# plumer/pbrs

Hardware: AMD Instinct MI355X
Metric: Msamples/s (higher is better)
Workload: dtype f32

## Files before the change

include/pbrs_gpu.h:

```cpp
#ifndef PBRS_GPU_H
#define PBRS_GPU_H

#include <stdint.h>

#ifdef __cplusplus
extern "C" {
#endif

#define PBRS_OK 0
#define PBRS_E_INVALID (-1)
#define PBRS_E_DEVICE (-2)
#define PBRS_E_NO_SCENE (-3)
#define PBRS_E_LIMIT (-4)

#define PBRS_LEAF_FLAG 0x80000000u
#define PBRS_TLAS_LEAF_KIND_SHIFT 8

typedef struct pbrs_node {
    float min[3];
    uint32_t a;
    float max[3];
    uint32_t b;
} pbrs_node;

// ... 109 lines not shown
    uint32_t tlas_height;
    uint32_t n_instances;
    const pbrs_instance* instances;
    uint32_t n_shapes;
    const pbrs_shape* shapes;
    uint32_t n_meshes;
    const pbrs_mesh* meshes;
    uint32_t n_blas_nodes;
    const pbrs_node* blas_nodes;
    uint32_t n_triangles;
    const pbrs_tri_verts* tri_verts;
    const pbrs_tri_shade* tri_shade;
    uint32_t n_materials;
    const pbrs_material* materials;
    uint32_t n_bxdfs;
    const pbrs_bxdf* bxdfs;
    uint32_t n_area_lights;
    const pbrs_area_light* area_lights;
    uint32_t n_delta_lights;
    const pbrs_delta_light* delta_lights;
    float env_constant[3];
    uint32_t env_kind;
    uint32_t n_textures;
    const pbrs_texture* textures;
    uint32_t n_tex_floats;
    const float* tex_floats;
    uint32_t n_tex_words;
    const uint32_t* tex_words;
    uint32_t env_texture;
    float env_scale[3];
    uint32_t n_fourier_tables;
    const pbrs_fourier_table* fourier_tables;
} pbrs_scene_desc;

typedef struct pbrs_camera {
    float center[3];
    uint32_t width;
    float c[3];
    uint32_t height;
    float a[3];
    float pad0;
    float b[3];
    float pad1;
} pbrs_camera;

typedef struct pbrs_stats {
    uint64_t samples;
    uint64_t closest_rays;
    uint64_t shadow_rays;
    uint64_t shade_events;
    uint64_t tlas_nodes, blas_nodes, instances, instance_hits, triangles, tri_shading;
    uint64_t spheres, quads, cuboids, disks;
    uint64_t shadow_tlas_nodes, shadow_blas_nodes, shadow_instances, shadow_triangles, shadow_prims;
    uint64_t invalid_samples;
    float ms_raygen, ms_extend, ms_shade, ms_shadow, ms_accumulate, ms_total;
    uint32_t launches_extend, launches_shadow, launches_shade, passes;
    uint32_t kernel_features_extend, kernel_features_shadow;
    uint64_t paths_at_bounce[16];
    uint64_t shadow_rays_at_bounce[16];
} pbrs_stats;
#define PBRS_STATS_MAX_BOUNCES 16

typedef struct pbrs_ctx pbrs_ctx;

int pbrs_create(int device_ordinal, pbrs_ctx** out);
void pbrs_destroy(pbrs_ctx*);
const char* pbrs_last_error(const pbrs_ctx*);
int pbrs_set_stream(pbrs_ctx*, void* hip_stream);

int pbrs_set_pass_overlap(pbrs_ctx*, int enabled);

int pbrs_upload_scene(pbrs_ctx*, const pbrs_scene_desc*);

typedef struct pbrs_render_params {
    uint32_t x0, y0, w, h;
    uint32_t strata_x, strata_y;
    uint32_t max_depth;
    uint32_t samples_per_pass;
    uint64_t seed;
    uint32_t collect_counters;
    uint32_t time_stages;
    uint32_t band_rows, band_count, band_index;
    uint32_t integrator;
} pbrs_render_params;
#define PBRS_INTEGRATOR_PATH 0u
#define PBRS_INTEGRATOR_DIRECT 1u
#define PBRS_INTEGRATOR_MATERIALS 2u
#define PBRS_INTEGRATOR_NORMALS 3u

int pbrs_render_tile(pbrs_ctx*, const pbrs_camera*, const pbrs_render_params*, float* rgb_out_host, pbrs_stats* stats_out);
int pbrs_render_tile_device(pbrs_ctx*, const pbrs_camera*, const pbrs_render_params*, float* rgb_out_device, pbrs_stats* stats_out);
int pbrs_collect_stats(pbrs_ctx*, pbrs_stats* stats_out);

typedef struct pbrs_aov_buffers {
    float* albedo;
    float* normal;
    float* coverage;
    float* depth;
    uint32_t* instance;
    uint32_t* material;
    uint32_t* prim;
} pbrs_aov_buffers;
int pbrs_render_tile_aovs(pbrs_ctx*, const pbrs_camera*, const pbrs_render_params*, float* rgb_out_host, const pbrs_aov_buffers* aovs_host,
                          pbrs_stats* stats_out);
int pbrs_render_tile_aovs_device(pbrs_ctx*, const pbrs_camera*, const pbrs_render_params*, float* rgb_out_device,
                                 const pbrs_aov_buffers* aovs_device, pbrs_stats* stats_out);

enum pbrs_filter_kind { PBRS_FILTER_BOX = 0, PBRS_FILTER_TRIANGLE = 1, PBRS_FILTER_GAUSSIAN = 2, PBRS_FILTER_MITCHELL = 3, PBRS_FILTER_LANCZOS = 4 };
#define PBRS_FILTER_MAX_RADIUS 4.0f
typedef struct pbrs_pixel_filter {
    uint32_t kind;
    float radius[2];
    float a, b;
    uint32_t pad;
} pbrs_pixel_filter;
int pbrs_render_tile_filtered(pbrs_ctx*, const pbrs_camera*, const pbrs_render_params*, const pbrs_pixel_filter*, float* rgb_out_host,
                              pbrs_stats* stats_out);
int pbrs_render_tile_filtered_device(pbrs_ctx*, const pbrs_camera*, const pbrs_render_params*, const pbrs_pixel_filter*,
                                     float* rgb_out_device, pbrs_stats* stats_out);

#define PBRS_DENOISE_MAX_ITERATIONS 6
#define PBRS_DENOISE_DEMODULATE 1u
#define PBRS_DENOISE_ID_STOP 2u
typedef struct pbrs_denoise_params {
    uint32_t w, h;
    uint32_t iterations;
    uint32_t flags;
    float sigma_color, sigma_normal, sigma_depth;
    float albedo_floor;
} pbrs_denoise_params;
typedef struct pbrs_denoise_guides {
    const float* albedo;
    const float* normal;
    const float* depth;
    const uint32_t* instance;
} pbrs_denoise_guides;
int pbrs_denoise(pbrs_ctx*, const pbrs_denoise_params*, const float* rgb_in_host, const pbrs_denoise_guides* guides_host, float* rgb_out_host);
int pbrs_denoise_device(pbrs_ctx*, const pbrs_denoise_params*, const float* rgb_in_device, const pbrs_denoise_guides* guides_device,
                        float* rgb_out_device);

typedef struct pbrs_hit_record {
    float t;
    uint32_t inst;
    uint32_t prim;
    float b1, b2;
} pbrs_hit_record;
int pbrs_intersect_rays(pbrs_ctx*, uint32_t n, const float* origins, const float* dirs, const float* tmax,
                        pbrs_hit_record* hits_out, uint8_t* occluded_out);
typedef struct pbrs_intersect_info {
    uint32_t wide_any, wide_closest;
    uint32_t slow_any, slow_closest;
} pbrs_intersect_info;
int pbrs_last_intersect_info(const pbrs_ctx*, pbrs_intersect_info* out);
int pbrs_camera_rays(pbrs_ctx*, const pbrs_camera*, const pbrs_render_params*, uint32_t sample_index, float* origins_out,
                     float* dirs_out);
int pbrs_numeric_eval(pbrs_ctx*, uint32_t fn, uint32_t n, const float* x, const float* y, float* out);
int pbrs_numeric_eval_k(pbrs_ctx*, uint32_t fn, uint32_t n, uint32_t k, const uint32_t* ops, uint32_t* out);
int pbrs_render_sample_radiance(pbrs_ctx*, const pbrs_camera*, const pbrs_render_params*, uint32_t sample_index, float* rgb_out_host);

int pbrs_render_tile_aovs_var(pbrs_ctx*, const pbrs_camera*, const pbrs_render_params*, float* rgb_out_host, const pbrs_aov_buffers* aovs_host,
                              float* variance_host, pbrs_stats* stats_out);
int pbrs_render_tile_aovs_var_device(pbrs_ctx*, const pbrs_camera*, const pbrs_render_params*, float* rgb_out_device,
                                     const pbrs_aov_buffers* aovs_device, float* variance_device, pbrs_stats* stats_out);

typedef struct pbrs_denoise_var_params {
    uint32_t w, h;
    uint32_t iterations;
    uint32_t flags;
    float sigma_luminance, sigma_normal, sigma_depth;
    float albedo_floor;
} pbrs_denoise_var_params;
typedef struct pbrs_denoise_var_guides {
    const float* albedo;
    const float* normal;
    const float* depth;
    const uint32_t* instance;
    const float* variance;
} pbrs_denoise_var_guides;
int pbrs_denoise_var(pbrs_ctx*, const pbrs_denoise_var_params*, const float* rgb_in_host, const pbrs_denoise_var_guides* guides_host,
                     float* rgb_out_host, float* variance_out_host);
int pbrs_denoise_var_device(pbrs_ctx*, const pbrs_denoise_var_params*, const float* rgb_in_device, const pbrs_denoise_var_guides* guides_device,
                            float* rgb_out_device, float* variance_out_device);

#define PBRS_MATTE_INSTANCE 0u
#define PBRS_MATTE_MATERIAL 1u
#define PBRS_MATTE_MAX_SLOTS 8u
typedef struct pbrs_matte_params {
    uint32_t key;
    uint32_t slots;
} pbrs_matte_params;
typedef struct pbrs_matte_buffers {
    uint32_t* ids;
    float* coverage;
    float* residual;
} pbrs_matte_buffers;
int pbrs_render_tile_matte(pbrs_ctx*, const pbrs_camera*, const pbrs_render_params*, float* rgb_out_host, const pbrs_aov_buffers* aovs_host,
                           float* variance_host, const pbrs_matte_params* params, const pbrs_matte_buffers* matte_host, pbrs_stats* stats_out);
int pbrs_render_tile_matte_device(pbrs_ctx*, const pbrs_camera*, const pbrs_render_params*, float* rgb_out_device,
                                  const pbrs_aov_buffers* aovs_device, float* variance_device, const pbrs_matte_params* params,
                                  const pbrs_matte_buffers* matte_device, pbrs_stats* stats_out);

#define PBRS_MATTE_MAX_SELECT 4096u
int pbrs_matte_mask(pbrs_ctx*, uint32_t w, uint32_t h, uint32_t slots, const uint32_t* ids_host, const float* coverage_host,
                    const uint32_t* select, uint32_t n_select, float* mask_out_host);
int pbrs_matte_mask_device(pbrs_ctx*, uint32_t w, uint32_t h, uint32_t slots, const uint32_t* ids_device, const float* coverage_device,
                           const uint32_t* select, uint32_t n_select, float* mask_out_device);

typedef struct pbrs_pass_buffers {
    float* direct;
    float* indirect;
    float* direct_variance;
    float* indirect_variance;
} pbrs_pass_buffers;
int pbrs_render_tile_passes(pbrs_ctx*, const pbrs_camera*, const pbrs_render_params*, float* rgb_out_host, const pbrs_aov_buffers* aovs_host,
                            float* variance_host, const pbrs_matte_params* matte_params, const pbrs_matte_buffers* matte_host,
                            const pbrs_pass_buffers* passes_host, pbrs_stats* stats_out);
int pbrs_render_tile_passes_device(pbrs_ctx*, const pbrs_camera*, const pbrs_render_params*, float* rgb_out_device,
                                   const pbrs_aov_buffers* aovs_device, float* variance_device, const pbrs_matte_params* matte_params,
                                   const pbrs_matte_buffers* matte_device, const pbrs_pass_buffers* passes_device, pbrs_stats* stats_out);

int pbrs_combine_passes(pbrs_ctx*, uint32_t w, uint32_t h, const float* direct_host, const float* indirect_host, float* rgb_out_host);
int pbrs_combine_passes_device(pbrs_ctx*, uint32_t w, uint32_t h, const float* direct_device, const float* indirect_device,
                               float* rgb_out_device);

#define PBRS_TEMPORAL_ID_TEST 1u
typedef struct pbrs_temporal_params {
    uint32_t w, h;
    uint32_t flags;
    float max_history;
    float depth_tolerance;
    float normal_tolerance;
    float min_temporal;
    uint32_t pad;
} pbrs_temporal_params;
typedef struct pbrs_temporal_frame {
    const float* rgb;
    const float* variance;
    const float* depth;
    const float* normal;
    const uint32_t* instance;
} pbrs_temporal_frame;
typedef struct pbrs_temporal_guides {
    const float* depth;
    const float* normal;
    const uint32_t* instance;
} pbrs_temporal_guides;
typedef struct pbrs_temporal_history {
    float* rgb;
    float* moments;
    float* length;
} pbrs_temporal_history;
int pbrs_temporal_accumulate(pbrs_ctx*, const pbrs_temporal_params*, const pbrs_camera* cam, const pbrs_camera* cam_prev,
                             const pbrs_temporal_frame* frame_host, const pbrs_temporal_guides* prev_host,
                             const pbrs_temporal_history* history_in_host, const pbrs_temporal_history* history_out_host, float* variance_out_host);
int pbrs_temporal_accumulate_device(pbrs_ctx*, const pbrs_temporal_params*, const pbrs_camera* cam, const pbrs_camera* cam_prev,
                                    const pbrs_temporal_frame* frame_device, const pbrs_temporal_guides* prev_device,
                                    const pbrs_temporal_history* history_in_device, const pbrs_temporal_history* history_out_device,
                                    float* variance_out_device);

#define PBRS_MOTION_IDENTITY 1u
typedef struct pbrs_instance_motion {
    float m[3][4];
    float n[3][3];
    uint32_t flags;
    uint32_t pad[2];
} pbrs_instance_motion;
int pbrs_temporal_accumulate_motion(pbrs_ctx*, const pbrs_temporal_params*, const pbrs_camera* cam, const pbrs_camera* cam_prev,
                                    const pbrs_temporal_frame* frame_host, const pbrs_temporal_guides* prev_host,
                                    const pbrs_temporal_history* history_in_host, const pbrs_temporal_history* history_out_host,
                                    float* variance_out_host, const pbrs_instance_motion* motion, uint32_t n_motion);
int pbrs_temporal_accumulate_motion_device(pbrs_ctx*, const pbrs_temporal_params*, const pbrs_camera* cam, const pbrs_camera* cam_prev,
                                           const pbrs_temporal_frame* frame_device, const pbrs_temporal_guides* prev_device,
                                           const pbrs_temporal_history* history_in_device, const pbrs_temporal_history* history_out_device,
                                           float* variance_out_device, const pbrs_instance_motion* motion, uint32_t n_motion);

int pbrs_motion_vectors(pbrs_ctx*, uint32_t w, uint32_t h, const pbrs_camera* cam, const pbrs_camera* cam_prev, const float* depth_host,
                        const uint32_t* instance_host, const pbrs_instance_motion* motion, uint32_t n_motion, float* motion_out_host,
                        float* prev_depth_out_host);
int pbrs_motion_vectors_device(pbrs_ctx*, uint32_t w, uint32_t h, const pbrs_camera* cam, const pbrs_camera* cam_prev,
                               const float* depth_device, const uint32_t* instance_device, const pbrs_instance_motion* motion,
                               uint32_t n_motion, float* motion_out_device, float* prev_depth_out_device);

#define PBRS_CLIP_MAX_RADIUS 3u
typedef struct pbrs_history_clip_params {
    uint32_t radius;
    float gamma;
    float clip_history;
    uint32_t flags;
} pbrs_history_clip_params;
int pbrs_temporal_accumulate_clip(pbrs_ctx*, const pbrs_temporal_params*, const pbrs_camera* cam, const pbrs_camera* cam_prev,
                                  const pbrs_temporal_frame* frame_host, const pbrs_temporal_guides* prev_host,
                                  const pbrs_temporal_history* history_in_host, const pbrs_temporal_history* history_out_host,
                                  float* variance_out_host, const pbrs_instance_motion* motion, uint32_t n_motion,
                                  const pbrs_history_clip_params* clip);
int pbrs_temporal_accumulate_clip_device(pbrs_ctx*, const pbrs_temporal_params*, const pbrs_camera* cam, const pbrs_camera* cam_prev,
                                         const pbrs_temporal_frame* frame_device, const pbrs_temporal_guides* prev_device,
                                         const pbrs_temporal_history* history_in_device, const pbrs_temporal_history* history_out_device,
                                         float* variance_out_device, const pbrs_instance_motion* motion, uint32_t n_motion,
                                         const pbrs_history_clip_params* clip);

#define PBRS_SPATIAL_ID_STOP 1u
#define PBRS_SPATIAL_ONLY_UNKNOWN 2u
#define PBRS_SPATIAL_MAX_RADIUS 3u
typedef struct pbrs_spatial_variance_params {
    uint32_t w, h;
    uint32_t radius;
// ... 74 lines not shown
```

pbrs_amd/api.py:

```python
import ctypes as C
import os

import numpy as np

from .spec import SceneSpec

from . import spec as _spec

_HERE = os.path.dirname(os.path.abspath(__file__))
_LIBDIR = os.path.join(_HERE, "lib")


class PbrsError(RuntimeError):
    pass


class Node(C.Structure):
    _fields_ = [("min", C.c_float * 3), ("a", C.c_uint32), ("max", C.c_float * 3), ("b", C.c_uint32)]


class SceneDesc(C.Structure):
    _fields_ = [("n_tlas_nodes", C.c_uint32), ("tlas_nodes", C.c_void_p), ("tlas_height", C.c_uint32),
                ("n_instances", C.c_uint32), ("instances", C.c_void_p),
                ("n_shapes", C.c_uint32), ("shapes", C.c_void_p),
# ... 253 lines not shown
                ("sigma_depth", C.c_float), ("min_temporal", C.c_float), ("pad", C.c_uint32)]

    @classmethod
    def make(cls, w, h, radius=3, sigma_normal=0.3, sigma_depth=0.2, min_temporal=4.0, id_stop=False, only_unknown=False):
        p = cls()
        p.w, p.h, p.radius = w, h, radius
        p.flags = (cls.ID_STOP if id_stop else 0) | (cls.ONLY_UNKNOWN if only_unknown else 0)
        p.sigma_normal, p.sigma_depth, p.min_temporal = sigma_normal, sigma_depth, min_temporal
        return p

    def as_dict(self):
        return {n: getattr(self, n) for n, _ in self._fields_}


class DisplayParams(C.Structure):
    CURVES = {"none": 0, "reinhard": 1, "aces": 2}
    ENCODES = {"sqrt": 0, "srgb": 1}
    QUANTIZERS = {"trunc": 0, "round": 1, "dither": 2}
    AUTO_EXPOSURE = 1
    BINS = 512
    _fields_ = [("w", C.c_uint32), ("h", C.c_uint32), ("curve", C.c_uint32), ("encode", C.c_uint32), ("quantize", C.c_uint32),
                ("flags", C.c_uint32), ("exposure", C.c_float), ("key", C.c_float), ("white", C.c_float), ("min_exposure", C.c_float),
                ("max_exposure", C.c_float), ("adapt", C.c_float), ("low_q16", C.c_uint32), ("high_q16", C.c_uint32), ("pad", C.c_uint32 * 2)]

    @classmethod
    def make(cls, w, h, curve="aces", encode="srgb", quantize="round", auto=False, exposure=1.0, key=0.18, white=None, min_exposure=2.0 ** -20,
             max_exposure=2.0 ** 20, adapt=1.0, low_q16=6554, high_q16=62259):
        p = cls()
        p.w, p.h = w, h
        p.curve = cls.CURVES[curve] if isinstance(curve, str) else curve
        p.encode = cls.ENCODES[encode] if isinstance(encode, str) else encode
        p.quantize = cls.QUANTIZERS[quantize] if isinstance(quantize, str) else quantize
        p.flags = cls.AUTO_EXPOSURE if auto else 0
        p.exposure, p.key, p.white = exposure, key, float("inf") if white is None else white
        p.min_exposure, p.max_exposure, p.adapt = min_exposure, max_exposure, adapt
        p.low_q16, p.high_q16 = low_q16, high_q16
        return p

    def as_dict(self):
        return {n: getattr(self, n) for n, _ in self._fields_ if n != "pad"}


class UpsampleParams(C.Structure):
    DEMODULATE, ID_STOP = 1, 2
    FACTORS, RADII = (2, 3, 4), (1, 2)
    _fields_ = [("w", C.c_uint32), ("h", C.c_uint32), ("factor", C.c_uint32), ("radius", C.c_uint32), ("flags", C.c_uint32),
                ("sigma_normal", C.c_float), ("sigma_depth", C.c_float), ("albedo_floor", C.c_float), ("min_weight", C.c_float),
                ("pad", C.c_uint32 * 3)]

    @classmethod
    def make(cls, w, h, factor=2, radius=1, sigma_normal=0.3, sigma_depth=0.2, albedo_floor=1e-3, min_weight=1e-3, demodulate=False,
             id_stop=False):
        p = cls()
        p.w, p.h, p.factor, p.radius = w, h, factor, radius
        p.flags = (cls.DEMODULATE if demodulate else 0) | (cls.ID_STOP if id_stop else 0)
        p.sigma_normal, p.sigma_depth, p.albedo_floor, p.min_weight = sigma_normal, sigma_depth, albedo_floor, min_weight
        return p

    @classmethod
    def for_guides(cls, w, h, factor, albedo=False, instance=False, **params):
        params.setdefault("demodulate", bool(albedo))
        params.setdefault("id_stop", bool(instance))
        return cls.make(w, h, factor, **params)

    @property
    def low_size(self):
        return (self.w + self.factor - 1) // self.factor, (self.h + self.factor - 1) // self.factor

    def as_dict(self):
        return {n: getattr(self, n) for n, _ in self._fields_ if n != "pad"}


def scaled_camera(camera, factor):
    factor = int(factor)
    if factor < 1:
        raise ValueError("the factor is a positive integer")
    cam = Camera.from_buffer_copy(camera)
    cam.width, cam.height = (camera.width + factor - 1) // factor, (camera.height + factor - 1) // factor
    f = np.float32(factor)
    for k in range(3):
        cam.a[k] = np.float32(camera.a[k]) * f
        cam.b[k] = np.float32(camera.b[k]) * f
    return cam


def _upscale_params(upscale, guides):
    if upscale is None or upscale is False:
        return None
    if isinstance(upscale, dict):
        up = dict(upscale)
        factor = int(up.pop("factor", 2))
    elif isinstance(upscale, (int, np.integer)) and not isinstance(upscale, bool):
        up, factor = {}, int(upscale)
    else:
        raise ValueError("upscale is None, a factor or a dict of UpsampleParams.make's keywords plus \"factor\"")
    if factor not in UpsampleParams.FACTORS:
        raise ValueError(f"the upscale factor is one of {UpsampleParams.FACTORS}, not {factor}")
    UpsampleParams.for_guides(1, 1, factor, "albedo" in guides, "instance" in guides, **up)
    return factor, up


class DisplayIO(C.Structure):
    _fields_ = [(n, C.c_void_p) for n in ("exposure_in", "exposure_out", "histogram_out")]


def _display_params(display):
    if display is None or display is False:
        return None
    if display is not True and not isinstance(display, dict):
        raise ValueError("display is None, True or a dict of DisplayParams.make's keywords")
    dp = {} if display is True else dict(display)
    dp.setdefault("auto", True)
    DisplayParams.make(1, 1, **dp)
    return dp


class SpatialVarianceGuides(C.Structure):
    _fields_ = [(n, C.c_void_p) for n in ("depth", "normal", "instance")]


TEMPORAL_FRAME = {"rgb": (3, np.float32), "variance": (1, np.float32), "depth": (1, np.float32), "normal": (3, np.float32),
                  "instance": (1, np.uint32)}
TEMPORAL_GUIDES = {n: TEMPORAL_FRAME[n] for n in ("depth", "normal", "instance")}
TEMPORAL_HISTORY = {"rgb": (3, np.float32), "moments": (2, np.float32), "length": (1, np.float32)}
SPATIAL_VARIANCE_PLANES = {"moments": (2, np.float32), "length": (1, np.float32), "variance": (1, np.float32)}


def _temporal_struct(cls, layout, ptrs, what):
    s = cls()
    for n, ptr in dict(ptrs).items():
        if n not in layout:
            raise ValueError(f"unknown {what} plane {n!r}; known: {list(layout)}")
        setattr(s, n, ptr)
    return s


def _matte_select(select):
    sel = np.unique(np.asarray(select, dtype=np.int64).reshape(-1))
    if sel.size and (sel[0] < 0 or sel[-1] > 0xFFFFFFFF):
        raise ValueError("a selected id is not a u32")
    return np.ascontiguousarray(sel, dtype=np.uint32)


DENOISE_GUIDES = {"albedo": (3, np.float32), "normal": (3, np.float32), "depth": (1, np.float32), "instance": (1, np.uint32)}

HIT_DTYPE = np.dtype([("t", np.float32), ("inst", np.uint32), ("prim", np.uint32), ("b1", np.float32), ("b2", np.float32)])
NUMERIC_FNS = {"sin": 0, "cos": 1, "tan": 2, "atan": 3, "atan2": 4, "acos": 5, "exp": 6, "ln": 7, "hypot": 8, "div": 9,
               "sqrt": 10, "asin": 11, "powi": 12, "fract": 13, "floor": 14, "box_quotient": 15, "trunc": 16, "f32_to_i32": 17, "ldexp": 18, "max": 19,
               "min": 20, "signum": 21, "weak_recip": 22, "sincos64_sin_hi": 23, "sincos64_sin_lo": 24, "sincos64_cos_hi": 25,
               "sincos64_cos_lo": 26, "rng_u32": 27, "rng_f32": 28}
NUMERIC_K_FNS = {"mul_add": 0, "clamp": 1, "slab_filter": 2, "rng_init_lo": 3, "rng_init_hi": 4, "rng_stream_u32": 5, "rng_stream_f32": 6}

GPU_SYMBOLS = ["pbrs_create", "pbrs_destroy", "pbrs_last_error", "pbrs_set_stream", "pbrs_set_pass_overlap", "pbrs_upload_scene", "pbrs_render_tile",
               "pbrs_render_tile_device", "pbrs_collect_stats", "pbrs_intersect_rays", "pbrs_last_intersect_info", "pbrs_camera_rays",
               "pbrs_numeric_eval", "pbrs_numeric_eval_k", "pbrs_render_sample_radiance", "pbrs_render_tile_aovs", "pbrs_render_tile_aovs_device",
               "pbrs_render_tile_filtered", "pbrs_render_tile_filtered_device", "pbrs_denoise", "pbrs_denoise_device",
               "pbrs_render_tile_aovs_var", "pbrs_render_tile_aovs_var_device", "pbrs_denoise_var", "pbrs_denoise_var_device",
               "pbrs_render_tile_matte", "pbrs_render_tile_matte_device", "pbrs_matte_mask", "pbrs_matte_mask_device",
               "pbrs_render_tile_passes", "pbrs_render_tile_passes_device", "pbrs_combine_passes", "pbrs_combine_passes_device",
               "pbrs_temporal_accumulate", "pbrs_temporal_accumulate_device", "pbrs_temporal_accumulate_motion",
               "pbrs_temporal_accumulate_motion_device", "pbrs_motion_vectors", "pbrs_motion_vectors_device",
               "pbrs_temporal_accumulate_clip", "pbrs_temporal_accumulate_clip_device",
               "pbrs_spatial_variance", "pbrs_spatial_variance_device",
               "pbrs_display_params_default", "pbrs_display", "pbrs_display_device",
               "pbrs_upsample_params_default", "pbrs_upsample", "pbrs_upsample_device"]
HOST_SYMBOLS = ["pbrs_host_scene_build", "pbrs_host_scene_free", "pbrs_host_scene_desc", "pbrs_host_scene_camera",
                "pbrs_host_scene_stack_depth", "pbrs_host_last_error",
                "pbrs_host_load_pbrt", "pbrs_loaded_scene_spec", "pbrs_loaded_scene_free", "pbrs_host_load_error", "pbrs_loaded_scene_filter",
                "pbrs_host_write_exr", "pbrs_host_write_png", "pbrs_host_write_png_rgba8", "pbrs_host_io_error"]

_host = None
_gpu = None


def lib_paths():
    return os.path.join(_LIBDIR, "libpbrs_host.so"), os.path.join(_LIBDIR, "libpbrs_gpu.so")


def host_lib():
    global _host
    if _host is None:
        path = os.environ.get("PBRS_HOST_LIB") or lib_paths()[0]
        if not os.path.exists(path):
            raise PbrsError(f"{path} is missing: run `python -c 'import __graft_entry__ as g; g.build()'` (make -C pbrs_amd/csrc)")
        L = C.CDLL(path)
        L.pbrs_host_scene_build.argtypes = [C.c_void_p, C.POINTER(C.c_void_p)]
        L.pbrs_host_scene_free.argtypes = [C.c_void_p]
        L.pbrs_host_scene_desc.restype = C.POINTER(SceneDesc)
        L.pbrs_host_scene_desc.argtypes = [C.c_void_p]
        L.pbrs_host_scene_camera.restype = C.POINTER(Camera)
        L.pbrs_host_scene_camera.argtypes = [C.c_void_p]
        L.pbrs_host_scene_stack_depth.restype = C.c_uint32
        L.pbrs_host_scene_stack_depth.argtypes = [C.c_void_p]
        L.pbrs_host_last_error.restype = C.c_char_p
        L.pbrs_host_load_pbrt.argtypes = [C.c_char_p, C.POINTER(C.c_void_p)]
        L.pbrs_loaded_scene_spec.restype = C.POINTER(SceneSpec)
        L.pbrs_loaded_scene_spec.argtypes = [C.c_void_p]
        L.pbrs_loaded_scene_free.argtypes = [C.c_void_p]
        L.pbrs_loaded_scene_filter.argtypes = [C.c_void_p, C.c_void_p]
        L.pbrs_host_load_error.restype = C.c_char_p
        L.pbrs_host_write_exr.argtypes = [C.c_char_p, C.c_void_p, C.c_uint32, C.c_uint32]
        L.pbrs_host_write_png.argtypes = [C.c_char_p, C.c_void_p, C.c_uint32, C.c_uint32]
        L.pbrs_host_write_png_rgba8.argtypes = [C.c_char_p, C.c_void_p, C.c_uint32, C.c_uint32]
        L.pbrs_host_io_error.restype = C.c_char_p
        _host = L
    return _host


def gpu_lib():
    global _gpu
    if _gpu is None:
        path = os.environ.get("PBRS_GPU_LIB") or lib_paths()[1]
        if not os.path.exists(path):
            raise PbrsError(f"{path} is missing: the HIP extension must be built (make -C pbrs_amd/csrc); there is no CPU fallback")
        L = C.CDLL(path)
        L.pbrs_create.argtypes = [C.c_int, C.POINTER(C.c_void_p)]
        L.pbrs_destroy.argtypes = [C.c_void_p]
        L.pbrs_last_error.restype = C.c_char_p
        L.pbrs_last_error.argtypes = [C.c_void_p]
        L.pbrs_set_stream.argtypes = [C.c_void_p, C.c_void_p]
        L.pbrs_set_pass_overlap.argtypes = [C.c_void_p, C.c_int]
        L.pbrs_upload_scene.argtypes = [C.c_void_p, C.c_void_p]
        L.pbrs_render_tile.argtypes = [C.c_void_p, C.c_void_p, C.c_void_p, C.c_void_p, C.c_void_p]
        L.pbrs_render_tile_device.argtypes = [C.c_void_p, C.c_void_p, C.c_void_p, C.c_void_p, C.c_void_p]
        L.pbrs_collect_stats.argtypes = [C.c_void_p, C.c_void_p]
        L.pbrs_intersect_rays.argtypes = [C.c_void_p, C.c_uint32] + [C.c_void_p] * 5
        L.pbrs_last_intersect_info.argtypes = [C.c_void_p, C.c_void_p]
        L.pbrs_camera_rays.argtypes = [C.c_void_p, C.c_void_p, C.c_void_p, C.c_uint32, C.c_void_p, C.c_void_p]
        L.pbrs_numeric_eval.argtypes = [C.c_void_p, C.c_uint32, C.c_uint32, C.c_void_p, C.c_void_p, C.c_void_p]
        L.pbrs_numeric_eval_k.argtypes = [C.c_void_p, C.c_uint32, C.c_uint32, C.c_uint32, C.c_void_p, C.c_void_p]
        L.pbrs_render_sample_radiance.argtypes = [C.c_void_p, C.c_void_p, C.c_void_p, C.c_uint32, C.c_void_p]
        L.pbrs_render_tile_aovs.argtypes = [C.c_void_p] * 6
        L.pbrs_render_tile_aovs_device.argtypes = [C.c_void_p] * 6
        L.pbrs_render_tile_filtered.argtypes = [C.c_void_p] * 6
        L.pbrs_render_tile_filtered_device.argtypes = [C.c_void_p] * 6
        L.pbrs_denoise.argtypes = [C.c_void_p] * 5
        L.pbrs_denoise_device.argtypes = [C.c_void_p] * 5
        L.pbrs_render_tile_aovs_var.argtypes = [C.c_void_p] * 7
        L.pbrs_render_tile_aovs_var_device.argtypes = [C.c_void_p] * 7
        L.pbrs_denoise_var.argtypes = [C.c_void_p] * 6
        L.pbrs_denoise_var_device.argtypes = [C.c_void_p] * 6
        L.pbrs_render_tile_matte.argtypes = [C.c_void_p] * 9
        L.pbrs_render_tile_matte_device.argtypes = [C.c_void_p] * 9
        L.pbrs_matte_mask.argtypes = [C.c_void_p, C.c_uint32, C.c_uint32, C.c_uint32, C.c_void_p, C.c_void_p, C.c_void_p, C.c_uint32, C.c_void_p]
        L.pbrs_matte_mask_device.argtypes = L.pbrs_matte_mask.argtypes
        L.pbrs_render_tile_passes.argtypes = [C.c_void_p] * 10
        L.pbrs_render_tile_passes_device.argtypes = [C.c_void_p] * 10
        L.pbrs_combine_passes.argtypes = [C.c_void_p, C.c_uint32, C.c_uint32, C.c_void_p, C.c_void_p, C.c_void_p]
        L.pbrs_combine_passes_device.argtypes = L.pbrs_combine_passes.argtypes
        L.pbrs_temporal_accumulate.argtypes = [C.c_void_p] * 9
        L.pbrs_temporal_accumulate_device.argtypes = [C.c_void_p] * 9
        L.pbrs_temporal_accumulate_motion.argtypes = [C.c_void_p] * 10 + [C.c_uint32]
        L.pbrs_temporal_accumulate_motion_device.argtypes = L.pbrs_temporal_accumulate_motion.argtypes
        L.pbrs_temporal_accumulate_clip.argtypes = L.pbrs_temporal_accumulate_motion.argtypes + [C.c_void_p]
        L.pbrs_temporal_accumulate_clip_device.argtypes = L.pbrs_temporal_accumulate_clip.argtypes
        L.pbrs_motion_vectors.argtypes = [C.c_void_p, C.c_uint32, C.c_uint32] + [C.c_void_p] * 5 + [C.c_uint32, C.c_void_p, C.c_void_p]
        L.pbrs_motion_vectors_device.argtypes = L.pbrs_motion_vectors.argtypes
        L.pbrs_spatial_variance.argtypes = [C.c_void_p] * 7
        L.pbrs_spatial_variance_device.argtypes = [C.c_void_p] * 7
        L.pbrs_display_params_default.argtypes = [C.c_uint32, C.c_uint32, C.c_void_p]
        L.pbrs_display_params_default.restype = None
        L.pbrs_display.argtypes = [C.c_void_p] * 5
        L.pbrs_display_device.argtypes = [C.c_void_p] * 5
        L.pbrs_upsample_params_default.argtypes = [C.c_uint32, C.c_uint32, C.c_uint32, C.c_void_p]
        L.pbrs_upsample_params_default.restype = None
        L.pbrs_upsample.argtypes = [C.c_void_p] * 7
        L.pbrs_upsample_device.argtypes = [C.c_void_p] * 7
        _gpu = L
    return _gpu


_hip = None


def hip_runtime():
    global _hip
    if _hip is None:
        gpu_lib()
        path = next(line.split()[-1] for line in open("/proc/self/maps") if "libamdhip64" in line)
        L = C.CDLL(path)
        L.hipMalloc.argtypes = [C.POINTER(C.c_void_p), C.c_size_t]
        L.hipMemcpy.argtypes = [C.c_void_p, C.c_void_p, C.c_size_t, C.c_int]
        L.hipFree.argtypes = [C.c_void_p]
        _hip = L
    return _hip


def orbited(camera, about, axis, degrees):
    k = np.asarray(axis, dtype=np.float64)
    k = k / np.linalg.norm(k)
    t = np.radians(degrees)

    def rot(v):
        return v * np.cos(t) + np.cross(k, v) * np.sin(t) + k * np.dot(k, v) * (1.0 - np.cos(t))
    about = np.asarray(about, dtype=np.float64)
    out = Camera()
    out.width, out.height = camera.width, camera.height
    out.center[:] = [float(v) for v in about + rot(np.array(list(camera.center), dtype=np.float64) - about)]
    for n in ("c", "a", "b"):
        getattr(out, n)[:] = [float(v) for v in rot(np.array(list(getattr(camera, n)), dtype=np.float64))]
    return out


def instance_motion(scene, scene_prev):
    fwd, inv = scene.instance_transforms()
    fwd_p, inv_p = scene_prev.instance_transforms()
    if len(fwd) != len(fwd_p):
        raise ValueError(f"instance_motion: {len(fwd)} instances beside {len(fwd_p)} in the previous scene")
    table = (InstanceMotion * max(len(fwd), 1))()
    bottom = np.array([[0.0, 0.0, 0.0, 1.0]])
    for i in range(len(fwd)):
        r = table[i]
        if fwd[i].tobytes() == fwd_p[i].tobytes() and inv[i].tobytes() == inv_p[i].tobytes():
            m, n, r.flags = np.eye(3, 4), np.eye(3), InstanceMotion.IDENTITY
        else:
            m = (np.vstack([fwd_p[i].astype(np.float64), bottom]) @ np.vstack([inv[i].astype(np.float64), bottom]))[:3]
            n = (fwd[i, :, :3].astype(np.float64) @ inv_p[i, :, :3].astype(np.float64)).T
        for a in range(3):
            r.m[a][:] = [float(v) for v in m[a].astype(np.float32)]
            r.n[a][:] = [float(v) for v in n[a].astype(np.float32)]
    return table


def _motion_args(motion):
    if motion is None:
        return None, 0
    if not isinstance(motion, C.Array) or motion._type_ is not InstanceMotion:
        raise ValueError("a motion table is a ctypes array of InstanceMotion (api.instance_motion)")
    return C.addressof(motion), len(motion)


INTEGRATORS = {"path": 0, "direct": 1, "materials": 2, "normals": 3}


class LoadedScene:

    def __init__(self, path):
        h = C.c_void_p()
        rc = host_lib().pbrs_host_load_pbrt(os.fsencode(path), C.byref(h))
        if rc != 0:
            raise PbrsError(f"pbrs_host_load_pbrt({path}) failed ({rc}): {host_lib().pbrs_host_load_error().decode()}")
        self._h = h
        self.spec = host_lib().pbrs_loaded_scene_spec(h).contents

    def build(self):
        return self.spec

    def pixel_filter(self):
        f = PixelFilter()
        rc = host_lib().pbrs_loaded_scene_filter(self._h, C.byref(f))
        if rc != 0:
            raise PbrsError(f"pbrs_loaded_scene_filter failed ({rc}): {host_lib().pbrs_host_load_error().decode()}")
        return f

    def close(self):
        if getattr(self, "_h", None):
            host_lib().pbrs_loaded_scene_free(self._h)
            self._h = None

    def __del__(self):
        self.close()


def load_pbrt(path):
    return LoadedScene(path)


def write_image(path, rgb):
    rgb = np.ascontiguousarray(rgb, dtype=np.float32)
    h, w, _ = rgb.shape
    fn = host_lib().pbrs_host_write_exr if str(path).lower().endswith(".exr") else host_lib().pbrs_host_write_png
    rc = fn(os.fsencode(path), rgb.ctypes.data, w, h)
    if rc != 0:
        raise PbrsError(f"writing {path} failed ({rc}): {host_lib().pbrs_host_io_error().decode()}")


def write_image_u8(path, rgba8):
    img = np.asarray(rgba8)
    if img.dtype != np.uint8 or img.ndim != 3 or img.shape[2] not in (3, 4):
# ... 631 lines not shown

    @staticmethod
    def _spatial_params(spatial, tparams, guides):
        if spatial is None or spatial is False:
            return None
        sp = {} if spatial is True else dict(spatial)
        sp.setdefault("min_temporal", tparams.get("min_temporal", TemporalParams.make(1, 1).min_temporal))
        sp.setdefault("id_stop", "instance" in guides)
        SpatialVarianceParams.make(1, 1, **sp)
        return sp

    def render_temporal(self, cameras, strata_x, strata_y, depth, seeds, guides=("albedo", "normal", "depth", "instance"), samples_per_pass=0,
                        temporal=None, spatial=None, clip=None, display=None, upscale=None, **params):
        self._denoise_guide_names(guides)
        if "depth" not in guides:
            raise ValueError("render_temporal reprojects through the depth AOV: guides must hold \"depth\"")
        cameras, seeds = list(cameras), list(seeds)
        if len(cameras) != len(seeds):
            raise ValueError(f"{len(cameras)} cameras beside {len(seeds)} seeds")
        frames = [(None, cam, seed) for cam, seed in zip(cameras, seeds)]
        for out in self._temporal_frames(frames, strata_x, strata_y, depth, guides, samples_per_pass, temporal, params, False, spatial, clip, display,
                                         upscale):
            yield out[:4]

    def render_animation(self, frames, strata_x, strata_y, depth, guides=("albedo", "normal", "depth", "instance"), samples_per_pass=0,
                         temporal=None, motion_vectors=False, spatial=None, clip=None, display=None, upscale=None, **params):
        self._denoise_guide_names(guides)
        if "depth" not in guides or "instance" not in guides:
            raise ValueError("render_animation reprojects through the depth AOV and the instance ids: guides must hold \"depth\" and \"instance\"")
        for out in self._temporal_frames(frames, strata_x, strata_y, depth, guides, samples_per_pass, temporal, params, motion_vectors, spatial, clip, display,
                                         upscale):
            yield out if motion_vectors else out[:4]

    def _temporal_frames(self, frames, strata_x, strata_y, depth, guides, samples_per_pass, temporal, params, motion_vectors, spatial=None,
                         clip=None, display=None, upscale=None):
        tparams = dict(temporal or {})
        TemporalParams.make(1, 1, **tparams)
        clip = _history_clip(clip)
        sparams = self._spatial_params(spatial, tparams, guides)
        dparams = _display_params(display)
        uparams = _upscale_params(upscale, guides)
        hip = hip_runtime()
        kept = [n for n in ("depth", "normal", "instance") if n in guides]
        dev = {}
        try:
            cam_prev = scene_prev = None
            w = h = fw = fh = n_rgb = 0
            for i, (scene, cam, seed) in enumerate(frames):
                table = None
                if scene is not None:
                    self.upload(scene)
                    if scene_prev is not None:
                        table = instance_motion(scene, scene_prev)
                    scene_prev = scene
                cam = Camera.from_buffer_copy(cam if cam is not None else self.scene.camera)
                cam_full, tile = cam, None
                if uparams is not None:
                    cam = scaled_camera(cam_full, uparams[0])
                    tile = (0, 0, cam.width, cam.height)
                if i == 0:
                    fw, fh = self.scene.width, self.scene.height
                    w, h = (fw, fh) if uparams is None else (cam.width, cam.height)
                    n_rgb = 3 * w * h * 4
                    sizes = {"rgb": n_rgb, "out": n_rgb, VARIANCE: w * h * 4, "acc_variance": w * h * 4}
                    for k in (0, 1):
                        sizes.update({f"{n}{k}": DENOISE_GUIDES[n][0] * w * h * 4 for n in kept})
                        sizes.update({f"h_{n}{k}": ch * w * h * 4 for n, (ch, _) in TEMPORAL_HISTORY.items()})
                    sizes.update({n: DENOISE_GUIDES[n][0] * w * h * 4 for n in guides if n not in kept})
                    if motion_vectors:
                        sizes["motion"], sizes["prev_depth"] = 2 * w * h * 4, w * h * 4
                    if uparams is not None:
                        sizes["up"] = 3 * fw * fh * 4
                        sizes.update({f"{n}_hi": DENOISE_GUIDES[n][0] * fw * fh * 4 for n in guides})
                    if dparams is not None:
                        sizes["display"], sizes["exposure"] = fw * fh * 4, 4
                    for n, nbytes in sizes.items():
                        ptr = C.c_void_p()
                        if hip.hipMalloc(C.byref(ptr), nbytes) != 0:
                            raise PbrsError(f"hipMalloc of {nbytes} bytes for a temporal sequence failed")
                        dev[n] = ptr
                elif (self.scene.width, self.scene.height) != (fw, fh):
                    raise ValueError(f"frame {i} has a film of {self.scene.width} x {self.scene.height}, the sequence {fw} x {fh}")
                cur, old = i & 1, (i & 1) ^ 1
                gp = {n: dev[f"{n}{cur}" if n in kept else n].value for n in guides}
                bufs, _ = self._aov_device(gp)
                self._render_device(self._params(strata_x, strata_y, depth, seed, tile, samples_per_pass), dev["rgb"].value, bufs,
                                    dev[VARIANCE].value, camera=cam)
                frame = {"rgb": dev["rgb"].value, "variance": dev[VARIANCE].value, **{n: gp[n] for n in kept}}
                hist = [{n: dev[f"h_{n}{k}"].value for n in TEMPORAL_HISTORY} for k in (0, 1)]
                self.temporal_accumulate_device(frame, hist[cur], w, h, cam, hist[old] if i else None,
                                                {n: dev[f"{n}{old}"].value for n in kept} if i else None, cam_prev,
                                                dev["acc_variance"].value, motion=table if i else None, clip=clip, **tparams)
                if motion_vectors and i:
                    self.motion_vectors_device(gp["depth"], dev["motion"].value, w, h, cam, cam_prev, gp.get("instance") if table else None, table,
                                               dev["prev_depth"].value)
                if sparams is not None:
                    self.spatial_variance_device(hist[cur]["moments"], hist[cur]["length"], dev["acc_variance"].value, dev["acc_variance"].value,
                                                 w, h, {n: gp[n] for n in kept}, **sparams)
                self.denoise_var_device(hist[cur]["rgb"], dev["out"].value, w, h, dev["acc_variance"].value, gp, **params)
                shown_src = dev["out"]
                if uparams is not None:
                    gh = {n: dev[f"{n}_hi"].value for n in guides}
                    self._render_guides_device(dev["up"].value, gh, seed, camera=cam_full)
                    self.upsample_device(dev["out"].value, dev["up"].value, fw, fh, uparams[0], gp, gh, **uparams[1])
                    shown_src = dev["up"]
                if dparams is not None:
                    self.display_device(shown_src.value, dev["display"].value, fw, fh,
                                        {"exposure_in": dev["exposure"].value if i else None, "exposure_out": dev["exposure"].value}, **dparams)
                stats = self.collect_stats()
                if dparams is not None:
                    shown, e = np.empty((fh, fw, 4), dtype=np.uint8), np.zeros(1, dtype=np.float32)
                    if hip.hipMemcpy(shown.ctypes.data, dev["display"], shown.nbytes, 2) != 0 or hip.hipMemcpy(e.ctypes.data, dev["exposure"], 4, 2) != 0:
                        raise PbrsError("hipMemcpy of a temporal sequence's display image failed")
                    stats["display"], stats["exposure"] = shown, e[0]
                if uparams is not None:
                    stats["low_res"] = (w, h)
                images = []
                for src in (shown_src, dev[f"h_rgb{cur}"], dev["rgb"]):
                    img = np.empty((fh, fw, 3) if src is dev.get("up") else (h, w, 3), dtype=np.float32)
                    if hip.hipMemcpy(img.ctypes.data, src, img.nbytes, 2) != 0:
                        raise PbrsError("hipMemcpy of a temporal sequence's image failed")
                    images.append(img)
                mv = None
                if motion_vectors:
                    mv, wq = np.zeros((h, w, 2), dtype=np.float32), np.full((h, w), np.inf, dtype=np.float32)
                    if i and (hip.hipMemcpy(mv.ctypes.data, dev["motion"], mv.nbytes, 2) != 0 or
                              hip.hipMemcpy(wq.ctypes.data, dev["prev_depth"], wq.nbytes, 2) != 0):
                        raise PbrsError("hipMemcpy of the motion vectors failed")
                    if motion_vectors == "prev_depth":
                        mv = np.concatenate([mv, wq[:, :, None]], axis=2)
                cam_prev = cam
                yield images[0], images[1], images[2], stats, mv
        finally:
            for ptr in dev.values():
                hip.hipFree(ptr)

    def collect_stats(self):
        st = Stats()
        self._check(self._L.pbrs_collect_stats(self._h, C.addressof(st)), "pbrs_collect_stats")
        return st.as_dict()

    def intersect(self, origins, dirs, tmax, closest=True, anyhit=True):
        origins = np.ascontiguousarray(origins, dtype=np.float32)
        dirs = np.ascontiguousarray(dirs, dtype=np.float32)
        tmax = np.ascontiguousarray(tmax, dtype=np.float32)
        n = len(tmax)
        hits = np.empty(n, dtype=HIT_DTYPE) if closest else None
        occ = np.empty(n, dtype=np.uint8) if anyhit else None
        self._check(self._L.pbrs_intersect_rays(self._h, n, origins.ctypes.data, dirs.ctypes.data, tmax.ctypes.data,
                                                hits.ctypes.data if closest else None, occ.ctypes.data if anyhit else None),
                    "pbrs_intersect_rays")
        return hits, occ

    def last_intersect_info(self):
        v = (C.c_uint32 * 4)()
        self._check(self._L.pbrs_last_intersect_info(self._h, C.addressof(v)), "pbrs_last_intersect_info")
        return {"wide_any": int(v[0]), "wide_closest": int(v[1]), "slow_any": int(v[2]), "slow_closest": int(v[3])}

    def camera_rays(self, sample, strata_x, strata_y, seed, tile=None):
        p = self._params(strata_x, strata_y, 1, seed, tile)
        o = np.empty((p.w * p.h, 3), dtype=np.float32)
        d = np.empty((p.w * p.h, 3), dtype=np.float32)
        self._check(self._L.pbrs_camera_rays(self._h, C.addressof(self.scene.camera), C.addressof(p), sample, o.ctypes.data, d.ctypes.data),
                    "pbrs_camera_rays")
        return o, d

    def sample_radiance(self, sample, strata_x, strata_y, depth, seed, tile=None, integrator="path"):
        p = self._params(strata_x, strata_y, depth, seed, tile, integrator=integrator)
        out = np.empty((p.h, p.w, 3), dtype=np.float32)
        self._check(self._L.pbrs_render_sample_radiance(self._h, C.addressof(self.scene.camera), C.addressof(p), sample, out.ctypes.data),
                    "pbrs_render_sample_radiance")
        return out

    def numeric_eval(self, fn, x, y=None):
        x = np.ascontiguousarray(x, dtype=np.float32)
        out = np.empty_like(x)
        yp = None
        if y is not None:
            y = np.ascontiguousarray(y, dtype=np.float32)
            yp = y.ctypes.data
        self._check(self._L.pbrs_numeric_eval(self._h, NUMERIC_FNS[fn], x.size, x.ctypes.data, yp, out.ctypes.data), "pbrs_numeric_eval")
        return out

    def numeric_eval_k(self, fn, ops):
        ops = np.ascontiguousarray(ops)
        assert ops.ndim == 2 and ops.dtype.itemsize == 4
        out = np.empty(len(ops), dtype=np.uint32)
        self._check(self._L.pbrs_numeric_eval_k(self._h, NUMERIC_K_FNS[fn], ops.shape[0], ops.shape[1], ops.ctypes.data, out.ctypes.data),
                    "pbrs_numeric_eval_k")
        return out
```

pbrs_amd/csrc/device/accumulate.h:

```cpp
#pragma once
#include "path_state.h"

__global__ void __launch_bounds__(256) k_nee_resolve(PathState st, const uint32_t* queue, const uint32_t* count) {
  const uint32_t n = count[0];
  for (uint32_t i = blockIdx.x * blockDim.x + threadIdx.x; i < n; i += gridDim.x * blockDim.x) {
    uint32_t slot = queue[i];
    bool occ0 = at(st.occ[0], slot) != 0, occ1 = at(st.occ[1], slot) != 0;
    const float4 n0 = st.nee[0][slot], n1 = st.nee[1][slot], n2 = st.nee[2][slot];
    f3 c1 = xyz(n0), c2 = xyz(n1);
    f3 one = gray(0.0f);
    if (!occ0) one = one + c1;
    if (!occ1) one = one + c2;
    f3 nb = xyz(n2);
    const float4 rl = st.L[slot];
    f3 L = xyz(rl);
    L = L + cmul(nb, one * n0.w) * n1.w;
    st.L[slot] = pack4(L, rl.w);
  }
}

__global__ void __launch_bounds__(256) k_accumulate(PathState st, float* sum, uint32_t n_pixels, uint32_t k_count, uint32_t chunk, uint32_t w,
                                                     uint32_t tiles8_per_row, unsigned long long* nonfinite) {
    uint32_t p = blockIdx.x * blockDim.x + threadIdx.x;
    if (p >= n_pixels) return;
    f3 s = mk3(sum[p], sum[n_pixels + p], sum[2 * n_pixels + p]);
    uint32_t bad = 0;
    for (uint32_t k = 0; k < k_count; ++k) {
        const uint32_t slot = slot_of_sample(k, order_of_pixel(p, w, tiles8_per_row), n_pixels, k_count, chunk);
        const f3 l = xyz(st.L[slot]);
        bad += (pn_isfinite(l.x) && pn_isfinite(l.y) && pn_isfinite(l.z)) ? 0u : 1u;
        s = s + l;
    }
    if (__ballot(bad != 0u)) {
        for (int off = 32; off > 0; off >>= 1) bad += __shfl_down(bad, off, 64);
        if ((threadIdx.x & 63u) == 0) atomicAdd(nonfinite, (unsigned long long)bad);
    }
    sum[p] = s.x;
    sum[n_pixels + p] = s.y;
    sum[2 * n_pixels + p] = s.z;
}
__global__ void __launch_bounds__(256) k_finalize(const float* sum, float* rgb, uint32_t n_pixels, float inv_spp) {
    uint32_t p = blockIdx.x * blockDim.x + threadIdx.x;
    if (p >= n_pixels) return;
    rgb[3 * p] = sum[p] * inv_spp;
    rgb[3 * p + 1] = sum[n_pixels + p] * inv_spp;
    rgb[3 * p + 2] = sum[2 * n_pixels + p] * inv_spp;
}

__global__ void k_sum_bounce_counts(const uint32_t* act, const unsigned long long* ns, uint32_t n_pass, uint32_t n_bounces, unsigned long long* acc) {
    const uint32_t b = threadIdx.x;
    if (b >= n_bounces) return;
    const uint32_t at = b < PBRS_STATS_MAX_BOUNCES ? b : PBRS_STATS_MAX_BOUNCES - 1u;
    atomicAdd(acc + at, (unsigned long long)(b == 0 ? n_pass : act[b]));
    atomicAdd(acc + PBRS_STATS_MAX_BOUNCES + at, ns[b] >> 32);
}
```

pbrs_amd/csrc/device/extend.h:

```cpp
#pragma once
#include "path_state.h"
#include "traverse.h"

template <bool STATS>
PD void flush_counters(const Cnt<STATS>& cnt, GlobalCounters* g, bool valid, uint32_t rays, uint32_t hits) {
    if (!STATS) return;
    const WorkCounters& c = cnt.c;
    uint32_t v[12] = {c.tlas_nodes, c.blas_nodes, c.instances, c.instance_hits, c.triangles, c.tri_shading,
                      c.spheres,    c.quads,      c.cuboids,   c.disks,         rays,        hits};
    unsigned long long* out = reinterpret_cast<unsigned long long*>(g);
    for (int k = 0; k < 12; ++k) {
        uint32_t x = valid ? v[k] : 0u;
        for (int off = 32; off > 0; off >>= 1) x += __shfl_down(x, off, 64);
        if ((threadIdx.x & 63u) == 0 && x) atomicAdd(out + k, (unsigned long long)x);
    }
}

#ifndef PBRS_NODE_STEPS_LONG
#define PBRS_NODE_STEPS_LONG 3u
#endif
#ifndef PBRS_CHUNK_MAX
#define PBRS_CHUNK_MAX 512u
#endif
#ifndef PBRS_TRAV_WAVES
#define PBRS_TRAV_WAVES 5
#endif
#ifndef PBRS_LEAN_EXTEND_WAVES
#define PBRS_LEAN_EXTEND_WAVES 6
#endif
#ifndef PBRS_SHADOW_WAVES
#define PBRS_SHADOW_WAVES 6
#endif

#ifndef PBRS_EXT_XFER_MIN
#define PBRS_EXT_XFER_MIN 8
#endif
#ifndef PBRS_EXT_LEAF_MIN
#define PBRS_EXT_LEAF_MIN 10
#endif
#ifndef PBRS_SHD_XFER_MIN
#define PBRS_SHD_XFER_MIN 2
#endif
#ifndef PBRS_SHD_LEAF_MIN
#define PBRS_SHD_LEAF_MIN 8
#endif
#define PBRS_MORE_NODE_STEPS(walk, S, stk, cnt, NSTEPS, FULL)                      \
    do {                                                                           \
        _Pragma("unroll") for (uint32_t k_ = 1; k_ < (NSTEPS); ++k_) {             \
            PBRS_KP_LANE(5 + (k_ < 2u ? k_ : 2u), walk.mode == PBRS_WALK_NODE);    \
            if (walk.mode == PBRS_WALK_NODE) {                                     \
                if constexpr (FULL) walk.node_step(S, stk, cnt);                   \
                else walk.node_step_fast(S, stk, cnt);                             \
            }                                                                      \
        }                                                                          \
    } while (0)
#define PBRS_STEP_WALK(walk, S, stk, cnt, XFER_MIN, LEAF_MIN, NSTEPS, FULL)                                                \
    do {                                                                                                       \
        PBRS_KP_WAVE(0);                                                                                       \
        PBRS_KP_LANE(10, walk.mode == PBRS_WALK_NODE || walk.mode == PBRS_WALK_LEAF || walk.mode == PBRS_WALK_XFER); \
        const uint32_t nx = (uint32_t)__popcll(__ballot(walk.mode == PBRS_WALK_XFER));                         \
        if (nx) {                                                                                              \
            if (nx >= XFER_MIN || __ballot(walk.mode == PBRS_WALK_NODE || walk.mode == PBRS_WALK_LEAF) == 0) { \
                PBRS_PROBE_XFER_COUNT(cnt);                                                                    \
                PBRS_KP_WAVE(3);                                                                               \
                PBRS_KP_LANE(4, walk.mode == PBRS_WALK_XFER);                                                  \
                if (walk.mode == PBRS_WALK_XFER) walk.xfer_step(S, stk, cnt);                                   \
            }                                                                                                  \
        }                                                                                                      \
        PBRS_TT(1);                                                                                            \
        PBRS_PROBE_UTIL_COUNT(walk, cnt);                                                                      \
        PBRS_KP_LANE(5, walk.mode == PBRS_WALK_NODE);                                                          \
        if (__ballot(walk.mode == PBRS_WALK_NODE)) PBRS_KP_WAVE(11);                                           \
        if (walk.mode == PBRS_WALK_NODE) walk.node_step(S, stk, cnt);                                          \
        PBRS_MORE_NODE_STEPS(walk, S, stk, cnt, NSTEPS, FULL);                                                            \
        PBRS_TT(2);                                                                                            \
        const uint32_t nl = (uint32_t)__popcll(__ballot(walk.mode == PBRS_WALK_LEAF));                         \
        if (nl && (nl >= LEAF_MIN || __ballot(walk.mode == PBRS_WALK_NODE) == 0)) {                            \
            PBRS_PROBE_LEAF_COUNT(cnt);                                                                        \
            PBRS_KP_WAVE(8);                                                                                   \
            PBRS_KP_LANE(9, walk.mode == PBRS_WALK_LEAF);                                                      \
            walk.leaf_wave(S, cnt);                                                                            \
        }                                                                                                      \
        PBRS_TT(3);                                                                                            \
    } while (0)
struct WaveWork {
    uint32_t cur, end, chunk;
    uint32_t head, tried;
    PD bool left() const { return tried < PBRS_WORK_HEADS || cur < end; }
};
PD WaveWork wave_work_init(uint32_t n) {
    uint32_t waves = gridDim.x * (blockDim.x >> 6);
    uint32_t chunk = n / (waves * 4u);
    chunk = chunk < 64u ? 64u : (chunk > PBRS_CHUNK_MAX ? PBRS_CHUNK_MAX : (chunk & ~63u));
    return WaveWork{0u, 0u, chunk, blockIdx.x % PBRS_WORK_HEADS, 0u};
}
PD uint32_t work_segment(uint32_t n, uint32_t h) {
    return h >= PBRS_WORK_HEADS ? n : (uint32_t)(((unsigned long long)n * h / PBRS_WORK_HEADS) & ~63ull);
}
PD uint32_t wave_fetch(WaveWork& w, bool need, uint32_t* heads, uint32_t n) {
    const uint64_t mask = __ballot(need);
    const uint32_t want = (uint32_t)__popcll(mask), rank = lane_prefix(mask);
    const uint32_t avail = w.end - w.cur;
    uint32_t idx = (need && rank < avail) ? w.cur + rank : 0xffffffffu;
    if (want <= avail) {
        w.cur += want;
        return idx;
    }
    w.cur = w.end;
    const int leader = __ffsll((unsigned long long)mask) - 1;
    while (w.tried < PBRS_WORK_HEADS) {
        const uint32_t seg_lo = work_segment(n, w.head), seg_hi = work_segment(n, w.head + 1);
        uint32_t base = 0;
        if ((int)(threadIdx.x & 63u) == leader) base = atomicAdd(heads + w.head * PBRS_WORK_HEAD_STRIDE, w.chunk);
        base = __shfl(base, leader, 64);
        const uint32_t len = seg_hi - seg_lo;
        const uint32_t lo = seg_lo + (base < len ? base : len), hi = seg_lo + (base + w.chunk < len ? base + w.chunk : len);
        if (base + w.chunk >= len) {
            w.head = (w.head + 1u) % PBRS_WORK_HEADS;
            w.tried++;
        }
        if (lo == hi) continue;
        const uint32_t rest = want - avail, got = hi - lo;
        if (need && rank >= avail && rank - avail < got) idx = lo + (rank - avail);
        w.cur = lo + (rest < got ? rest : got);
        w.end = hi;
        break;
    }
    return idx;
}
PD void wave_append_slow(bool slow, uint32_t item, uint32_t* list, uint32_t* count) {
    const uint64_t m = __ballot(slow);
    if (m == 0) return;
    const int leader = __ffsll((unsigned long long)m) - 1;
    uint32_t base = 0;
    if ((int)(threadIdx.x & 63u) == leader) base = atomicAdd(count, (uint32_t)__popcll(m));
    base = __shfl(base, leader, 64);
    if (slow) list[base + lane_prefix(m)] = item;
}
#ifndef PBRS_WIDE_SHADOW_WAVES
#define PBRS_WIDE_SHADOW_WAVES 5
#endif
#ifndef PBRS_WIDE_NODE_STEPS
#define PBRS_WIDE_NODE_STEPS 2u
#endif
template <uint32_t ARITY, bool STATS, uint32_t FEAT>
struct AnySel {
    typedef AnyWalkW<FEAT> type;
};
template <bool STATS, uint32_t FEAT>
struct AnySel<0u, STATS, FEAT> {
    typedef AnyWalk<STATS, (FEAT & (PBRS_FEAT_ALL | PBRS_FEAT_LDS_TOP))> type;
};
#define PBRS_WALK_ARITY(STATS, FEAT) ((STATS) ? 0u : ((FEAT) & PBRS_FEAT_WIDE) ? 4u : 0u)
#ifndef PBRS_NODE_STEPS_SHORT
#define PBRS_NODE_STEPS_SHORT 1u
#endif
#define PBRS_WALK_NSTEPS(FEAT, ARITY) \
    (!((FEAT) & PBRS_FEAT_LONG_WALKS) ? ((ARITY) == 0u ? PBRS_NODE_STEPS_SHORT : 1u) : (ARITY) == 4u ? PBRS_WIDE_NODE_STEPS : PBRS_NODE_STEPS_LONG)
PD DevScene stage_scene(const DevScene& G, uint32_t* lds_base) {
    DevScene S = G;
    uint4* dst = reinterpret_cast<uint4*>(__builtin_assume_aligned(lds_base + G.lds_off_words, 16));
    S.nodes = reinterpret_cast<const pbrs_node*>(dst);
    dst = stage_array(dst, G.nodes, G.lds_nodes * (uint32_t)(sizeof(pbrs_node) / 16));
    S.tv = reinterpret_cast<const pbrs_tri_verts*>(dst);
    dst = stage_array(dst, G.tv, G.lds_tris * (uint32_t)(sizeof(pbrs_tri_verts) / 16));
    S.inst = reinterpret_cast<const pbrs_instance*>(dst);
    dst = stage_array(dst, G.inst, G.lds_inst * (uint32_t)(sizeof(pbrs_instance) / 16));
    S.shapes = reinterpret_cast<const pbrs_shape*>(dst);
    stage_array(dst, G.shapes, G.lds_shapes * (uint32_t)(sizeof(pbrs_shape) / 16));
    __syncthreads();
    return S;
}
static_assert(sizeof(pbrs_node) % 16 == 0 && sizeof(pbrs_tri_verts) % 16 == 0 && sizeof(pbrs_instance) % 16 == 0 && sizeof(pbrs_shape) % 16 == 0, "stage_scene copies 16-byte pieces");

PD DevScene stage_top(const DevScene& G, uint32_t* lds_base) {
    DevScene S = G;
    uint4* dst = reinterpret_cast<uint4*>(__builtin_assume_aligned(lds_base + G.lds_off_words, 16));
    S.nodes_top = reinterpret_cast<const pbrs_node*>(dst);
    stage_array(dst, G.nodes, G.lds_nodes * (uint32_t)(sizeof(pbrs_node) / 16));
    __syncthreads();
    return S;
}

template <bool STATS, uint32_t FEAT>
__global__ void __launch_bounds__(256, STATS ? 3 : (FEAT & PBRS_FEAT_SHADING_CHECK) ? PBRS_TRAV_WAVES : PBRS_LEAN_EXTEND_WAVES)
    k_extend(DevScene G, PathState st, uint32_t set, const uint32_t* count, uint32_t n_direct, uint32_t* next, GlobalCounters* gc, const uint32_t* indirect,
             uint32_t* slow_list, uint32_t* slow_count, uint32_t split) {
    extern __shared__ __attribute__((aligned(16))) uint32_t lds_stack[];
    const DevScene S = (!STATS && (FEAT & PBRS_FEAT_LDS_SCENE)) ? stage_scene(G, lds_stack) : (!STATS && (FEAT & PBRS_FEAT_LDS_TOP)) ? stage_top(G, lds_stack) : G;
    const uint32_t n = count ? *count : n_direct;
    const float4* q0 = st.q[set][0];
    const float4* q1 = st.q[set][1];
    LaneStack stk{lds_stack + threadIdx.x, q0, q1, 0u};
    Cnt<STATS> cnt;
    cnt.init();
    uint32_t nrays = 0, nhit = 0;
    ClosestWalk<STATS, (FEAT & (PBRS_FEAT_ALL | PBRS_FEAT_LDS_TOP | PBRS_FEAT_EXTENT))> walk;
    walk.mode = PBRS_WALK_IDLE;
    PBRS_KP_DECL(walk);
    PBRS_TT_DECL;
    uint32_t item = 0;
    WaveWork work = wave_work_init(n);
    for (;;) {
        uint64_t live = __ballot(walk.mode == PBRS_WALK_NODE || walk.mode == PBRS_WALK_LEAF || walk.mode == PBRS_WALK_XFER);
        if ((uint32_t)__popcll(live) < S.refill_below) {
            PBRS_KP_WAVE(1);
            if (walk.mode == PBRS_WALK_DONE) {
                walk.finish(cnt);
                const Hit& h = walk.best;
                nhit += h.inst != 0xffffffffu ? 1u : 0u;
                uint32_t cls = (S.n_classes > 1u && h.inst != 0xffffffffu) ? S.inst[h.inst].pad[0] : 0u;
                if (split) {
                    cls = 1u;
                    if (h.inst == 0xffffffffu) {
                        const bool specular = (item >> 31) != 0u;
                        cls = (specular || ((split & PBRS_QSPLIT_ENV) && S.has_env != 0u)) ? 1u : 0u;
                    }
                }
                const uint32_t pos = item & 0x7fffffffu;
                if (!split || cls) st_stream(&st.hit[pos], make_float4(h.t, __uint_as_float(h.inst), __uint_as_float(h.prim), __uint_as_float(split ? 0u : cls)));
                if (S.n_classes > 1u || split) st.cls[pos] = (uint8_t)cls;
                walk.mode = PBRS_WALK_IDLE;
            }
            if (work.left()) {
                uint32_t idx = wave_fetch(work, walk.mode == PBRS_WALK_IDLE, next, n);
                if (idx != 0xffffffffu) {
                    if (indirect) idx = indirect[idx];
                    stk.item = idx;
                    const float4 a = q0[idx], b = q1[idx];
                    item = idx | (__float_as_uint(a.w) & 0x80000000u);
                    walk.start(S, xyz(a), xyz(b), pn_inf(), stk);
                    nrays++;
                    PBRS_KP_LANE(2, true);
                }
                walk.scan_wave(S, cnt);
                live = __ballot(walk.mode == PBRS_WALK_NODE || walk.mode == PBRS_WALK_LEAF || walk.mode == PBRS_WALK_XFER);
            }
            if (live == 0) break;
        }
        PBRS_TT(0);
        PBRS_STEP_WALK(walk, S, stk, cnt, PBRS_EXT_XFER_MIN, PBRS_EXT_LEAF_MIN, PBRS_WALK_NSTEPS(FEAT, 0u), ((FEAT & PBRS_FEAT_FULL_STEPS) != 0u));
    }
    flush_counters<STATS>(cnt, gc, true, nrays, nhit);
    if (!STATS) PBRS_KP_FLUSH(0, walk);
    if (!STATS) PBRS_TT_FLUSH(0);
}
```

pbrs_amd/csrc/device/intersect.h:

```cpp
#pragma once
#include "extend.h"

template <bool WIDE_ANY>
__global__ void __launch_bounds__(256) k_intersect_rays(DevScene S, uint32_t n, const float4* origins, const float4* dirs, const float* tmax,
                                                       pbrs_hit_record* hits, uint8_t* occluded, uint32_t* info) {
    extern __shared__ __attribute__((aligned(16))) uint32_t lds_stack[];
    LaneStack stk{lds_stack + threadIdx.x, origins, dirs, 0u};
    Cnt<false> cnt;
    for (uint32_t base = blockIdx.x * blockDim.x; base < n; base += gridDim.x * blockDim.x) {
        const uint32_t i = base + threadIdx.x;
        const bool active = i < n;
        f3 o = gray(0.0f), d = gray(1.0f);
        float t_max = 0.0f;
        if (active) {
            o = xyz(origins[i]);
            d = xyz(dirs[i]);
            t_max = tmax[i];
            stk.item = i;
        }
        if (hits) {
            Hit h;
            if (S.exact_extent) tlas_closest<false, PBRS_FEAT_EXTENT>(S, active, o, d, t_max, stk, h, cnt);
            else tlas_closest<false>(S, active, o, d, t_max, stk, h, cnt);
            if (active) {
                pbrs_hit_record r;
                r.t = h.t;
                r.inst = h.inst;
                r.prim = 0;
                if (h.inst != 0xffffffffu && S.inst[h.inst].shape_kind == PBRS_SHAPE_MESH) r.prim = S.ts[h.prim].orig;
                r.b1 = h.b1;
                r.b2 = h.b2;
                hits[i] = r;
            }
        }
        if (occluded) {
            bool slow = false;
            const bool occ = WIDE_ANY ? tlas_any_wide(S, active, o, d, t_max, stk, slow) : tlas_any<false>(S, active, o, d, t_max, stk, cnt);
            if (active) {
                occluded[i] = occ ? 1 : 0;
                if (slow) atomicAdd(info, 1u);
            }
        }
    }
}
```

pbrs_amd/csrc/device/scene.h:

```cpp
#pragma once
#include <stddef.h>
#include <stdint.h>

#include "../../../include/pbrs_gpu.h"

constexpr uint32_t kBlock = 256;
constexpr size_t kLdsBytesPerCU = 160 * 1024;

struct pbrs_wnode;
struct DevScene {
    const pbrs_node* nodes;
    const pbrs_instance* inst;
    const pbrs_shape* shapes;
    const pbrs_mesh* meshes;
    const pbrs_tri_verts* tv;
    const pbrs_tri_shade* ts;
    const pbrs_material* mats;
    const pbrs_bxdf* bxdfs;
    const pbrs_area_light* alights;
    const pbrs_delta_light* dlights;
    uint32_t n_area, n_delta;
    float env[3];
    uint32_t has_env;
    uint32_t fast_slab;
    uint32_t exact_extent;
    uint32_t flat_off, n_flat;
    uint32_t features;
    uint32_t refill_below;
    uint32_t refill_below_shadow;
    const pbrs_texture* textures;
    const float* tex_floats;
    const uint32_t* tex_words;
    uint32_t env_kind, env_texture;
    float env_scale[3];
    const pbrs_fourier_table* fourier;
    uint32_t n_classes;
    const pbrs_wnode* wnodes;
    uint32_t wide_cap;
    uint32_t lds_off_words, lds_nodes, lds_tris, lds_inst, lds_shapes;
    const pbrs_node* nodes_top;
    uint32_t n_inst, n_shapes, n_tris, n_mats, n_bxdfs;
};

#define PBRS_INSTANCE_TRANSLATION 0x100u
#define PBRS_FEAT_ANALYTIC 1u
#define PBRS_FEAT_SHADING_CHECK 2u
#define PBRS_FEAT_FLAT_TLAS 4u
#define PBRS_FEAT_ALL 7u
#define PBRS_FEAT_EXTENT 256u
#define PBRS_FEAT_LONG_WALKS 8u
#define PBRS_FEAT_WIDE 16u
#define PBRS_FEAT_LDS_TOP 128u
#define PBRS_FEAT_LDS_SCENE 64u
#define PBRS_FEAT_FULL_STEPS 32u
#define PBRS_FLAT_TLAS_MIN 2u
#ifndef PBRS_FLAT_TLAS_MAX
#define PBRS_FLAT_TLAS_MAX 20u
#endif
#ifndef PBRS_FLAT_TLAS_MAX_ANYHIT
#define PBRS_FLAT_TLAS_MAX_ANYHIT 32u
#endif

struct pbrs_wnode {
    float lo[3][4];
    float hi[3][4];
    uint32_t child[4];
    uint32_t pad[4];
};
#ifndef PBRS_WIDE_STACK_MAX
#define PBRS_WIDE_STACK_MAX 16
#endif
#ifndef PBRS_WIDE_MIN_LEVELS
#define PBRS_WIDE_MIN_LEVELS 4u
#endif
#define PBRS_WREF_LEAF 0x80000000u
#define PBRS_WREF_NONE 0xffffffffu
#define PBRS_WREF_INDEX 0x07ffffffu
#define PBRS_WREF_AXIS_SHIFT 27
#define PBRS_WIDE_UNUSED_PLANE 1152921504606846976.0f

#ifndef PBRS_REFILL_BELOW_SHORT
#define PBRS_REFILL_BELOW_SHORT 20u
#endif
#ifndef PBRS_REFILL_BELOW_LONG
#define PBRS_REFILL_BELOW_LONG 48u
#endif
#ifndef PBRS_REFILL_BELOW_LONG_SHADOW
#define PBRS_REFILL_BELOW_LONG_SHADOW 40u
#endif
#define PBRS_LONG_WALK_HEIGHT 12u

#define PBRS_SHADE_LAMBERT 1u
#define PBRS_SHADE_LIGHT_SPHERE 2u
#define PBRS_SHADE_LIGHT_TRIANGLE 4u
#define PBRS_SHADE_FOURIER 8u
#define PBRS_SHADE_FOURIER_ONLY 16u
#define PBRS_SHADE_LDS_RECORDS 32u
#define PBRS_SHADE_LDS_TRIS 64u
#define PBRS_MAX_CLASSES 16u

#define PBRS_PERSISTENT_BLOCKS 1536
#ifndef PBRS_WORK_HEADS
#define PBRS_WORK_HEADS 8u
#endif
#define PBRS_WORK_HEAD_STRIDE 32u
#define PBRS_SORT_TILE 16384u
#define PBRS_QSPLIT_ON 1u
#define PBRS_QSPLIT_ENV 2u
```

pbrs_amd/csrc/host/kernel_choice.cpp:

```cpp
#include "kernel_choice.h"

#include <algorithm>

namespace pbrs {

KernelChoice choose_kernels(const SceneFacts& f, const DevOverrides& dev) {
    KernelChoice p;
    const bool long_walks = dev.long_walks.value_or(f.long_walks);
    const bool full_steps = dev.full_steps.value_or(f.full_steps);
    const uint32_t steps = long_walks ? PBRS_FEAT_LONG_WALKS | (full_steps ? PBRS_FEAT_FULL_STEPS : 0u) : 0u;
    p.wide_shadow = f.tlas_scanned && f.wide_ok && dev.wide_shadow;
    const bool lds_scene = dev.lds_scene && !p.wide_shadow && !full_steps && f.stack_bytes + f.scene_bytes <= kLdsBytesPerCU / 8;
    const bool lds_top = dev.lds_top && !lds_scene && !f.tlas_scanned && !full_steps && f.stack_bytes + f.top_bytes + 512 <= kLdsBytesPerCU / 7;
    p.lds_staging = lds_scene ? PBRS_FEAT_LDS_SCENE : lds_top ? PBRS_FEAT_LDS_TOP : 0u;
    const size_t stack = std::max(f.stack_bytes, dev.lds_min);
    const size_t staged = stack + (lds_scene ? f.scene_bytes : lds_top ? f.top_bytes : 0u);
    if (f.exact_extent) {
        p.extend[0] = {kExtentFeatures, stack};
        p.extend[1] = {kStatsKey | kExtentFeatures, stack};
    } else {
        p.extend[0] = {(f.features & PBRS_FEAT_ALL) | steps | p.lds_staging, staged};
        p.extend[1] = {kStatsKey | PBRS_FEAT_ALL, stack};
    }
    const uint32_t shadow_feat = (f.features & PBRS_FEAT_ANALYTIC) | (f.tlas_scanned ? PBRS_FEAT_FLAT_TLAS : 0u) | steps;
    if (p.wide_shadow) {
        p.shadow[0] = {shadow_feat | PBRS_FEAT_WIDE, f.wide_stack_bytes};
        p.shadow_slow = {shadow_feat, stack};
    } else {
        p.shadow[0] = {shadow_feat | p.lds_staging, staged};
    }
    p.shadow[1] = {kStatsKey | kShadowStatsFeatures, stack};
    p.split_queue = f.n_classes <= 1u && dev.split_queue;

    const uint32_t shade_lds = f.shade_lds & dev.shade_lds;
    const uint32_t path_lds = (shade_lds == PBRS_SHADE_LDS_ALL || shade_lds == PBRS_SHADE_LDS_RECORDS) ? shade_lds : 0u;
    const size_t path_lds_bytes = path_lds == PBRS_SHADE_LDS_ALL ? f.shade_rec_bytes + f.shade_tri_bytes : path_lds ? f.shade_rec_bytes : 0u;
    uint32_t spec = f.lambert ? (PBRS_SHADE_LAMBERT | f.light_spec) & dev.shade_spec : 0u;
    if (!(spec & PBRS_SHADE_LAMBERT)) spec = 0u;
    auto shade = [](IntegratorChoice& ip, uint32_t integ, bool tex, uint32_t sp, size_t lds, uint32_t range) {
        ip.shade[ip.n_shade++] = ShadeKey{integ, tex, sp, lds, range};
    };
    auto path_untextured = [&](IntegratorChoice& ip, uint32_t sp, uint32_t range) { shade(ip, PBRS_INTEGRATOR_PATH, false, sp | path_lds, path_lds_bytes, range); };
    const bool sorted = f.n_classes > 1u && dev.sort_classes;
    for (uint32_t i = PBRS_INTEGRATOR_PATH; i <= PBRS_INTEGRATOR_DIRECT; ++i) {
        IntegratorChoice& ip = p.integ[i];
        const bool path = i == PBRS_INTEGRATOR_PATH;
        const bool split = sorted && path && f.lambert_class && dev.split_lambert && !f.textured && !f.fourier;
        const bool fsplit = sorted && f.fourier && f.fourier_class && dev.split_fourier;
        ip.order = (split || fsplit) ? IntegratorChoice::CLASS_MAJOR : sorted ? IntegratorChoice::CLASS_SORT : IntegratorChoice::NO_ORDER;
        ip.last_class = split ? f.lambert_class : fsplit ? f.fourier_class : 0u;
        if (fsplit) {
            shade(ip, i, false, PBRS_SHADE_FOURIER_ALONE, 0, f.fourier_class);
            shade(ip, i, f.textured, 0u, 0, PBRS_MAX_CLASSES);
        } else if (f.fourier && f.fourier_class && f.n_classes == 1u) {
            shade(ip, i, false, PBRS_SHADE_FOURIER_ALONE, 0, 0u);
        } else if (f.fourier) {
            shade(ip, i, true, PBRS_SHADE_FOURIER, 0, 0u);
        } else if (f.textured) {
            shade(ip, i, true, 0u, 0, 0u);
        } else if (!path) {
            shade(ip, i, false, 0u, 0, 0u);
        } else if (split) {
            path_untextured(ip, PBRS_SHADE_LAMBERT | f.light_spec, f.lambert_class);
            path_untextured(ip, 0u, PBRS_MAX_CLASSES);
        } else {
            path_untextured(ip, spec, 0u);
        }
    }
    shade(p.integ[PBRS_INTEGRATOR_MATERIALS], PBRS_INTEGRATOR_MATERIALS, false, 0u, 0, 0u);
    shade(p.integ[PBRS_INTEGRATOR_NORMALS], PBRS_INTEGRATOR_NORMALS, false, 0u, 0, 0u);
    return p;
}

}
```

pbrs_amd/csrc/host/kernel_choice.h:

```cpp
#pragma once
#include <cstddef>
#include <cstdint>
#include <optional>

#include "../device/scene.h"

namespace pbrs {

struct DevOverrides {
    bool overlap_passes = true;
    bool sort_classes = true;
    bool split_lambert = true;
    bool split_fourier = true;
    bool split_queue = true;
    bool wide_shadow = true;
    bool lds_scene = true;
    bool lds_top = true;
    bool raygen_tiles8 = true;
    uint32_t shade_spec = ~0u;
    uint32_t shade_lds = ~0u;
    std::optional<bool> long_walks, full_steps;
    std::optional<uint32_t> overlap_from, refill_below;
    std::optional<uint32_t> raygen_chunk;
    size_t lds_min = 0;
};

struct SceneFacts {
    uint32_t features = 0;
    bool tlas_scanned = false;
    bool exact_extent = false;
    bool long_walks = false;
    bool full_steps = false;
    bool wide_ok = false;
    size_t stack_bytes = 0;
    size_t wide_stack_bytes = 0;
    size_t scene_bytes = 0;
    size_t top_bytes = 0;
    uint32_t n_classes = 0;
    uint32_t lambert_class = 0;
    uint32_t fourier_class = 0;
    bool textured = false;
    bool fourier = false;
    bool lambert = false;
    uint32_t light_spec = 0;
    uint32_t shade_lds = 0;
    size_t shade_rec_bytes = 0, shade_tri_bytes = 0;
};

constexpr uint32_t kStatsKey = 512u;
constexpr uint32_t kTraversalKeys = 2u * kStatsKey;
constexpr uint32_t kExtentFeatures = PBRS_FEAT_ANALYTIC | PBRS_FEAT_SHADING_CHECK | PBRS_FEAT_EXTENT;
constexpr uint32_t kShadowStatsFeatures = PBRS_FEAT_ANALYTIC | PBRS_FEAT_FLAT_TLAS;
constexpr bool extend_key_ok(uint32_t k) {
    const uint32_t f = k & ~kStatsKey;
    if (f & PBRS_FEAT_EXTENT) return f == kExtentFeatures;
    if (k & kStatsKey) return f == PBRS_FEAT_ALL;
    if (f & PBRS_FEAT_WIDE) return false;
    if ((f & PBRS_FEAT_FULL_STEPS) && !(f & PBRS_FEAT_LONG_WALKS)) return false;
    if ((f & PBRS_FEAT_LDS_SCENE) && (f & PBRS_FEAT_FULL_STEPS)) return false;
    if ((f & PBRS_FEAT_LDS_TOP) && (f & (PBRS_FEAT_LDS_SCENE | PBRS_FEAT_FULL_STEPS | PBRS_FEAT_FLAT_TLAS))) return false;
    return true;
}
constexpr bool shadow_key_ok(uint32_t k) {
    const uint32_t f = k & ~kStatsKey;
    if (k & kStatsKey) return f == kShadowStatsFeatures;
    if (f & (PBRS_FEAT_SHADING_CHECK | PBRS_FEAT_EXTENT)) return false;
    if ((f & PBRS_FEAT_FULL_STEPS) && !(f & PBRS_FEAT_LONG_WALKS)) return false;
    if ((f & PBRS_FEAT_LDS_SCENE) && (f & (PBRS_FEAT_WIDE | PBRS_FEAT_FULL_STEPS))) return false;
    if ((f & PBRS_FEAT_LDS_TOP) && (f & (PBRS_FEAT_LDS_SCENE | PBRS_FEAT_WIDE | PBRS_FEAT_FULL_STEPS | PBRS_FEAT_FLAT_TLAS))) return false;
    if ((f & PBRS_FEAT_WIDE) && !(f & PBRS_FEAT_FLAT_TLAS)) return false;
    return true;
}

#define PBRS_SHADE_LDS_ALL (PBRS_SHADE_LDS_RECORDS | PBRS_SHADE_LDS_TRIS)
#define PBRS_SHADE_FOURIER_ALONE (PBRS_SHADE_FOURIER | PBRS_SHADE_FOURIER_ONLY)
#define PBRS_SHADE_KERNELS(X)                                                                                                            \
                                                                                         \
    X(PBRS_INTEGRATOR_PATH, false, 0u)                                                                                                   \
    X(PBRS_INTEGRATOR_PATH, false, PBRS_SHADE_LAMBERT)                                                                                   \
    X(PBRS_INTEGRATOR_PATH, false, PBRS_SHADE_LAMBERT | PBRS_SHADE_LIGHT_SPHERE)                                                         \
    X(PBRS_INTEGRATOR_PATH, false, PBRS_SHADE_LAMBERT | PBRS_SHADE_LIGHT_TRIANGLE)                                                       \
    X(PBRS_INTEGRATOR_PATH, false, PBRS_SHADE_LDS_RECORDS)                                                                               \
    X(PBRS_INTEGRATOR_PATH, false, PBRS_SHADE_LDS_RECORDS | PBRS_SHADE_LAMBERT)                                                          \
    X(PBRS_INTEGRATOR_PATH, false, PBRS_SHADE_LDS_RECORDS | PBRS_SHADE_LAMBERT | PBRS_SHADE_LIGHT_SPHERE)                                \
    X(PBRS_INTEGRATOR_PATH, false, PBRS_SHADE_LDS_RECORDS | PBRS_SHADE_LAMBERT | PBRS_SHADE_LIGHT_TRIANGLE)                              \
    X(PBRS_INTEGRATOR_PATH, false, PBRS_SHADE_LDS_ALL)                                                                                   \
    X(PBRS_INTEGRATOR_PATH, false, PBRS_SHADE_LDS_ALL | PBRS_SHADE_LAMBERT)                                                              \
    X(PBRS_INTEGRATOR_PATH, false, PBRS_SHADE_LDS_ALL | PBRS_SHADE_LAMBERT | PBRS_SHADE_LIGHT_SPHERE)                                    \
    X(PBRS_INTEGRATOR_PATH, false, PBRS_SHADE_LDS_ALL | PBRS_SHADE_LAMBERT | PBRS_SHADE_LIGHT_TRIANGLE)                                  \
                                                                    \
    X(PBRS_INTEGRATOR_PATH, true, 0u)                                                                                                    \
    X(PBRS_INTEGRATOR_PATH, true, PBRS_SHADE_FOURIER)                                                                                    \
    X(PBRS_INTEGRATOR_PATH, false, PBRS_SHADE_FOURIER_ALONE)                                                                             \
    X(PBRS_INTEGRATOR_DIRECT, false, 0u)                                                                                                 \
    X(PBRS_INTEGRATOR_DIRECT, true, 0u)                                                                                                  \
    X(PBRS_INTEGRATOR_DIRECT, true, PBRS_SHADE_FOURIER)                                                                                  \
    X(PBRS_INTEGRATOR_DIRECT, false, PBRS_SHADE_FOURIER_ALONE)                                                                           \
                                                                                                                   \
    X(PBRS_INTEGRATOR_MATERIALS, false, 0u)                                                                                              \
    X(PBRS_INTEGRATOR_NORMALS, false, 0u)

struct TraversalKey {
    uint32_t key = 0;
    size_t lds = 0;
};
struct ShadeKey {
    uint32_t integ = 0;
    bool tex = false;
    uint32_t spec = 0;
    size_t lds = 0;
    uint32_t range = 0;
};
struct IntegratorChoice {
    enum Order { NO_ORDER, CLASS_SORT, CLASS_MAJOR } order = NO_ORDER;
    uint32_t last_class = 0;
    uint32_t n_shade = 0;
    ShadeKey shade[2];
};
struct KernelChoice {
    TraversalKey extend[2];
    TraversalKey shadow[2];
    bool wide_shadow = false;
    TraversalKey shadow_slow;
    bool split_queue = false;
    uint32_t lds_staging = 0;
    IntegratorChoice integ[PBRS_INTEGRATOR_NORMALS + 1];
};

KernelChoice choose_kernels(const SceneFacts& f, const DevOverrides& dev);

}
```

pbrs_amd/csrc/host/pass_plan.cpp:

```cpp
#include "pass_plan.h"

namespace pbrs {

PathLayout path_layout(size_t n_slots) {
    PathLayout l{};
    size_t at = 0;
    for (uint32_t i = 0; i < N_PATH_COLUMNS; ++i) {
        const PathColumnRow& r = kPathColumns[i];
        const size_t part = (r.per_slot * n_slots + r.per_tile * path_tiles(n_slots) + r.fixed) * r.elem / r.parts;
        l.offset[i] = at;
        l.bytes[i] = r.parts * ((part + kPathAlign - 1) / kPathAlign * kPathAlign);
        at += l.bytes[i];
    }
    l.total = at;
    return l;
}

uint32_t samples_per_pass(uint64_t tile_pixels, uint64_t spp, uint32_t requested, bool with_direct, uint64_t held_slots, uint64_t held_direct_bytes,
                          std::optional<uint64_t> free_bytes) {
    const uint64_t P = tile_pixels;
    uint64_t k = requested;
    if (k == 0) {
        uint64_t target = 240ull << 20;
        if (free_bytes) {
            const uint64_t per_path = kPathBytesPerSlot + (with_direct ? 16u : 0u);
            const uint64_t held_direct = with_direct ? held_direct_bytes : 0u;
            const uint64_t fit = (*free_bytes + held_slots * kPathBytesPerSlot + held_direct) / 4 / per_path;
            if (fit < target) target = fit < (4ull << 20) ? (4ull << 20) : fit;
        }
        k = P >= target ? 1 : target / P;
        if (k < 1) k = 1;
        if (k < spp) {
            const uint64_t passes = (spp + k - 1) / k;
            k = (spp + passes - 1) / passes;
        }
    }
    if (k > spp) k = spp;
    if (k < 1) k = 1;
    return (uint32_t)k;
}

uint32_t bounce_count(uint32_t integrator, uint32_t max_depth) {
    if (integrator == PBRS_INTEGRATOR_DIRECT) return max_depth ? 2u : 0u;
    if (integrator >= PBRS_INTEGRATOR_MATERIALS) return 1u;
    return max_depth;
}

PassShape pass_shape(uint32_t P, uint32_t kc) {
    PassShape s{};
    s.n_slots = P * kc;
    s.grid = (s.n_slots + kBlock - 1) / kBlock;
    s.sgrid = s.grid < kStreamGridCap ? s.grid : kStreamGridCap;
    s.pgrid = s.grid < kPersistentBlocks ? s.grid : kPersistentBlocks;
    s.slow_grid = s.pgrid < kSlowGrid ? s.pgrid : kSlowGrid;
    s.n_tiles = (s.n_slots + PBRS_SORT_TILE - 1) / PBRS_SORT_TILE;
    return s;
}

BouncePlan bounce_plan(uint32_t integrator, bool split_queue, const IntegratorChoice& ic, int split_decision, uint32_t bounce) {
    BouncePlan b{};
    const bool split = integrator == PBRS_INTEGRATOR_PATH && split_queue && split_decision != 2;
    b.split = split ? (PBRS_QSPLIT_ON | (bounce == 0 ? PBRS_QSPLIT_ENV : 0u)) : 0u;
    b.order = split ? IntegratorChoice::CLASS_MAJOR : ic.order;
    b.n_classes = split ? 2u : PBRS_MAX_CLASSES;
    b.last = split ? 1u : ic.last_class;
    b.zero_dropped = (split && bounce == 0) ? 1u : 0u;
    b.sorted = b.order != IntegratorChoice::NO_ORDER ? 1u : 0u;
    for (uint32_t k = 0; k < ic.n_shade; ++k) b.shade_range[k] = ic.shade[k].range ? ic.shade[k].range : split ? 1u : 0u;
    return b;
}

}
```

pbrs_amd/csrc/host/pass_plan.h:

```cpp
#pragma once
#include <cstddef>
#include <cstdint>
#include <optional>

#include "arg_checks.h"
#include "kernel_choice.h"

namespace pbrs {

enum PathColumn : uint32_t {
    COL_Q,
    COL_HIT = COL_Q + 6,
    COL_L,
    COL_NEE,
    COL_SR = COL_NEE + 3,
    COL_OCC = COL_SR + 3,
    COL_NEEQ,
    COL_PERM,
    COL_CLS,
    COL_SLOW,
    COL_TILE_HIST,
    COL_CLASS_RANGE,
    COL_RNG_HI0,
    N_PATH_COLUMNS
};
struct PathColumnRow {
    const char* name;
    uint32_t elem, per_slot, per_tile, fixed, parts;
};
constexpr size_t kPathAlign = 256;
constexpr PathColumnRow kPathColumns[N_PATH_COLUMNS] = {
    {"q[0][0]", 16, 1, 0, 0, 1}, {"q[0][1]", 16, 1, 0, 0, 1}, {"q[0][2]", 16, 1, 0, 0, 1},
    {"q[1][0]", 16, 1, 0, 0, 1}, {"q[1][1]", 16, 1, 0, 0, 1}, {"q[1][2]", 16, 1, 0, 0, 1},
    {"hit", 16, 1, 0, 0, 1},
    {"L", 16, 1, 0, 0, 1},
    {"nee[0]", 16, 1, 0, 0, 1}, {"nee[1]", 16, 1, 0, 0, 1}, {"nee[2]", 16, 1, 0, 0, 1},
    {"sr[0]", 16, 2, 0, 0, 2}, {"sr[1]", 16, 2, 0, 0, 2}, {"sr[2]", 16, 2, 0, 0, 2},
    {"occ", 1, 2, 0, 0, 1},
    {"nee queue", 4, 1, 0, 0, 1},
    {"perm", 4, 1, 0, 0, 1},
    {"cls", 1, 1, 0, 0, 1},
    {"slow", 4, 2, 0, 0, 1},
    {"tile_hist", 4, 0, PBRS_MAX_CLASSES, 0, 1},
    {"class_range", 8, 0, 0, PBRS_MAX_CLASSES + 1, 1},
    {"rng_hi0", 4, 1, 0, 0, 1},
};
constexpr uint64_t path_bytes_per_slot() {
    uint64_t b = 0;
    for (const PathColumnRow& r : kPathColumns) b += (uint64_t)r.elem * r.per_slot;
    return b;
}
constexpr uint64_t kPathBytesPerSlot = path_bytes_per_slot();
static_assert(kPathBytesPerSlot == 295, "a column changed: every automatic pass size moves with it");

constexpr size_t path_tiles(size_t n_slots) { return n_slots / PBRS_SORT_TILE + 1; }

struct PathLayout {
    size_t offset[N_PATH_COLUMNS];
    size_t bytes[N_PATH_COLUMNS];
    size_t total;
};
PathLayout path_layout(size_t n_slots);

constexpr uint32_t kHeadWords = PBRS_WORK_HEADS * PBRS_WORK_HEAD_STRIDE;
struct CounterLayout {
    uint32_t act, ns, slows, xhead, shead, shead2;
    uint32_t words;
};
constexpr CounterLayout counter_layout(uint32_t max_depth, uint32_t head_words) {
    const uint32_t stride = max_depth + 2;
    CounterLayout l{};
    l.act = 0;
    l.ns = l.act + stride;
    l.slows = l.ns + 2 * stride;
    l.xhead = l.slows + stride;
    l.shead = l.xhead + stride * head_words;
    l.shead2 = l.shead + stride * head_words;
    l.words = l.shead2 + stride * head_words;
    return l;
}
constexpr CounterLayout kCounters = counter_layout(kMaxDepth, kHeadWords);
static_assert(kCounters.ns % 2 == 0, "ns is read as 64-bit words");

uint32_t samples_per_pass(uint64_t tile_pixels, uint64_t spp, uint32_t requested, bool with_direct, uint64_t held_slots, uint64_t held_direct_bytes,
                          std::optional<uint64_t> free_bytes);

uint32_t bounce_count(uint32_t integrator, uint32_t max_depth);

constexpr uint32_t kStreamGridCap = 4096;
constexpr uint32_t kPersistentBlocks = PBRS_PERSISTENT_BLOCKS;
constexpr uint32_t kSlowGrid = 64;
struct PassShape {
    uint32_t n_slots;
    uint32_t grid;
    uint32_t sgrid;
    uint32_t pgrid;
    uint32_t slow_grid;
    uint32_t n_tiles;
};
PassShape pass_shape(uint32_t P, uint32_t kc);

struct BouncePlan {
    uint32_t split;
    IntegratorChoice::Order order;
    uint32_t n_classes;
    uint32_t last;
    uint32_t zero_dropped;
    uint32_t sorted;
    uint32_t shade_range[2];
};
BouncePlan bounce_plan(uint32_t integrator, bool split_queue, const IntegratorChoice& ic, int split_decision, uint32_t bounce);

}
```

pbrs_amd/csrc/kernel_tables.h:

```cpp
#pragma once
#include <cstdint>

#include "device/path_state.h"
#include "host/kernel_choice.h"

#pragma GCC visibility push(hidden)
namespace pbrs {

typedef void (*extend_fn_t)(DevScene, PathState, uint32_t, const uint32_t*, uint32_t, uint32_t*, GlobalCounters*, const uint32_t*, uint32_t*, uint32_t*, uint32_t);
typedef void (*shadow_fn_t)(DevScene, PathState, const uint32_t*, uint32_t*, GlobalCounters*, const uint32_t*, uint32_t*, uint32_t*);
typedef void (*shade_fn_t)(DevScene, PathState, RenderConst, uint32_t, const uint32_t*, uint32_t, uint32_t*, uint32_t*, unsigned long long*, uint32_t, const uint2*,
                           const uint32_t*);
typedef void (*intersect_fn_t)(DevScene, uint32_t, const float4*, const float4*, const float*, pbrs_hit_record*, uint8_t*, uint32_t*);

const extend_fn_t* extend_fns();
const shadow_fn_t* shadow_fns();
intersect_fn_t intersect_fn(bool wide_any);

shade_fn_t shade_fn(const ShadeKey& key);

}
#pragma GCC visibility pop
```

pbrs_amd/csrc/pbrs_gpu.hip:

```cpp
#include <hip/hip_runtime.h>

#include <algorithm>
#include <cmath>
#include <cstdio>
#include <cstdlib>
#include <cstring>
#include <utility>
#include <mutex>
#include <optional>
#include <string>
#include <vector>

#include "../../include/pbrs_gpu.h"
#include "device/raygen.h"
#include "device/class_sort.h"
#include "device/accumulate.h"
#include "device/dev_kernels.h"
#include "kernel_tables.h"
#include "host/scene_prepare.h"
#include "host/arg_checks.h"
#include "host/pass_plan.h"
#include "device/aov.h"
#include "device/film.h"
#include "device/denoise.h"
#include "device/moments.h"
#include "device/matte.h"
#include "device/passes.h"
#include "device/temporal.h"
#include "device/spatial_variance.h"
#include "device/display.h"
#include "device/upsample.h"

using namespace pbrs;

namespace {

#ifndef PBRS_SPLIT_KEEP_PERCENT
#define PBRS_SPLIT_KEEP_PERCENT 85u
#endif

struct StageEvent {
    int stage;
    hipEvent_t a, b;
};

#ifdef PBRS_DEV_OVERRIDES
const char* dev_env(const char* name) { return std::getenv(name); }

DevOverrides read_dev_overrides() {
    DevOverrides o;
    auto flag = [](const char* name, bool& v) {
        if (const char* e = dev_env(name)) v = std::atoi(e) != 0;
    };
    flag("PBRS_OVERLAP_PASSES", o.overlap_passes);
    flag("PBRS_SORT_CLASSES", o.sort_classes);
    flag("PBRS_SPLIT_LAMBERT", o.split_lambert);
    flag("PBRS_SPLIT_FOURIER", o.split_fourier);
    flag("PBRS_SPLIT_QUEUE", o.split_queue);
    flag("PBRS_LDS_SCENE", o.lds_scene);
    flag("PBRS_LDS_TOP", o.lds_top);
    flag("PBRS_RAYGEN_TILES8", o.raygen_tiles8);
    if (const char* e = dev_env("PBRS_WIDE")) o.wide_shadow = (std::atoi(e) & 2) != 0;
    if (const char* e = dev_env("PBRS_SHADE_SPEC")) o.shade_spec = (uint32_t)std::atoi(e);
    if (const char* e = dev_env("PBRS_SHADE_LDS")) o.shade_lds = (uint32_t)std::atoi(e);
    if (const char* e = dev_env("PBRS_LONG_WALKS")) o.long_walks = std::atoi(e) != 0;
    if (const char* e = dev_env("PBRS_FULL_STEPS")) o.full_steps = std::atoi(e) != 0;
    if (const char* e = dev_env("PBRS_OVERLAP_FROM")) o.overlap_from = (uint32_t)std::atoi(e);
    if (const char* e = dev_env("PBRS_REFILL_BELOW")) o.refill_below = (uint32_t)std::atoi(e);
    if (const char* e = dev_env("PBRS_RAYGEN_CHUNK")) {
        const long v = std::atol(e);
        o.raygen_chunk = v > 0 ? (uint32_t)v : 0xffffffffu;
    }
    if (const char* e = dev_env("PBRS_LDS_MIN")) o.lds_min = (size_t)std::atol(e);
    return o;
}
#endif

struct IntegratorPlan {
    IntegratorChoice choice;
    shade_fn_t shade[2] = {};
};
struct KernelPlan {
    KernelChoice choice;
    extend_fn_t extend[2] = {};
    shadow_fn_t shadow[2] = {};
    shadow_fn_t shadow_slow = nullptr;
    IntegratorPlan integ[PBRS_INTEGRATOR_NORMALS + 1];
};
uint32_t reported_features(const TraversalKey& k) { return (k.key & ~kStatsKey) | ((k.key & kStatsKey) ? 0x80000000u : 0u); }

struct DeviceBuffer {
    void* p = nullptr;
    size_t cap_bytes = 0;
    int grow(pbrs_ctx* c, size_t bytes, const char* what);
    template <class T>
    T* as() const { return static_cast<T*>(p); }
};
enum BufferId {
    BUF_AOV_STATE, BUF_AOV_OUT,
    BUF_FILTER_SUM,
    BUF_DENOISE, BUF_DENOISE_VAR, BUF_DENOISE_STAGE, BUF_DENOISE_VAR_STAGE,
    BUF_MOMENT_STATE, BUF_VARIANCE_OUT,
    BUF_MATTE_STATE, BUF_MATTE_OUT, BUF_MATTE_SELECT,
    BUF_PASS_STATE, BUF_PASS_OUT, BUF_PASS_DIRECT, BUF_PASS_DIRECT_SET1,
    BUF_TEMPORAL_STAGE,
    BUF_MOTION_TABLE, BUF_MOTION_STAGE,
    BUF_SPATIAL_STAGE,
    BUF_DISPLAY, BUF_DISPLAY_STAGE,
    BUF_UPSAMPLE_STAGE,
    N_BUFFERS
};

}

struct pbrs_ctx {
    int device = 0;
    hipStream_t own_stream = nullptr;
    hipStream_t stream = nullptr;
    std::string error;

    bool has_scene = false;
    std::vector<void*> scene_allocs;
    DevScene S{};
    uint32_t stack_depth = 0;

    struct PassSet {
        void* state_mem = nullptr;
        size_t cap_slots = 0;
        PathState st{};
        uint32_t* neeq = nullptr;
        uint32_t* rng_hi0 = nullptr;
        uint32_t* slow = nullptr;
        uint32_t* counters = nullptr;
        float4* direct = nullptr;
        hipEvent_t accumulated = nullptr;
        hipEvent_t late = nullptr;
        bool in_flight = false;
    } pass_set[2];
    int cur_set = 0;
    hipStream_t main_stream = nullptr;
    hipStream_t second_stream = nullptr;
    bool overlap_passes = true;
    uint32_t overlap_from = 2;
    size_t cap_pixels = 0;
    float* sum = nullptr;
    float* rgb_dev = nullptr;
    GlobalCounters* gcnt = nullptr;
    unsigned long long* nonfinite = nullptr;
    unsigned long long* bounce_acc = nullptr;

    std::vector<StageEvent> events;
    size_t events_used = 0;
    std::vector<hipEvent_t> total_ev;
    pbrs_stats pending{};
    bool pending_counters = false, pending_times = false;
    DevOverrides dev;
    KernelPlan plan;
    int split_decision = 0;
    unsigned long long* split_host = nullptr;
    hipEvent_t split_ev = nullptr;
    bool split_probe_in_flight = false;
    bool has_vis_records = false;
    uint64_t pending_closest = 0;
    pbrs_intersect_info last_intersect{};
    DeviceBuffer buf[N_BUFFERS];
};

namespace {

#define HIPCHK(ctx, expr)                                                                             \
    do {                                                                                              \
        hipError_t e_ = (expr);                                                                       \
        if (e_ != hipSuccess) {                                                                       \
            (ctx)->error = std::string(#expr) + ": " + hipGetErrorString(e_);                         \
            (void)hipGetLastError();  \
            return PBRS_E_DEVICE;                                                                     \
        }                                                                                             \
    } while (0)

struct CallAllocs {
    std::vector<void*> held;
    CallAllocs() = default;
    CallAllocs(const CallAllocs&) = delete;
    CallAllocs& operator=(const CallAllocs&) = delete;
    ~CallAllocs() {
        for (void* p : held) (void)hipFree(p);
    }
    template <class T>
    hipError_t alloc(T** p, size_t bytes) {
        void* q = nullptr;
        const hipError_t e = hipMalloc(&q, bytes);
        if (e == hipSuccess) held.push_back(q);
        *p = static_cast<T*>(q);
        return e;
    }
};

int fail(pbrs_ctx* c, int code, const char* msg) {
    c->error = msg;
    return code;
}
int fail(pbrs_ctx* c, const Refusal& r) { return r.code ? fail(c, r.code, r.message) : PBRS_OK; }

int enter(pbrs_ctx* c, const Refusal& r) {
    if (!c) return PBRS_E_INVALID;
    if (r.code) return fail(c, r);
    HIPCHK(c, hipSetDevice(c->device));
    return PBRS_OK;
}

template <class T>
int upload(pbrs_ctx* c, const T* src, size_t n, const T** dst) {
    *dst = nullptr;
    size_t bytes = (n ? n : 1) * sizeof(T);
    void* p = nullptr;
    HIPCHK(c, hipMalloc(&p, bytes));
    c->scene_allocs.push_back(p);
    if (n) HIPCHK(c, hipMemcpy(p, src, n * sizeof(T), hipMemcpyHostToDevice));
    *dst = static_cast<const T*>(p);
    return PBRS_OK;
}

void free_scene(pbrs_ctx* c) {
    for (void* p : c->scene_allocs) (void)hipFree(p);
    c->scene_allocs.clear();
    c->has_scene = false;
}

pbrs_ctx::PassSet& cur(pbrs_ctx* c) { return c->pass_set[c->cur_set]; }

void use_pass_set(pbrs_ctx* c, int k) {
    c->cur_set = k;
    c->stream = c->main_stream;
}

void free_paths(pbrs_ctx::PassSet& set) {
    set.cap_slots = 0;
// ... 73 lines not shown
}

int DeviceBuffer::grow(pbrs_ctx* c, size_t bytes, const char* what) {
    if (bytes <= cap_bytes) return PBRS_OK;
    cap_bytes = 0;
    if (p) (void)hipFree(p);
    p = nullptr;
    hipError_t e = hipMalloc(&p, bytes);
    if (e != hipSuccess) {
        p = nullptr;
        c->error = std::string("hipMalloc of ") + what + " (" + std::to_string(bytes >> 20) + " MiB): " + hipGetErrorString(e);
        (void)hipGetLastError();
        return PBRS_E_DEVICE;
    }
    cap_bytes = bytes;
    return PBRS_OK;
}

int ensure_direct(pbrs_ctx* c, int k, size_t n_slots, bool wanted) {
    c->pass_set[k].direct = nullptr;
    if (!wanted) return PBRS_OK;
    DeviceBuffer& b = c->buf[BUF_PASS_DIRECT + k];
    const int rc = b.grow(c, n_slots * sizeof(float4), "the light passes' path column");
    if (rc) return rc;
    c->pass_set[k].direct = b.as<float4>();
    return PBRS_OK;
}

struct Staged {
    const void* up;
    size_t words;
    void* down = nullptr;
    void* dev = nullptr;
    size_t pixels = 0;
    size_t count(size_t P) const { return words * (pixels ? pixels : P); }
    template <class T>
    T* as() const { return static_cast<T*>(dev); }
};

template <size_t N>
int stage(pbrs_ctx* c, BufferId id, const char* what, Staged (&s)[N], size_t P) {
    size_t words = 0;
    for (const Staged& r : s) words += r.count(P);
    DeviceBuffer& buf = c->buf[id];
    int rc = buf.grow(c, words * sizeof(uint32_t), what);
    if (rc) return rc;
    uint32_t* at = buf.as<uint32_t>();
    for (Staged& r : s) {
        r.dev = (r.up || r.down) ? at : nullptr;
        at += r.count(P);
    }
    return PBRS_OK;
}

template <size_t N>
int copy_staged(pbrs_ctx* c, const Staged (&s)[N], size_t P, hipMemcpyKind kind) {
    for (const Staged& r : s) {
        const bool up = kind == hipMemcpyHostToDevice;
        if (!(up ? r.up != nullptr : r.down != nullptr)) continue;
        HIPCHK(c, hipMemcpyAsync(up ? r.dev : r.down, up ? r.up : r.dev, r.count(P) * sizeof(uint32_t), kind, c->stream));
    }
    return PBRS_OK;
}

template <size_t N, class Launch>
int run_staged(pbrs_ctx* c, BufferId id, const char* what, Staged (&s)[N], size_t P, Launch launch) {
    int rc = stage(c, id, what, s, P);
    if (!rc) rc = copy_staged(c, s, P, hipMemcpyHostToDevice);
    if (!rc) rc = launch();
    if (!rc) rc = copy_staged(c, s, P, hipMemcpyDeviceToHost);
    if (rc) return rc;
    HIPCHK(c, hipStreamSynchronize(c->stream));
    return PBRS_OK;
}

constexpr size_t kDenoiseBytesPerPixel = 3 * sizeof(float4) + sizeof(uint32_t);

struct RenderTargets {
    float* rgb = nullptr;
    pbrs_aov_buffers aovs{};
    float* variance = nullptr;
    bool want_matte = false;
    const pbrs_matte_params* matte = nullptr;
    pbrs_matte_buffers matte_out{};
    pbrs_pass_buffers passes{};
    const FilterConst* filt = nullptr;

    bool want_aovs() const {
        const pbrs_aov_buffers& a = aovs;
        return a.albedo || a.normal || a.coverage || a.depth || a.instance || a.material || a.prim;
    }
    bool want_passes() const { return passes.direct || passes.indirect || passes.direct_variance || passes.indirect_variance; }
    WantedOutputs wanted() const { return {want_aovs(), variance != nullptr, want_passes(), want_matte, matte, matte_out.ids && matte_out.coverage}; }
};

SceneState scene_state(const pbrs_ctx* c) { return {c->has_scene, c->has_vis_records}; }

int pass_size(pbrs_ctx* c, const pbrs_render_params* p, uint32_t& K, bool with_direct = false) {
    std::optional<uint64_t> free_bytes;
    size_t free_b = 0, total_b = 0;
    if (p->samples_per_pass == 0 && hipMemGetInfo(&free_b, &total_b) == hipSuccess) free_bytes = free_b;
    K = samples_per_pass((uint64_t)p->w * p->h, (uint64_t)p->strata_x * p->strata_y, p->samples_per_pass, with_direct,
                         (uint64_t)c->pass_set[0].cap_slots + c->pass_set[1].cap_slots,
                         (uint64_t)c->buf[BUF_PASS_DIRECT].cap_bytes + c->buf[BUF_PASS_DIRECT_SET1].cap_bytes, free_bytes);
    if ((uint64_t)p->w * p->h * K >= (1ull << 28)) return fail(c, PBRS_E_LIMIT, "tile x samples_per_pass above 2^28 paths");
    return PBRS_OK;
}

struct Timer {
    pbrs_ctx* c;
    bool on;
    int begin(int stage) {
        if (!on) return 0;
        if (c->events_used == c->events.size()) {
            StageEvent e{};
            if (hipEventCreate(&e.a) != hipSuccess || hipEventCreate(&e.b) != hipSuccess) return -1;
            c->events.push_back(e);
        }
        StageEvent& e = c->events[c->events_used];
        e.stage = stage;
        return hipEventRecord(e.a, c->stream) == hipSuccess ? 0 : -1;
    }
    int end() {
        if (!on) return 0;
        StageEvent& e = c->events[c->events_used++];
        return hipEventRecord(e.b, c->stream) == hipSuccess ? 0 : -1;
    }
};

RenderConst make_const(const pbrs_ctx* c, const pbrs_camera* cam, const pbrs_render_params* p) {
    RenderConst rc{};
    rc.cam = *cam;
    rc.x0 = p->x0; rc.y0 = p->y0; rc.w = p->w; rc.h = p->h;
    rc.strata_x = p->strata_x; rc.strata_y = p->strata_y;
    rc.max_depth = p->max_depth;
    rc.n_pixels = p->w * p->h;
    rc.band_rows = p->band_rows; rc.band_count = p->band_count; rc.band_index = p->band_index;
    rc.seed = p->seed;
    rc.integrator = p->integrator;
    rc.chunk_pixels = c->dev.raygen_chunk.value_or(4096u);
    if (rc.chunk_pixels > rc.n_pixels) rc.chunk_pixels = rc.n_pixels;
    rc.tiles8_per_row = (c->dev.raygen_tiles8 && p->w % 8u == 0u && p->h % 8u == 0u) ? p->w / 8u : 0u;
    return rc;
}

bool bind_kernels(const KernelChoice& ch, KernelPlan& p) {
    p = KernelPlan{};
    p.choice = ch;
    for (int s = 0; s < 2; ++s) {
        p.extend[s] = extend_fns()[ch.extend[s].key];
        p.shadow[s] = shadow_fns()[ch.shadow[s].key];
    }
    if (ch.wide_shadow) p.shadow_slow = shadow_fns()[ch.shadow_slow.key];
    bool ok = p.extend[0] && p.extend[1] && p.shadow[0] && p.shadow[1] && (!ch.wide_shadow || p.shadow_slow);
    for (uint32_t i = 0; i <= PBRS_INTEGRATOR_NORMALS; ++i) {
        IntegratorPlan& ip = p.integ[i];
        ip.choice = ch.integ[i];
        for (uint32_t k = 0; k < ip.choice.n_shade; ++k) {
            ip.shade[k] = shade_fn(ip.choice.shade[k]);
            ok = ok && ip.shade[k];
        }
    }
    return ok;
}

void poll_split_probe(pbrs_ctx* c) {
    if (!c->split_probe_in_flight || hipEventQuery(c->split_ev) != hipSuccess) {
        (void)hipGetLastError();
        return;
    }
    c->split_probe_in_flight = false;
    c->split_decision = (c->split_host[0] * 100ull <= c->split_host[1] * PBRS_SPLIT_KEEP_PERCENT) ? 1 : 2;
}

struct MatteKernels {
    void (*fold)(const pbrs_instance*, PathState, uint32_t*, uint32_t, uint32_t, uint32_t, uint32_t, uint32_t);
    void (*finalize)(const uint32_t*, uint32_t, uint32_t, uint32_t, float, uint32_t*, float*, float*);
};
#define PBRS_MATTE_KERNELS(N) {k_matte<N>, k_matte_finalize<N>}
constexpr MatteKernels kMatte[PBRS_MATTE_MAX_SLOTS] = {PBRS_MATTE_KERNELS(1), PBRS_MATTE_KERNELS(2), PBRS_MATTE_KERNELS(3), PBRS_MATTE_KERNELS(4),
                                                       PBRS_MATTE_KERNELS(5), PBRS_MATTE_KERNELS(6), PBRS_MATTE_KERNELS(7), PBRS_MATTE_KERNELS(8)};
#undef PBRS_MATTE_KERNELS

int run_pass(pbrs_ctx* c, RenderConst rc, uint32_t first, uint32_t kc, bool stats, Timer& tm, bool handoff, const RenderTargets& t) {
    pbrs_ctx::PassSet& set = cur(c);
    if (handoff && set.in_flight) HIPCHK(c, hipStreamWaitEvent(c->stream, set.accumulated, 0));
    auto to_late_stream = [&]() -> hipError_t {
        hipError_t e = hipEventRecord(set.late, c->stream);
        c->stream = c->second_stream;
        return e != hipSuccess ? e : hipStreamWaitEvent(c->stream, set.late, 0);
    };
    const uint32_t P = rc.n_pixels;
    const PassShape shape = pass_shape(P, kc);
    const uint32_t N = shape.n_slots, grid = shape.grid, pgrid = shape.pgrid, n_tiles = shape.n_tiles;
    rc.pass_first_sample = first;
    rc.n_slots = N;
    uint32_t* act = set.counters + kCounters.act;
    unsigned long long* ns = reinterpret_cast<unsigned long long*>(set.counters + kCounters.ns);
    uint32_t* slows = set.counters + kCounters.slows;
    uint32_t* xhead = set.counters + kCounters.xhead;
    uint32_t* shead = set.counters + kCounters.shead;
    uint32_t* shead2 = set.counters + kCounters.shead2;
    uint32_t* neeq = set.neeq;
    const KernelPlan& plan = c->plan;
    const KernelChoice& choice = plan.choice;
    const IntegratorPlan& ip = plan.integ[rc.integrator];
    const TraversalKey &xk = choice.extend[stats], &sk = choice.shadow[stats];
    DevScene xS = c->S;
    if (!(xS.features & PBRS_FEAT_FLAT_TLAS)) xS.n_flat = 0u;
    HIPCHK(c, hipMemsetAsync(set.counters, 0, kCounters.words * sizeof(uint32_t), c->stream));
    if (tm.begin(0)) return fail(c, PBRS_E_DEVICE, "event record failed");
    hipLaunchKernelGGL(k_raygen, dim3(grid), dim3(kBlock), 0, c->stream, set.st, rc, set.rng_hi0);
    tm.end();
    poll_split_probe(c);
    const uint32_t n_bounces = bounce_count(rc.integrator, rc.max_depth);
    if (n_bounces == 0) HIPCHK(c, hipMemsetAsync(set.st.L, 0, (size_t)N * sizeof(float4), c->stream));
    const bool probe_split = c->split_decision == 0 && !c->split_probe_in_flight && rc.integrator == PBRS_INTEGRATOR_PATH && choice.split_queue && n_bounces > 0;
    for (uint32_t b = 0; b < n_bounces; ++b) {
        if (handoff && b == c->overlap_from) HIPCHK(c, to_late_stream());
        const uint32_t* cnt_in = b == 0 ? nullptr : act + b;
        const BouncePlan bp = bounce_plan(rc.integrator, choice.split_queue, ip.choice, c->split_decision, b);
        const uint32_t qsplit = bp.split;
        if (tm.begin(1)) return fail(c, PBRS_E_DEVICE, "event record failed");
        hipLaunchKernelGGL(plan.extend[stats], dim3(pgrid), dim3(kBlock), xk.lds, c->stream, xS, set.st, b & 1u, cnt_in, N, xhead + b * kHeadWords, c->gcnt, nullptr,
                           nullptr, nullptr, qsplit);
        c->pending.kernel_features_extend = reported_features(xk);
        tm.end();
        if (b == 0 && t.want_aovs())
            hipLaunchKernelGGL(k_aov, dim3((P + kBlock - 1) / kBlock), dim3(kBlock), 0, c->stream, c->S, set.st, c->buf[BUF_AOV_STATE].as<float>(), P, kc,
                               rc.chunk_pixels, qsplit);
        if (b == 0 && t.want_matte)
            hipLaunchKernelGGL(kMatte[t.matte->slots - 1u].fold, dim3((P + kBlock - 1) / kBlock), dim3(kBlock), 0, c->stream, c->S.inst, set.st,
                               c->buf[BUF_MATTE_STATE].as<uint32_t>(), P, kc, rc.chunk_pixels, qsplit, t.matte->key);
        if (tm.begin(2)) return fail(c, PBRS_E_DEVICE, "event record failed");
        if (bp.order == IntegratorChoice::CLASS_MAJOR) {
            const bool two = bp.n_classes == 2u;
            if (two) hipLaunchKernelGGL(k_class_count<2u>, dim3(n_tiles), dim3(kBlock), 0, c->stream, set.st, cnt_in, N);
            else hipLaunchKernelGGL(k_class_count<PBRS_MAX_CLASSES>, dim3(n_tiles), dim3(kBlock), 0, c->stream, set.st, cnt_in, N);
            hipLaunchKernelGGL(k_class_scan, dim3(1), dim3(64 * PBRS_MAX_CLASSES), 0, c->stream, set.st, cnt_in, N, bp.last,
                               (qsplit && probe_split) ? c->bounce_acc + 2 * PBRS_STATS_MAX_BOUNCES : nullptr);
            if (two) hipLaunchKernelGGL(k_class_scatter<2u>, dim3(n_tiles), dim3(kBlock), 0, c->stream, set.st, cnt_in, N, bp.zero_dropped);
            else hipLaunchKernelGGL(k_class_scatter<PBRS_MAX_CLASSES>, dim3(n_tiles), dim3(kBlock), 0, c->stream, set.st, cnt_in, N, bp.zero_dropped);
        } else if (bp.order == IntegratorChoice::CLASS_SORT) {
            hipLaunchKernelGGL(k_class_sort, dim3(n_tiles), dim3(kBlock), 0, c->stream, set.st, cnt_in, N);
        }
        for (uint32_t k = 0; k < ip.choice.n_shade; ++k) {
            const uint2* range = bp.shade_range[k] ? set.st.class_range + bp.shade_range[k] : nullptr;
            hipLaunchKernelGGL(ip.shade[k], dim3(grid), dim3(kBlock), ip.choice.shade[k].lds, c->stream, c->S, set.st, rc, b, cnt_in, N, act + b + 1, neeq, ns + b,
                               bp.sorted, range, set.rng_hi0);
        }
        tm.end();
        if (tm.begin(3)) return fail(c, PBRS_E_DEVICE, "event record failed");
        hipLaunchKernelGGL(plan.shadow[stats], dim3(pgrid), dim3(kBlock), sk.lds, c->stream, c->S, set.st, reinterpret_cast<const uint32_t*>(ns + b),
                           shead + b * kHeadWords, c->gcnt + 1, nullptr, set.slow, slows + b);
        c->pending.kernel_features_shadow = reported_features(sk);
        if (choice.wide_shadow && !stats)
            hipLaunchKernelGGL(plan.shadow_slow, dim3(shape.slow_grid), dim3(kBlock), choice.shadow_slow.lds, c->stream, c->S, set.st, slows + b, shead2 + b * kHeadWords,
                               c->gcnt + 1, set.slow, nullptr, nullptr);
        hipLaunchKernelGGL(k_nee_resolve, dim3(shape.sgrid), dim3(kBlock), 0, c->stream, set.st, neeq, reinterpret_cast<const uint32_t*>(ns + b));
        tm.end();
        if (b == 0 && t.want_passes()) hipLaunchKernelGGL(k_pass_direct, dim3(grid), dim3(kBlock), 0, c->stream, set.st.L, set.direct, N);
    }
    if (probe_split) {
        unsigned long long* acc = c->bounce_acc + 2 * PBRS_STATS_MAX_BOUNCES;
        HIPCHK(c, hipMemcpyAsync(c->split_host, acc, 2 * sizeof(unsigned long long), hipMemcpyDeviceToHost, c->stream));
        HIPCHK(c, hipEventRecord(c->split_ev, c->stream));
        HIPCHK(c, hipMemsetAsync(acc, 0, 2 * sizeof(unsigned long long), c->stream));
        c->split_probe_in_flight = true;
    }
    if (stats)
        hipLaunchKernelGGL(k_sum_bounce_counts, dim3(1), dim3(64), 0, c->stream, act, ns, N, n_bounces, c->bounce_acc);
    if (handoff && c->stream != c->second_stream) HIPCHK(c, to_late_stream());
    if (tm.begin(4)) return fail(c, PBRS_E_DEVICE, "event record failed");
    if (const FilterConst* filt = t.filt)
        hipLaunchKernelGGL(k_filter_accumulate, dim3((filt->w + PBRS_FILTER_CELL - 1) / PBRS_FILTER_CELL, (filt->h + PBRS_FILTER_CELL - 1) / PBRS_FILTER_CELL),
                           dim3(kBlock), filter_lds_bytes(filt->hx, filt->hy), c->stream, set.st, c->buf[BUF_FILTER_SUM].as<float>(), rc, *filt, kc, c->nonfinite);
    else
        hipLaunchKernelGGL(k_accumulate, dim3((P + kBlock - 1) / kBlock), dim3(kBlock), 0, c->stream, set.st, c->sum, P, kc, rc.chunk_pixels, rc.w, rc.tiles8_per_row, c->nonfinite);
    if (t.variance)
        hipLaunchKernelGGL(k_moments, dim3((P + kBlock - 1) / kBlock), dim3(kBlock), 0, c->stream, set.st, c->buf[BUF_MOMENT_STATE].as<float>(), P, kc, rc.chunk_pixels);
    if (t.want_passes())
        hipLaunchKernelGGL(k_pass_fold, dim3((P + kBlock - 1) / kBlock), dim3(kBlock), 0, c->stream, set.st.L, set.direct,
                           c->buf[BUF_PASS_STATE].as<float>(), P, kc, rc.chunk_pixels);
    tm.end();
    if (handoff) {
        HIPCHK(c, hipEventRecord(set.accumulated, c->stream));
        set.in_flight = true;
    }
    HIPCHK(c, hipGetLastError());
    return PBRS_OK;
}

int render_common(pbrs_ctx* c, const pbrs_camera* cam, const pbrs_render_params* p, uint32_t K, const RenderTargets& t) {
    const uint32_t P = p->w * p->h;
    const uint32_t spp = p->strata_x * p->strata_y;
    const FilterConst* filt = t.filt;
    float* aov = t.want_aovs() ? c->buf[BUF_AOV_STATE].as<float>() : nullptr;
    float* moments = t.variance ? c->buf[BUF_MOMENT_STATE].as<float>() : nullptr;
    uint32_t* matte = t.want_matte ? c->buf[BUF_MATTE_STATE].as<uint32_t>() : nullptr;
    float* pass_state = t.want_passes() ? c->buf[BUF_PASS_STATE].as<float>() : nullptr;
    float* filter_sum = c->buf[BUF_FILTER_SUM].as<float>();
    RenderConst rc = make_const(c, cam, p);
    const bool stats = p->collect_counters != 0;
    Timer tm{c, p->time_stages != 0};
    c->events_used = 0;
    c->pending = pbrs_stats{};
    c->pending_counters = stats;
    c->pending_times = p->time_stages != 0;
    c->pending.samples = (uint64_t)P * spp;
    if (stats) HIPCHK(c, hipMemsetAsync(c->gcnt, 0, 2 * sizeof(GlobalCounters), c->stream));
    if (stats) HIPCHK(c, hipMemsetAsync(c->bounce_acc, 0, 2 * PBRS_STATS_MAX_BOUNCES * sizeof(unsigned long long), c->stream));
    HIPCHK(c, hipMemsetAsync(c->nonfinite, 0, sizeof(unsigned long long), c->stream));
    if (c->pending_times) HIPCHK(c, hipEventRecord(c->total_ev[0], c->stream));
    if (filt) HIPCHK(c, hipMemsetAsync(filter_sum, 0, 4 * (size_t)filt->w * filt->h * sizeof(float), c->stream));
    else HIPCHK(c, hipMemsetAsync(c->sum, 0, 3 * (size_t)P * sizeof(float), c->stream));
    if (aov) HIPCHK(c, hipMemsetAsync(aov, 0, PBRS_AOV_STATE_WORDS * (size_t)P * sizeof(float), c->stream));
    if (moments) HIPCHK(c, hipMemsetAsync(moments, 0, PBRS_MOMENT_STATE_WORDS * (size_t)P * sizeof(float), c->stream));
    if (matte) HIPCHK(c, hipMemsetAsync(matte, 0, PBRS_MATTE_STATE_WORDS(t.matte->slots) * (size_t)P * sizeof(uint32_t), c->stream));
    if (pass_state) HIPCHK(c, hipMemsetAsync(pass_state, 0, PBRS_PASS_STATE_WORDS * (size_t)P * sizeof(float), c->stream));
    uint32_t passes = 0;
    bool two = c->overlap_passes && !stats && spp > K;
    if (two && (ensure_work(c, c->pass_set[1], (size_t)P * K, P) || ensure_direct(c, 1, (size_t)P * K, pass_state != nullptr))) {
        two = false;
        c->error.clear();
    }
    for (uint32_t first = 0; first < spp; first += K) {
        uint32_t kc = spp - first < K ? spp - first : K;
        if (two) use_pass_set(c, (int)(passes & 1u));
        const int rcode = run_pass(c, rc, first, kc, stats, tm, two, t);
        if (rcode) {
            use_pass_set(c, 0);
            return rcode;
        }
        ++passes;
    }
    if (two) {
        const hipEvent_t last = cur(c).accumulated;
        use_pass_set(c, 0);
        HIPCHK(c, hipStreamWaitEvent(c->main_stream, last, 0));
    }
    if (filt) {
        const uint32_t PT = filt->w * filt->h;
        hipLaunchKernelGGL(k_filter_finalize, dim3((PT + kBlock - 1) / kBlock), dim3(kBlock), 0, c->stream, filter_sum, t.rgb, PT);
    } else {
        hipLaunchKernelGGL(k_finalize, dim3((P + kBlock - 1) / kBlock), dim3(kBlock), 0, c->stream, c->sum, t.rgb, P, 1.0f / (float)spp);
    }
    if (aov)
        hipLaunchKernelGGL(k_aov_finalize, dim3((P + kBlock - 1) / kBlock), dim3(kBlock), 0, c->stream, aov, c->S.inst, P, rc.w, rc.tiles8_per_row,
                           1.0f / (float)spp, t.aovs);
    if (moments)
        hipLaunchKernelGGL(k_moments_finalize, dim3((P + kBlock - 1) / kBlock), dim3(kBlock), 0, c->stream, moments, P, rc.w, rc.tiles8_per_row, t.variance);
    if (matte)
        hipLaunchKernelGGL(kMatte[t.matte->slots - 1u].finalize, dim3((P + kBlock - 1) / kBlock), dim3(kBlock), 0, c->stream, matte, P, rc.w,
                           rc.tiles8_per_row, 1.0f / (float)spp, t.matte_out.ids, t.matte_out.coverage, t.matte_out.residual);
    if (pass_state)
        hipLaunchKernelGGL(k_pass_finalize, dim3((P + kBlock - 1) / kBlock), dim3(kBlock), 0, c->stream, pass_state, P, rc.w, rc.tiles8_per_row,
                           1.0f / (float)spp, t.passes);
    if (c->pending_times) HIPCHK(c, hipEventRecord(c->total_ev[1], c->stream));
    HIPCHK(c, hipGetLastError());
    c->pending.passes = passes;
    c->pending.launches_extend = c->pending.launches_shade = c->pending.launches_shadow = passes * bounce_count(rc.integrator, rc.max_depth);
    return PBRS_OK;
}

int collect(pbrs_ctx* c, pbrs_stats* out) {
    HIPCHK(c, hipStreamSynchronize(c->stream));
    pbrs_stats s = c->pending;
    {
        unsigned long long bad = 0;
        HIPCHK(c, hipMemcpy(&bad, c->nonfinite, sizeof bad, hipMemcpyDeviceToHost));
        s.invalid_samples = bad;
    }
    if (c->pending_counters) {
        GlobalCounters g[2];
        HIPCHK(c, hipMemcpy(g, c->gcnt, sizeof g, hipMemcpyDeviceToHost));
        s.closest_rays = g[0].rays;
        s.shade_events = g[0].hits;
        s.tlas_nodes = g[0].tlas_nodes; s.blas_nodes = g[0].blas_nodes; s.instances = g[0].instances;
        s.instance_hits = g[0].instance_hits; s.triangles = g[0].triangles; s.tri_shading = g[0].tri_shading;
        s.spheres = g[0].spheres; s.quads = g[0].quads; s.cuboids = g[0].cuboids; s.disks = g[0].disks;
        s.shadow_rays = g[1].rays;
        s.shadow_tlas_nodes = g[1].tlas_nodes; s.shadow_blas_nodes = g[1].blas_nodes; s.shadow_instances = g[1].instances;
        s.shadow_triangles = g[1].triangles;
        s.shadow_prims = g[1].spheres + g[1].quads + g[1].cuboids + g[1].disks;
        unsigned long long per_bounce[2 * PBRS_STATS_MAX_BOUNCES];
        HIPCHK(c, hipMemcpy(per_bounce, c->bounce_acc, sizeof per_bounce, hipMemcpyDeviceToHost));
        for (uint32_t b = 0; b < PBRS_STATS_MAX_BOUNCES; ++b) {
            s.paths_at_bounce[b] = per_bounce[b];
            s.shadow_rays_at_bounce[b] = per_bounce[PBRS_STATS_MAX_BOUNCES + b];
        }
    }
    if (c->pending_times) {
        float* acc[5] = {&s.ms_raygen, &s.ms_extend, &s.ms_shade, &s.ms_shadow, &s.ms_accumulate};
        for (size_t i = 0; i < c->events_used; ++i) {
            float ms = 0.0f;
            HIPCHK(c, hipEventElapsedTime(&ms, c->events[i].a, c->events[i].b));
            *acc[c->events[i].stage] += ms;
        }
        HIPCHK(c, hipEventElapsedTime(&s.ms_total, c->total_ev[0], c->total_ev[1]));
    }
    if (out) *out = s;
    return PBRS_OK;
}

std::mutex g_kernel_cfg_mutex;
bool g_kernel_cfg_done[64] = {};
int configure_kernels(pbrs_ctx* c) {
    std::lock_guard<std::mutex> lock(g_kernel_cfg_mutex);
    if (c->device < 64 && g_kernel_cfg_done[c->device]) return PBRS_OK;
    const int cap = (int)(kLdsBytesPerCU / 2);
    std::vector<const void*> traversal_kernels = {reinterpret_cast<const void*>(intersect_fn(false)), reinterpret_cast<const void*>(intersect_fn(true))};
    for (uint32_t k = 0; k < kTraversalKeys; ++k) {
        if (extend_fns()[k]) traversal_kernels.push_back(reinterpret_cast<const void*>(extend_fns()[k]));
        if (shadow_fns()[k]) traversal_kernels.push_back(reinterpret_cast<const void*>(shadow_fns()[k]));
    }
    for (const void* k : traversal_kernels) HIPCHK(c, hipFuncSetAttribute(k, hipFuncAttributeMaxDynamicSharedMemorySize, cap));
    if (c->device < 64) g_kernel_cfg_done[c->device] = true;
    return PBRS_OK;
}

int filter_setup(pbrs_ctx* c, const pbrs_camera* cam, const pbrs_render_params* p, const pbrs_pixel_filter* f, FilterConst& fc, pbrs_render_params& region) {
    const int rc = fail(c, check_filter(p, f));
    if (rc) return rc;
    fc = FilterConst{};
    fc.kind = f->kind;
    fc.rx = f->radius[0], fc.ry = f->radius[1], fc.a = f->a, fc.b = f->b;
    fc.hx = pf_halo(fc.rx), fc.hy = pf_halo(fc.ry);
    fc.x0 = p->x0, fc.y0 = p->y0, fc.w = p->w, fc.h = p->h;
    region = *p;
    region.x0 = p->x0 > fc.hx ? p->x0 - fc.hx : 0u;
    region.y0 = p->y0 > fc.hy ? p->y0 - fc.hy : 0u;
    region.w = std::min(p->x0 + p->w + fc.hx, cam->width) - region.x0;
    region.h = std::min(p->y0 + p->h + fc.hy, cam->height) - region.y0;
    return fail(c, check_params(scene_state(c), cam, &region));
}

int render(pbrs_ctx* c, const pbrs_camera* cam, const pbrs_render_params* p, const pbrs_pixel_filter* filter, RenderTargets t, bool host, pbrs_stats* stats_out) {
    HIPCHK(c, hipSetDevice(c->device));
    FilterConst fc;
    pbrs_render_params region;
    int rc = fail(c, check_params(scene_state(c), cam, p));
    if (rc) return rc;
    const size_t PT = (size_t)p->w * p->h;
    if (filter) {
        if ((rc = filter_setup(c, cam, p, filter, fc, region))) return rc;
        t.filt = &fc;
        p = &region;
    }
    if ((rc = fail(c, check_targets(p, t.wanted())))) return rc;
    const size_t P = (size_t)p->w * p->h;
    const pbrs_aov_buffers& a = t.aovs;
    Staged aovs[] = {{nullptr, 3, a.albedo}, {nullptr, 3, a.normal}, {nullptr, 1, a.coverage}, {nullptr, 1, a.depth}, {nullptr, 1, a.instance},
                     {nullptr, 1, a.material}, {nullptr, 1, a.prim}};
    Staged variance[] = {{nullptr, 1, t.variance}};
    const size_t slots = t.want_matte ? t.matte->slots : 0;
    Staged matte[] = {{nullptr, slots, t.matte_out.ids}, {nullptr, slots, t.matte_out.coverage}, {nullptr, 1, t.matte_out.residual}};
    Staged passes[] = {{nullptr, 3, t.passes.direct}, {nullptr, 3, t.passes.indirect}, {nullptr, 1, t.passes.direct_variance},
                       {nullptr, 1, t.passes.indirect_variance}};
    float* const rgb_host = t.rgb;
    if (t.filt) rc = c->buf[BUF_FILTER_SUM].grow(c, 4 * PT * sizeof(float), "the filter sums");
    if (t.want_aovs()) {
        if (!rc) rc = c->buf[BUF_AOV_STATE].grow(c, PBRS_AOV_STATE_WORDS * P * sizeof(float), "the AOV state");
        if (!rc && host) rc = stage(c, BUF_AOV_OUT, "the AOV buffers", aovs, P);
    }
    if (t.variance) {
        if (!rc) rc = c->buf[BUF_MOMENT_STATE].grow(c, PBRS_MOMENT_STATE_WORDS * P * sizeof(float), "the variance AOV's moments");
        if (!rc && host) rc = stage(c, BUF_VARIANCE_OUT, "the variance buffer", variance, P);
    }
    if (t.want_matte) {
        if (!rc) rc = c->buf[BUF_MATTE_STATE].grow(c, PBRS_MATTE_STATE_WORDS(slots) * P * sizeof(uint32_t), "the matte state");
        if (!rc && host) rc = stage(c, BUF_MATTE_OUT, "the matte buffers", matte, P);
    }
    if (t.want_passes()) {
        if (!rc) rc = c->buf[BUF_PASS_STATE].grow(c, PBRS_PASS_STATE_WORDS * P * sizeof(float), "the light passes' state");
        if (!rc && host) rc = stage(c, BUF_PASS_OUT, "the light pass buffers", passes, P);
    }
    uint32_t K = 0;
    if (!rc) rc = pass_size(c, p, K, t.want_passes());
    if (!rc) rc = ensure_work(c, cur(c), P * K, P);
    if (!rc) rc = ensure_direct(c, c->cur_set, P * K, t.want_passes());
    if (rc) return rc;
    if (host) {
        t.rgb = c->rgb_dev;
        t.aovs = {aovs[0].as<float>(), aovs[1].as<float>(), aovs[2].as<float>(), aovs[3].as<float>(), aovs[4].as<uint32_t>(), aovs[5].as<uint32_t>(), aovs[6].as<uint32_t>()};
        t.variance = variance[0].as<float>();
        t.matte_out = {matte[0].as<uint32_t>(), matte[1].as<float>(), matte[2].as<float>()};
        t.passes = {passes[0].as<float>(), passes[1].as<float>(), passes[2].as<float>(), passes[3].as<float>()};
    }
    rc = render_common(c, cam, p, K, t);
    if (rc) return rc;
    if (!host) return stats_out ? collect(c, stats_out) : PBRS_OK;
    HIPCHK(c, hipMemcpyAsync(rgb_host, t.rgb, 3 * PT * sizeof(float), hipMemcpyDeviceToHost, c->stream));
    if ((rc = copy_staged(c, variance, P, hipMemcpyDeviceToHost))) return rc;
    if ((rc = copy_staged(c, aovs, P, hipMemcpyDeviceToHost))) return rc;
    if ((rc = copy_staged(c, matte, P, hipMemcpyDeviceToHost))) return rc;
    if ((rc = copy_staged(c, passes, P, hipMemcpyDeviceToHost))) return rc;
    return collect(c, stats_out);
}

RenderTargets make_targets(float* rgb, const pbrs_aov_buffers* aovs, float* variance, const pbrs_matte_params* params, const pbrs_matte_buffers* matte,
                           const pbrs_pass_buffers* passes) {
    RenderTargets t;
    t.rgb = rgb;
    if (aovs) t.aovs = *aovs;
    t.variance = variance;
    t.want_matte = matte != nullptr;
    t.matte = params;
    if (matte) t.matte_out = *matte;
    if (passes) t.passes = *passes;
    return t;
}

}

extern "C" {

int pbrs_create(int device_ordinal, pbrs_ctx** out) {
    if (!out) return PBRS_E_INVALID;
    *out = nullptr;
    int n = 0;
    if (hipGetDeviceCount(&n) != hipSuccess || n <= 0 || device_ordinal < 0 || device_ordinal >= n) return PBRS_E_DEVICE;
    pbrs_ctx* c = new pbrs_ctx();
    c->device = device_ordinal;
    bool ok = hipSetDevice(device_ordinal) == hipSuccess && hipStreamCreateWithFlags(&c->own_stream, hipStreamNonBlocking) == hipSuccess;
    c->stream = c->main_stream = c->own_stream;
    {
        int least = 0, greatest = 0;
        ok = ok && hipDeviceGetStreamPriorityRange(&least, &greatest) == hipSuccess &&
             hipStreamCreateWithPriority(&c->second_stream, hipStreamNonBlocking, greatest) == hipSuccess;
    }
    ok = ok && hipEventCreateWithFlags(&c->pass_set[0].accumulated, hipEventDisableTiming) == hipSuccess &&
         hipEventCreateWithFlags(&c->pass_set[1].accumulated, hipEventDisableTiming) == hipSuccess &&
         hipEventCreateWithFlags(&c->pass_set[0].late, hipEventDisableTiming) == hipSuccess &&
         hipEventCreateWithFlags(&c->pass_set[1].late, hipEventDisableTiming) == hipSuccess;
#ifdef PBRS_DEV_OVERRIDES
    c->dev = read_dev_overrides();
#endif
    c->overlap_passes = c->dev.overlap_passes;
    for (int k = 0; ok && k < 2; ++k) {
        hipEvent_t ev = nullptr;
        ok = hipEventCreate(&ev) == hipSuccess;
        if (ok) c->total_ev.push_back(ev);
    }
    for (pbrs_ctx::PassSet& set : c->pass_set) ok = ok && hipMalloc(reinterpret_cast<void**>(&set.counters), kCounters.words * sizeof(uint32_t)) == hipSuccess;
    ok = ok && hipMalloc(reinterpret_cast<void**>(&c->gcnt), 2 * sizeof(GlobalCounters)) == hipSuccess &&
         hipMalloc(reinterpret_cast<void**>(&c->nonfinite), sizeof(unsigned long long)) == hipSuccess &&
         hipMalloc(reinterpret_cast<void**>(&c->bounce_acc), (2 * PBRS_STATS_MAX_BOUNCES + 2) * sizeof(unsigned long long)) == hipSuccess &&
         hipMemset(c->bounce_acc, 0, (2 * PBRS_STATS_MAX_BOUNCES + 2) * sizeof(unsigned long long)) == hipSuccess &&
         hipMemset(c->nonfinite, 0, sizeof(unsigned long long)) == hipSuccess &&
         hipHostMalloc(reinterpret_cast<void**>(&c->split_host), 2 * sizeof(unsigned long long), hipHostMallocDefault) == hipSuccess &&
         hipEventCreateWithFlags(&c->split_ev, hipEventDisableTiming) == hipSuccess;
    ok = ok && configure_kernels(c) == PBRS_OK;
    if (!ok) {
        pbrs_destroy(c);
        return PBRS_E_DEVICE;
    }
    *out = c;
    return PBRS_OK;
}

void pbrs_destroy(pbrs_ctx* c) {
    if (!c) return;
    (void)hipSetDevice(c->device);
    if (c->stream) (void)hipStreamSynchronize(c->stream);
    if (c->second_stream) (void)hipStreamSynchronize(c->second_stream);
    free_scene(c);
    free_work(c);
    for (DeviceBuffer& b : c->buf)
// ... 538 lines not shown
int pbrs_spatial_variance(pbrs_ctx* c, const pbrs_spatial_variance_params* p, const float* moments_host, const float* length_host,
                          const pbrs_spatial_variance_guides* guides_host, const float* variance_in_host, float* variance_out_host) {
    const int rc = enter(c, check_spatial_variance(p, moments_host, length_host, guides_host, variance_in_host, variance_out_host));
    if (rc) return rc;
    const size_t P = (size_t)p->w * p->h;
    const pbrs_spatial_variance_guides g = guides_host ? *guides_host : pbrs_spatial_variance_guides{};
    Staged s[] = {{moments_host, 2}, {length_host, 1}, {g.depth, 1}, {g.normal, 3}, {g.instance, 1}, {variance_in_host, 1, variance_out_host}};
    return run_staged(c, BUF_SPATIAL_STAGE, "the spatial variance estimate's staging", s, P, [&] {
        const pbrs_spatial_variance_guides gd{s[2].as<float>(), s[3].as<float>(), s[4].as<uint32_t>()};
        return spatial_variance_launch(c, *p, s[0].as<float>(), s[1].as<float>(), gd, s[5].as<float>(), s[5].as<float>());
    });
}

static_assert(sizeof(pbrs_display_params) == 64, "pbrs_display_params is 64 B");
static_assert(PBRS_DISPLAY_BINS == 512u && PBRS_DISPLAY_BINS % 64u == 0, "k_display_resolve holds the bins in one wave, eight per lane");

namespace {

using DisplayApplyKernel = void (*)(const float*, uint32_t*, DisplayApply);
#define PBRS_DISPLAY_ROW(C) {{k_display_apply<C, PBRS_ENCODE_SQRT, false>, k_display_apply<C, PBRS_ENCODE_SQRT, true>}, \
                             {k_display_apply<C, PBRS_ENCODE_SRGB, false>, k_display_apply<C, PBRS_ENCODE_SRGB, true>}}
constexpr DisplayApplyKernel kDisplayApply[3][2][2] = {PBRS_DISPLAY_ROW(PBRS_CURVE_NONE), PBRS_DISPLAY_ROW(PBRS_CURVE_REINHARD), PBRS_DISPLAY_ROW(PBRS_CURVE_ACES)};
#undef PBRS_DISPLAY_ROW

uint32_t display_grid(uint32_t work, uint32_t cap = kDisplayMaxBlocks) { return std::min((work + kDisplayBlock - 1) / kDisplayBlock, cap); }

int display_launch(pbrs_ctx* c, const pbrs_display_params& p, const float* rgb, const pbrs_display_io& io, uint32_t* out, bool histogram) {
    const uint32_t P = p.w * p.h;
    const bool auto_exposure = (p.flags & PBRS_DISPLAY_AUTO_EXPOSURE) != 0;
    DisplayApply a{};
    a.w = p.w, a.P = P;
    a.scale = p.exposure;
    a.iw2 = 1.0f / (p.white * p.white);
    a.d = p.quantize == PBRS_QUANT_ROUND ? 0.5f : 0.0f;
    a.dither = p.quantize == PBRS_QUANT_DITHER;
    a.exposure_out = io.exposure_out;
    if (auto_exposure || histogram) {
        uint32_t* scratch = c->buf[BUF_DISPLAY].as<uint32_t>();
        HIPCHK(c, hipMemsetAsync(scratch, 0, PBRS_DISPLAY_BINS * sizeof(uint32_t), c->stream));
        const bool rgb_aligned = (reinterpret_cast<uintptr_t>(rgb) & 15u) == 0;
        hipLaunchKernelGGL(rgb_aligned ? k_display_hist<true> : k_display_hist<false>, dim3(display_grid((P + 3u) / 4u, kDisplayHistMaxBlocks)),
                           dim3(kDisplayBlock), 0, c->stream, rgb, P, scratch);
        HIPCHK(c, hipGetLastError());
        float* scale_word = reinterpret_cast<float*>(scratch + kDisplayScaleWord);
        const DisplayResolve r{auto_exposure ? 1u : 0u, p.exposure, p.key, p.min_exposure, p.max_exposure, p.adapt, p.low_q16, p.high_q16,
                               auto_exposure ? io.exposure_in : nullptr, io.exposure_out, io.histogram_out};
        hipLaunchKernelGGL(k_display_resolve, dim3(1), dim3(64), 0, c->stream, scratch, scale_word, r);
        HIPCHK(c, hipGetLastError());
        a.scale_word = scale_word;
        a.exposure_out = nullptr;
    }
    const bool aligned = ((reinterpret_cast<uintptr_t>(rgb) | reinterpret_cast<uintptr_t>(out)) & 15u) == 0;
    hipLaunchKernelGGL(kDisplayApply[p.curve][p.encode][aligned], dim3(display_grid((P + 3u) / 4u)), dim3(kDisplayBlock), 0, c->stream, rgb, out, a);
    HIPCHK(c, hipGetLastError());
    return PBRS_OK;
}

int display_scratch(pbrs_ctx* c, bool needed) {
    return needed ? c->buf[BUF_DISPLAY].grow(c, kDisplayScratchWords * sizeof(uint32_t), "the display transform's histogram") : PBRS_OK;
}

}

int pbrs_display_device(pbrs_ctx* c, const pbrs_display_params* p, const float* rgb_device, const pbrs_display_io* io_device, uint32_t* rgba8_out_device) {
    int rc = enter(c, check_display(p, rgb_device, io_device, rgba8_out_device));
    if (rc) return rc;
    const pbrs_display_io io = io_device ? *io_device : pbrs_display_io{};
    if ((rc = display_scratch(c, (p->flags & PBRS_DISPLAY_AUTO_EXPOSURE) || io.histogram_out))) return rc;
    return display_launch(c, *p, rgb_device, io, rgba8_out_device, io.histogram_out != nullptr);
}

int pbrs_display(pbrs_ctx* c, const pbrs_display_params* p, const float* rgb_host, const pbrs_display_io* io_host, uint32_t* rgba8_out_host) {
    int rc = enter(c, check_display(p, rgb_host, io_host, rgba8_out_host));
    if (rc) return rc;
    const pbrs_display_io io = io_host ? *io_host : pbrs_display_io{};
    const bool auto_exposure = (p->flags & PBRS_DISPLAY_AUTO_EXPOSURE) != 0;
    if ((rc = display_scratch(c, auto_exposure || io.histogram_out || io.exposure_out))) return rc;
    const size_t P = (size_t)p->w * p->h;
    Staged s[] = {{rgb_host, 3}, {nullptr, 1, rgba8_out_host}};
    return run_staged(c, BUF_DISPLAY_STAGE, "the display transform's staging", s, P, [&] {
        uint32_t* scratch = c->buf[BUF_DISPLAY].as<uint32_t>();
        pbrs_display_io iod{};
        if (auto_exposure && io.exposure_in) {
            iod.exposure_in = reinterpret_cast<const float*>(scratch + kDisplayPrevWord);
            HIPCHK(c, hipMemcpyAsync(scratch + kDisplayPrevWord, io.exposure_in, sizeof(float), hipMemcpyHostToDevice, c->stream));
        }
        if (io.exposure_out) iod.exposure_out = reinterpret_cast<float*>(scratch + kDisplayExposureWord);
        const int lrc = display_launch(c, *p, s[0].as<float>(), iod, s[1].as<uint32_t>(), io.histogram_out != nullptr);
        if (lrc) return lrc;
        if (io.exposure_out) HIPCHK(c, hipMemcpyAsync(io.exposure_out, scratch + kDisplayExposureWord, sizeof(float), hipMemcpyDeviceToHost, c->stream));
        if (io.histogram_out) HIPCHK(c, hipMemcpyAsync(io.histogram_out, scratch, PBRS_DISPLAY_BINS * sizeof(uint32_t), hipMemcpyDeviceToHost, c->stream));
        return (int)PBRS_OK;
    });
}

static_assert(sizeof(pbrs_upsample_params) == 48, "pbrs_upsample_params is 48 B");
static_assert(PBRS_UPSAMPLE_MIN_FACTOR == 2u && PBRS_UPSAMPLE_MAX_FACTOR == 4u && PBRS_UPSAMPLE_MAX_RADIUS == 2u, "kUpsample holds every factor and radius");

namespace {

using UpsampleKernel = void (*)(UpsampleIn, float*, float*, UpsampleConst);
#define PBRS_UPSAMPLE_ROW(F) {{k_upsample<F, 1u, false>, k_upsample<F, 1u, true>}, {k_upsample<F, 2u, false>, k_upsample<F, 2u, true>}}
constexpr UpsampleKernel kUpsample[3][2][2] = {PBRS_UPSAMPLE_ROW(2u), PBRS_UPSAMPLE_ROW(3u), PBRS_UPSAMPLE_ROW(4u)};
#undef PBRS_UPSAMPLE_ROW

int upsample_launch(pbrs_ctx* c, const pbrs_upsample_params& p, const float* rgb_lo, const pbrs_denoise_guides& lo, const pbrs_denoise_guides& hi,
                    float* out, float* weight_out) {
    UpsampleConst k{};
    k.w = p.w, k.h = p.h;
    k.wl = (p.w + p.factor - 1) / p.factor, k.hl = (p.h + p.factor - 1) / p.factor;
    k.in = 1.0f / (p.sigma_normal * p.sigma_normal);
    k.id = 1.0f / (p.sigma_depth * p.sigma_depth);
    k.albedo_floor = p.albedo_floor, k.min_weight = p.min_weight;
    const bool demodulate = (p.flags & PBRS_UPSAMPLE_DEMODULATE) != 0, ids = (p.flags & PBRS_UPSAMPLE_ID_STOP) != 0;
    const UpsampleIn in{rgb_lo, demodulate ? lo.albedo : nullptr, lo.normal, lo.depth, ids ? lo.instance : nullptr,
                        demodulate ? hi.albedo : nullptr, hi.normal, hi.depth, ids ? hi.instance : nullptr};
    const dim3 grid((p.w + PBRS_DENOISE_CELL - 1) / PBRS_DENOISE_CELL, (p.h + PBRS_DENOISE_CELL - 1) / PBRS_DENOISE_CELL);
    hipLaunchKernelGGL(kUpsample[p.factor - 2u][p.radius - 1u][ids], grid, dim3(kBlock), 0, c->stream, in, out, weight_out, k);
    HIPCHK(c, hipGetLastError());
    return PBRS_OK;
}

}

int pbrs_upsample_device(pbrs_ctx* c, const pbrs_upsample_params* p, const float* rgb_lo_device, const pbrs_denoise_guides* guides_lo_device,
                         const pbrs_denoise_guides* guides_hi_device, float* out_device, float* weight_out_device) {
    const int rc = enter(c, check_upsample(p, rgb_lo_device, guides_lo_device, guides_hi_device, out_device, weight_out_device));
    if (rc) return rc;
    return upsample_launch(c, *p, rgb_lo_device, *guides_lo_device, *guides_hi_device, out_device, weight_out_device);
}

int pbrs_upsample(pbrs_ctx* c, const pbrs_upsample_params* p, const float* rgb_lo_host, const pbrs_denoise_guides* guides_lo_host,
                  const pbrs_denoise_guides* guides_hi_host, float* out_host, float* weight_out_host) {
    const int rc = enter(c, check_upsample(p, rgb_lo_host, guides_lo_host, guides_hi_host, out_host, weight_out_host));
    if (rc) return rc;
    const size_t P = (size_t)p->w * p->h;
    const size_t Pl = (size_t)((p->w + p->factor - 1) / p->factor) * ((p->h + p->factor - 1) / p->factor);
    const pbrs_denoise_guides &lo = *guides_lo_host, &hi = *guides_hi_host;
    Staged s[] = {{rgb_lo_host, 3, nullptr, nullptr, Pl}, {lo.albedo, 3, nullptr, nullptr, Pl}, {lo.normal, 3, nullptr, nullptr, Pl},
                  {lo.depth, 1, nullptr, nullptr, Pl},    {lo.instance, 1, nullptr, nullptr, Pl},
                  {hi.albedo, 3}, {hi.normal, 3}, {hi.depth, 1}, {hi.instance, 1}, {nullptr, 3, out_host}, {nullptr, 1, weight_out_host}};
    return run_staged(c, BUF_UPSAMPLE_STAGE, "the guided upsampling's staging", s, P, [&] {
        const pbrs_denoise_guides lod{s[1].as<float>(), s[2].as<float>(), s[3].as<float>(), s[4].as<uint32_t>()};
        const pbrs_denoise_guides hid{s[5].as<float>(), s[6].as<float>(), s[7].as<float>(), s[8].as<uint32_t>()};
        return upsample_launch(c, *p, s[0].as<float>(), lod, hid, s[9].as<float>(), s[10].as<float>());
    });
}

int pbrs_collect_stats(pbrs_ctx* c, pbrs_stats* stats_out) {
    if (!c) return PBRS_E_INVALID;
    return collect(c, stats_out);
}

int pbrs_intersect_rays(pbrs_ctx* c, uint32_t n, const float* origins, const float* dirs, const float* tmax, pbrs_hit_record* hits_out,
                        uint8_t* occluded_out) {
    if (!c) return PBRS_E_INVALID;
    if (!c->has_scene) return fail(c, PBRS_E_NO_SCENE, "no scene uploaded");
    if (n == 0) return PBRS_OK;
    if (!origins || !dirs || !tmax) return fail(c, PBRS_E_INVALID, "null ray arrays");
    HIPCHK(c, hipSetDevice(c->device));
    float4 *d_o = nullptr, *d_d = nullptr;
    float* d_t = nullptr;
    pbrs_hit_record* d_h = nullptr;
    uint8_t* d_occ = nullptr;
    uint32_t* d_info = nullptr;
    CallAllocs mem;
    std::vector<float4> h_o(n), h_d(n);
    for (uint32_t i = 0; i < n; ++i) {
        h_o[i] = make_float4(origins[3 * i], origins[3 * i + 1], origins[3 * i + 2], 0.0f);
        h_d[i] = make_float4(dirs[3 * i], dirs[3 * i + 1], dirs[3 * i + 2], 0.0f);
    }
    HIPCHK(c, mem.alloc(&d_o, (size_t)n * 16));
    HIPCHK(c, mem.alloc(&d_d, (size_t)n * 16));
    HIPCHK(c, mem.alloc(&d_t, (size_t)n * 4));
    if (hits_out) HIPCHK(c, mem.alloc(&d_h, (size_t)n * sizeof(pbrs_hit_record)));
    if (occluded_out) HIPCHK(c, mem.alloc(&d_occ, (size_t)n));
    HIPCHK(c, mem.alloc(&d_info, 2 * sizeof(uint32_t)));
    HIPCHK(c, hipMemsetAsync(d_info, 0, 2 * sizeof(uint32_t), c->stream));
    HIPCHK(c, hipMemcpyAsync(d_o, h_o.data(), (size_t)n * 16, hipMemcpyHostToDevice, c->stream));
    HIPCHK(c, hipMemcpyAsync(d_d, h_d.data(), (size_t)n * 16, hipMemcpyHostToDevice, c->stream));
    HIPCHK(c, hipMemcpyAsync(d_t, tmax, (size_t)n * 4, hipMemcpyHostToDevice, c->stream));
    {
        const uint32_t rows = std::max(c->stack_depth, c->S.wide_cap);
        const size_t lds = (size_t)(rows + c->S.n_flat) * kBlock * sizeof(uint32_t);
        const dim3 grid(std::min<uint32_t>((n + kBlock - 1) / kBlock, kPersistentBlocks));
        const bool wide = c->plan.choice.wide_shadow;
        c->last_intersect = pbrs_intersect_info{wide ? 1u : 0u, 0u, 0u, 0u};
        hipLaunchKernelGGL(intersect_fn(wide), grid, dim3(kBlock), lds, c->stream, c->S, n, d_o, d_d, d_t, d_h, d_occ, d_info);
    }
    HIPCHK(c, hipGetLastError());
    if (hits_out) HIPCHK(c, hipMemcpyAsync(hits_out, d_h, (size_t)n * sizeof(pbrs_hit_record), hipMemcpyDeviceToHost, c->stream));
    if (occluded_out) HIPCHK(c, hipMemcpyAsync(occluded_out, d_occ, (size_t)n, hipMemcpyDeviceToHost, c->stream));
    uint32_t slow[2] = {0u, 0u};
    HIPCHK(c, hipMemcpyAsync(slow, d_info, sizeof slow, hipMemcpyDeviceToHost, c->stream));
    HIPCHK(c, hipStreamSynchronize(c->stream));
    c->last_intersect.slow_any = slow[0];
    c->last_intersect.slow_closest = slow[1];
    return PBRS_OK;
}

int pbrs_last_intersect_info(const pbrs_ctx* c, pbrs_intersect_info* out) {
    if (!c || !out) return PBRS_E_INVALID;
    *out = c->last_intersect;
    return PBRS_OK;
}

int pbrs_camera_rays(pbrs_ctx* c, const pbrs_camera* cam, const pbrs_render_params* p, uint32_t sample_index, float* origins_out, float* dirs_out) {
    if (!c) return PBRS_E_INVALID;
    HIPCHK(c, hipSetDevice(c->device));
    int rc = fail(c, check_params(scene_state(c), cam, p));
    if (rc) return rc;
    if (!origins_out || !dirs_out) return fail(c, PBRS_E_INVALID, "null output");
    const uint32_t P = p->w * p->h;
    uint32_t K;
    if ((rc = pass_size(c, p, K))) return rc;
    rc = ensure_work(c, cur(c), P, P);
    if (rc) return rc;
    RenderConst k = make_const(c, cam, p);
    k.tiles8_per_row = 0u;
    k.pass_first_sample = sample_index;
    k.n_slots = P;
    hipLaunchKernelGGL(k_raygen, dim3((P + kBlock - 1) / kBlock), dim3(kBlock), 0, c->stream, cur(c).st, k, cur(c).rng_hi0);
    float *d_o = nullptr, *d_d = nullptr;
    CallAllocs mem;
    HIPCHK(c, mem.alloc(&d_o, (size_t)P * 12));
    HIPCHK(c, mem.alloc(&d_d, (size_t)P * 12));
    hipLaunchKernelGGL(k_export_rays, dim3((P + kBlock - 1) / kBlock), dim3(kBlock), 0, c->stream, cur(c).st, P, d_o, d_d);
    HIPCHK(c, hipGetLastError());
    HIPCHK(c, hipMemcpyAsync(origins_out, d_o, (size_t)P * 12, hipMemcpyDeviceToHost, c->stream));
    HIPCHK(c, hipMemcpyAsync(dirs_out, d_d, (size_t)P * 12, hipMemcpyDeviceToHost, c->stream));
    HIPCHK(c, hipStreamSynchronize(c->stream));
    return PBRS_OK;
}

int pbrs_numeric_eval(pbrs_ctx* c, uint32_t fn, uint32_t n, const float* x, const float* y, float* out) {
    if (!c) return PBRS_E_INVALID;
    if (n == 0) return PBRS_OK;
    if (!x || !out || fn > PN_PROBE_LAST) return fail(c, PBRS_E_INVALID, "bad numeric_eval arguments");
    HIPCHK(c, hipSetDevice(c->device));
    float *d_x = nullptr, *d_y = nullptr, *d_r = nullptr;
    CallAllocs mem;
    HIPCHK(c, mem.alloc(&d_x, (size_t)n * 4));
    HIPCHK(c, mem.alloc(&d_r, (size_t)n * 4));
    HIPCHK(c, hipMemcpyAsync(d_x, x, (size_t)n * 4, hipMemcpyHostToDevice, c->stream));
    if (y) {
        HIPCHK(c, mem.alloc(&d_y, (size_t)n * 4));
        HIPCHK(c, hipMemcpyAsync(d_y, y, (size_t)n * 4, hipMemcpyHostToDevice, c->stream));
    }
    hipLaunchKernelGGL(k_numeric_eval, dim3((n + kBlock - 1) / kBlock), dim3(kBlock), 0, c->stream, fn, n, d_x, d_y, d_r);
    HIPCHK(c, hipGetLastError());
    HIPCHK(c, hipMemcpyAsync(out, d_r, (size_t)n * 4, hipMemcpyDeviceToHost, c->stream));
    HIPCHK(c, hipStreamSynchronize(c->stream));
    return PBRS_OK;
}

int pbrs_numeric_eval_k(pbrs_ctx* c, uint32_t fn, uint32_t n, uint32_t k, const uint32_t* ops, uint32_t* out) {
    if (!c) return PBRS_E_INVALID;
    if (n == 0) return PBRS_OK;
    if (!ops || !out || fn > PN_PROBE_K_LAST || k > PN_PROBE_MAX_K || k < pn_probe_k_operands(fn))
        return fail(c, PBRS_E_INVALID, "bad numeric_eval_k arguments");
    HIPCHK(c, hipSetDevice(c->device));
    uint32_t *d_ops = nullptr, *d_r = nullptr;
    CallAllocs mem;
    HIPCHK(c, mem.alloc(&d_ops, (size_t)n * k * 4));
    HIPCHK(c, mem.alloc(&d_r, (size_t)n * 4));
    HIPCHK(c, hipMemcpyAsync(d_ops, ops, (size_t)n * k * 4, hipMemcpyHostToDevice, c->stream));
    hipLaunchKernelGGL(k_numeric_eval_k, dim3((n + kBlock - 1) / kBlock), dim3(kBlock), 0, c->stream, fn, n, k, d_ops, d_r);
    HIPCHK(c, hipGetLastError());
    HIPCHK(c, hipMemcpyAsync(out, d_r, (size_t)n * 4, hipMemcpyDeviceToHost, c->stream));
    HIPCHK(c, hipStreamSynchronize(c->stream));
    return PBRS_OK;
}

int pbrs_render_sample_radiance(pbrs_ctx* c, const pbrs_camera* cam, const pbrs_render_params* p, uint32_t sample_index, float* rgb_out_host) {
    if (!c) return PBRS_E_INVALID;
    HIPCHK(c, hipSetDevice(c->device));
    int rc = fail(c, check_params(scene_state(c), cam, p));
    if (rc) return rc;
    if (!rgb_out_host) return fail(c, PBRS_E_INVALID, "null output");
    const uint32_t P = p->w * p->h;
    uint32_t K;
    if ((rc = pass_size(c, p, K))) return rc;
    rc = ensure_work(c, cur(c), P, P);
    if (rc) return rc;
    RenderConst k = make_const(c, cam, p);
    k.tiles8_per_row = 0u;
    Timer tm{c, false};
    HIPCHK(c, hipMemsetAsync(c->sum, 0, 3 * (size_t)P * sizeof(float), c->stream));
    rc = run_pass(c, k, sample_index, 1, false, tm, false, RenderTargets{});
    if (rc) return rc;
    hipLaunchKernelGGL(k_export_radiance, dim3((P + kBlock - 1) / kBlock), dim3(kBlock), 0, c->stream, cur(c).st, P, c->rgb_dev);
    HIPCHK(c, hipGetLastError());
    HIPCHK(c, hipMemcpyAsync(rgb_out_host, c->rgb_dev, 3 * (size_t)P * sizeof(float), hipMemcpyDeviceToHost, c->stream));
    HIPCHK(c, hipStreamSynchronize(c->stream));
    return PBRS_OK;
}

}
```

pbrs_amd/csrc/traverse.hip:

```cpp
#include <hip/hip_runtime.h>

#include <utility>

#include "kernel_tables.h"

#ifdef PBRS_PROBE_TIME
__device__ unsigned long long g_trav_time[2][8];
#endif
#ifdef PBRS_PROBE_TRAV
__device__ unsigned long long g_trav_probe[2][24];
#endif
#define PBRS_TRAVERSAL_PROBES_DEFINED
#include "device/extend.h"
#include "device/intersect.h"
#include "device/shadow.h"

using namespace pbrs;

namespace {

template <uint32_t K>
constexpr extend_fn_t extend_fn_of() {
    if constexpr (extend_key_ok(K)) return &k_extend<(K & kStatsKey) != 0u, (K & ~kStatsKey)>;
    else return nullptr;
}
template <uint32_t K>
constexpr shadow_fn_t shadow_fn_of() {
    if constexpr (shadow_key_ok(K)) return &k_shadow<(K & kStatsKey) != 0u, (K & ~kStatsKey)>;
    else return nullptr;
}
template <uint32_t... K>
const extend_fn_t* extend_table(std::integer_sequence<uint32_t, K...>) {
    static const extend_fn_t t[sizeof...(K)] = {extend_fn_of<K>()...};
    return t;
}
template <uint32_t... K>
const shadow_fn_t* shadow_table(std::integer_sequence<uint32_t, K...>) {
    static const shadow_fn_t t[sizeof...(K)] = {shadow_fn_of<K>()...};
    return t;
}

}

namespace pbrs {

const extend_fn_t* extend_fns() { return extend_table(std::make_integer_sequence<uint32_t, kTraversalKeys>{}); }
const shadow_fn_t* shadow_fns() { return shadow_table(std::make_integer_sequence<uint32_t, kTraversalKeys>{}); }
intersect_fn_t intersect_fn(bool wide_any) { return wide_any ? &k_intersect_rays<true> : &k_intersect_rays<false>; }

}

extern "C" {

#ifdef PBRS_PROBE_TIME
int pbrs_debug_trav_time(unsigned long long* out16) {
    if (hipDeviceSynchronize() != hipSuccess) return -1;
    if (hipMemcpyFromSymbol(out16, HIP_SYMBOL(g_trav_time), 16 * sizeof(unsigned long long)) != hipSuccess) return -1;
    unsigned long long zero[16] = {0};
    return hipMemcpyToSymbol(HIP_SYMBOL(g_trav_time), zero, sizeof zero) == hipSuccess ? 0 : -1;
}
#endif
#ifdef PBRS_PROBE_TRAV
int pbrs_debug_trav_probe(unsigned long long* out48) {
    if (hipDeviceSynchronize() != hipSuccess) return -1;
    if (hipMemcpyFromSymbol(out48, HIP_SYMBOL(g_trav_probe), 48 * sizeof(unsigned long long)) != hipSuccess) return -1;
    unsigned long long zero[48] = {0};
    return hipMemcpyToSymbol(HIP_SYMBOL(g_trav_probe), zero, sizeof zero) == hipSuccess ? 0 : -1;
}
#endif

}
```

Baseline: 1678.

## Add wave-coherent packet traversal for primary camera rays with slow-path fallback

Adds a packet traversal kernel in which a whole wave walks the BLAS together, using a per-wave LDS stack of node and lane-mask pairs and scalar node loads, for the first bounce of camera rays. Rays the packet walk refuses are appended to a slow list and finished by the normal per-ray extend kernel. A new accumulation kernel stages per-sample radiance through LDS when the packet path is used. The aim is to cut divergent per-lane node fetches on coherent primary rays, at the cost of extra LDS use, a second launch and lower occupancy. A packet intersect API is also exposed.

```diff
diff --git a/include/pbrs_gpu.h b/include/pbrs_gpu.h
--- a/include/pbrs_gpu.h
+++ b/include/pbrs_gpu.h
@@ -285,6 +285,7 @@
     uint32_t slow_any, slow_closest;
 } pbrs_intersect_info;
 int pbrs_last_intersect_info(const pbrs_ctx*, pbrs_intersect_info* out);
+int pbrs_intersect_packets(pbrs_ctx*, uint32_t n, const float* origins, const float* dirs, const float* tmax, pbrs_hit_record* hits_out);
 int pbrs_camera_rays(pbrs_ctx*, const pbrs_camera*, const pbrs_render_params*, uint32_t sample_index, float* origins_out,
                      float* dirs_out);
 int pbrs_numeric_eval(pbrs_ctx*, uint32_t fn, uint32_t n, const float* x, const float* y, float* out);
diff --git a/pbrs_amd/api.py b/pbrs_amd/api.py
--- a/pbrs_amd/api.py
+++ b/pbrs_amd/api.py
@@ -429,7 +429,7 @@
 NUMERIC_K_FNS = {"mul_add": 0, "clamp": 1, "slab_filter": 2, "rng_init_lo": 3, "rng_init_hi": 4, "rng_stream_u32": 5, "rng_stream_f32": 6}
 
 GPU_SYMBOLS = ["pbrs_create", "pbrs_destroy", "pbrs_last_error", "pbrs_set_stream", "pbrs_set_pass_overlap", "pbrs_upload_scene", "pbrs_render_tile",
-               "pbrs_render_tile_device", "pbrs_collect_stats", "pbrs_intersect_rays", "pbrs_last_intersect_info", "pbrs_camera_rays",
+               "pbrs_render_tile_device", "pbrs_collect_stats", "pbrs_intersect_rays", "pbrs_intersect_packets", "pbrs_last_intersect_info", "pbrs_camera_rays",
                "pbrs_numeric_eval", "pbrs_numeric_eval_k", "pbrs_render_sample_radiance", "pbrs_render_tile_aovs", "pbrs_render_tile_aovs_device",
                "pbrs_render_tile_filtered", "pbrs_render_tile_filtered_device", "pbrs_denoise", "pbrs_denoise_device",
                "pbrs_render_tile_aovs_var", "pbrs_render_tile_aovs_var_device", "pbrs_denoise_var", "pbrs_denoise_var_device",
@@ -502,6 +502,7 @@
         L.pbrs_render_tile_device.argtypes = [C.c_void_p, C.c_void_p, C.c_void_p, C.c_void_p, C.c_void_p]
         L.pbrs_collect_stats.argtypes = [C.c_void_p, C.c_void_p]
         L.pbrs_intersect_rays.argtypes = [C.c_void_p, C.c_uint32] + [C.c_void_p] * 5
+        L.pbrs_intersect_packets.argtypes = [C.c_void_p, C.c_uint32] + [C.c_void_p] * 4
         L.pbrs_last_intersect_info.argtypes = [C.c_void_p, C.c_void_p]
         L.pbrs_camera_rays.argtypes = [C.c_void_p, C.c_void_p, C.c_void_p, C.c_uint32, C.c_void_p, C.c_void_p]
         L.pbrs_numeric_eval.argtypes = [C.c_void_p, C.c_uint32, C.c_uint32, C.c_void_p, C.c_void_p, C.c_void_p]
@@ -1439,6 +1440,15 @@
                     "pbrs_intersect_rays")
         return hits, occ
 
+    def intersect_packets(self, origins, dirs, tmax):
+        origins = np.ascontiguousarray(origins, dtype=np.float32)
+        dirs = np.ascontiguousarray(dirs, dtype=np.float32)
+        tmax = np.ascontiguousarray(tmax, dtype=np.float32)
+        n = len(tmax)
+        hits = np.empty(n, dtype=HIT_DTYPE)
+        self._check(self._L.pbrs_intersect_packets(self._h, n, origins.ctypes.data, dirs.ctypes.data, tmax.ctypes.data, hits.ctypes.data), "pbrs_intersect_packets")
+        return hits
+
     def last_intersect_info(self):
         v = (C.c_uint32 * 4)()
         self._check(self._L.pbrs_last_intersect_info(self._h, C.addressof(v)), "pbrs_last_intersect_info")
diff --git a/pbrs_amd/csrc/device/accumulate.h b/pbrs_amd/csrc/device/accumulate.h
--- a/pbrs_amd/csrc/device/accumulate.h
+++ b/pbrs_amd/csrc/device/accumulate.h
@@ -39,6 +39,49 @@
     sum[n_pixels + p] = s.y;
     sum[2 * n_pixels + p] = s.z;
 }
+#define PBRS_FOLD_TILE 8u
+#define PBRS_FOLD_ROW (3u * PBRS_FOLD_TILE + 1u)
+__global__ void __launch_bounds__(256) k_accumulate_pixels(PathState st, float* sum, uint32_t n_pixels, uint32_t k_count, uint32_t w, uint32_t tiles8_per_row,
+                                                            unsigned long long* nonfinite) {
+    __shared__ float tile[256u * PBRS_FOLD_ROW];
+    const uint32_t q0 = blockIdx.x * 256u, q = q0 + threadIdx.x;
+    const bool live = q < n_pixels;
+    const uint32_t p = live ? pixel_of_order(q, w, tiles8_per_row) : 0u;
+    f3 s = gray(0.0f);
+    if (live) s = mk3(sum[p], sum[n_pixels + p], sum[2 * n_pixels + p]);
+    uint32_t bad = 0;
+    for (uint32_t kt = 0; kt < k_count; kt += PBRS_FOLD_TILE) {
+        const uint32_t nk = k_count - kt < PBRS_FOLD_TILE ? k_count - kt : PBRS_FOLD_TILE;
+#pragma unroll
+        for (uint32_t it = 0; it < PBRS_FOLD_TILE; ++it) {
+            const uint32_t r = it * 256u + threadIdx.x, i = r / PBRS_FOLD_TILE, j = r % PBRS_FOLD_TILE;
+            if (q0 + i < n_pixels && j < nk) {
+                const float4 l = st.L[(q0 + i) * k_count + kt + j];
+                float* at = tile + i * PBRS_FOLD_ROW + 3u * j;
+                at[0] = l.x, at[1] = l.y, at[2] = l.z;
+            }
+        }
+        __syncthreads();
+        if (live) {
+            for (uint32_t j = 0; j < nk; ++j) {
+                const float* at = tile + threadIdx.x * PBRS_FOLD_ROW + 3u * j;
+                const f3 l = mk3(at[0], at[1], at[2]);
+                bad += (pn_isfinite(l.x) && pn_isfinite(l.y) && pn_isfinite(l.z)) ? 0u : 1u;
+                s = s + l;
+            }
+        }
+        __syncthreads();
+    }
+    if (__ballot(bad != 0u)) {
+        for (int off = 32; off > 0; off >>= 1) bad += __shfl_down(bad, off, 64);
+        if ((threadIdx.x & 63u) == 0) atomicAdd(nonfinite, (unsigned long long)bad);
+    }
+    if (live) {
+        sum[p] = s.x;
+        sum[n_pixels + p] = s.y;
+        sum[2 * n_pixels + p] = s.z;
+    }
+}
 __global__ void __launch_bounds__(256) k_finalize(const float* sum, float* rgb, uint32_t n_pixels, float inv_spp) {
     uint32_t p = blockIdx.x * blockDim.x + threadIdx.x;
     if (p >= n_pixels) return;
diff --git a/pbrs_amd/csrc/device/extend.h b/pbrs_amd/csrc/device/extend.h
--- a/pbrs_amd/csrc/device/extend.h
+++ b/pbrs_amd/csrc/device/extend.h
@@ -1,6 +1,7 @@
 #pragma once
 #include "path_state.h"
 #include "traverse.h"
+#include "packet.h"
 
 template <bool STATS>
 PD void flush_counters(const Cnt<STATS>& cnt, GlobalCounters* g, bool valid, uint32_t rays, uint32_t hits) {
@@ -182,6 +183,21 @@
     return S;
 }
 
+#define PBRS_RETIRE_CLOSEST(S, st, h, item, split)                                                                                                            \
+    do {                                                                                                                                                      \
+        uint32_t cls = (S.n_classes > 1u && h.inst != 0xffffffffu) ? S.inst[h.inst].pad[0] : 0u;                                                              \
+        if (split) {                                                                                                                                          \
+            cls = 1u;                                                                                                                                         \
+            if (h.inst == 0xffffffffu) {                                                                                                                      \
+                const bool specular = (item >> 31) != 0u;                                                                                                     \
+                cls = (specular || ((split & PBRS_QSPLIT_ENV) && S.has_env != 0u)) ? 1u : 0u;                                                                 \
+            }                                                                                                                                                 \
+        }                                                                                                                                                     \
+        const uint32_t pos = item & 0x7fffffffu;                                                                                                              \
+        if (!split || cls) st_stream(&st.hit[pos], make_float4(h.t, __uint_as_float(h.inst), __uint_as_float(h.prim), __uint_as_float(split ? 0u : cls))); \
+        if (S.n_classes > 1u || split) st.cls[pos] = (uint8_t)cls;                                                                                            \
+    } while (0)
+
 template <bool STATS, uint32_t FEAT>
 __global__ void __launch_bounds__(256, STATS ? 3 : (FEAT & PBRS_FEAT_SHADING_CHECK) ? PBRS_TRAV_WAVES : PBRS_LEAN_EXTEND_WAVES)
     k_extend(DevScene G, PathState st, uint32_t set, const uint32_t* count, uint32_t n_direct, uint32_t* next, GlobalCounters* gc, const uint32_t* indirect,
@@ -209,17 +225,7 @@
                 walk.finish(cnt);
                 const Hit& h = walk.best;
                 nhit += h.inst != 0xffffffffu ? 1u : 0u;
-                uint32_t cls = (S.n_classes > 1u && h.inst != 0xffffffffu) ? S.inst[h.inst].pad[0] : 0u;
-                if (split) {
-                    cls = 1u;
-                    if (h.inst == 0xffffffffu) {
-                        const bool specular = (item >> 31) != 0u;
-                        cls = (specular || ((split & PBRS_QSPLIT_ENV) && S.has_env != 0u)) ? 1u : 0u;
-                    }
-                }
-                const uint32_t pos = item & 0x7fffffffu;
-                if (!split || cls) st_stream(&st.hit[pos], make_float4(h.t, __uint_as_float(h.inst), __uint_as_float(h.prim), __uint_as_float(split ? 0u : cls)));
-                if (S.n_classes > 1u || split) st.cls[pos] = (uint8_t)cls;
+                PBRS_RETIRE_CLOSEST(S, st, h, item, split);
                 walk.mode = PBRS_WALK_IDLE;
             }
             if (work.left()) {
@@ -245,3 +251,80 @@
     if (!STATS) PBRS_KP_FLUSH(0, walk);
     if (!STATS) PBRS_TT_FLUSH(0);
 }
+
+#ifndef PBRS_PACKET_WAVES
+#define PBRS_PACKET_WAVES 6
+#endif
+template <uint32_t FEAT>
+__global__ void __launch_bounds__(256, PBRS_PACKET_WAVES)
+    k_extend_packets(DevScene S, PathState st, uint32_t set, const uint32_t* count, uint32_t n_direct, uint32_t* next, GlobalCounters* gc, const uint32_t* indirect,
+                     uint32_t* slow_list, uint32_t* slow_count, uint32_t split) {
+    static_assert((FEAT & PBRS_FEAT_FLAT_TLAS) && !(FEAT & (PBRS_FEAT_SHADING_CHECK | PBRS_FEAT_EXTENT | PBRS_FEAT_LDS_SCENE | PBRS_FEAT_LDS_TOP)), "k_extend_packets: host/kernel_choice.cpp");
+    extern __shared__ __attribute__((aligned(16))) uint32_t lds_stack[];
+    const uint32_t n = count ? *count : n_direct;
+    const float4* q0 = st.q[set][0];
+    const float4* q1 = st.q[set][1];
+    const WaveStack ws = WaveStack::of_wave(lds_stack);
+    LaneStack stk{lds_stack + PBRS_PACKET_LDS_WORDS + threadIdx.x, q0, q1, 0u};
+    Cnt<false> cnt;
+    typedef ClosestWalk<false, (FEAT & PBRS_FEAT_ALL)> Walk;
+    WaveWork work = wave_work_init(n);
+    while (work.left()) {
+        const uint32_t idx = wave_fetch(work, true, next, n);
+        const bool active = idx != 0xffffffffu;
+        if (__ballot(active) == 0) continue;
+        Walk walk;
+        uint32_t item = 0;
+        bool refused = false;
+        {
+            float4 a = make_float4(0.0f, 0.0f, 0.0f, 0.0f), b = make_float4(1.0f, 1.0f, 1.0f, 0.0f);
+            if (active) {
+                stk.item = idx;
+                a = q0[idx], b = q1[idx];
+                item = idx | (__float_as_uint(a.w) & 0x80000000u);
+            }
+            walk.start(S, xyz(a), xyz(b), pn_inf(), stk);
+            refused = active && walk.mode != PBRS_WALK_SCAN;
+            if (!active || refused) walk.mode = PBRS_WALK_DONE;
+        }
+        walk.scan_wave(S, cnt);
+        while (__ballot(walk.mode != PBRS_WALK_DONE)) {
+            bool fresh = false;
+            if (walk.mode == PBRS_WALK_XFER) {
+                const bool entering = !walk.in_blas;
+                walk.xfer_step(S, stk, cnt);
+                if (entering && walk.in_blas) {
+                    fresh = walk.mode == PBRS_WALK_NODE && walk.C.fast;
+                    if (!fresh) {
+                        refused = true;
+                        walk.mode = PBRS_WALK_DONE;
+                    }
+                }
+            }
+            if (packet_meshes<false, false>(S, walk, fresh, stk, ws)) {
+                refused = true;
+                walk.mode = PBRS_WALK_DONE;
+            }
+            if (walk.mode == PBRS_WALK_NODE) {
+                if (walk.cand == 0u) {
+                    walk.mode = PBRS_WALK_DONE;
+                } else {
+                    const uint32_t ni = S.flat_off + (uint32_t)__builtin_ctz(walk.cand);
+                    walk.cand &= walk.cand - 1u;
+                    const pbrs_node node = load_node_at(S.nodes, ni);
+                    if (slab_rs(node, walk.C, walk.lt)) {
+                        walk.cur_inst = node.a;
+                        walk.inst_info = (node.b >> PBRS_TLAS_LEAF_KIND_SHIFT) & 7u;
+                        walk.mode = PBRS_WALK_XFER;
+                    }
+                }
+            }
+        }
+        if (active && !refused) {
+            walk.finish(cnt);
+            const Hit& h = walk.best;
+            PBRS_RETIRE_CLOSEST(S, st, h, item, split);
+        }
+        wave_append_slow(refused, idx, slow_list, slow_count);
+    }
+}
diff --git a/pbrs_amd/csrc/device/intersect.h b/pbrs_amd/csrc/device/intersect.h
--- a/pbrs_amd/csrc/device/intersect.h
+++ b/pbrs_amd/csrc/device/intersect.h
@@ -1,5 +1,39 @@
 #pragma once
 #include "extend.h"
+
+__global__ void __launch_bounds__(256) k_intersect_packets(DevScene S, uint32_t n, const float4* origins, const float4* dirs, const float* tmax, pbrs_hit_record* hits,
+                                                          uint8_t*, uint32_t* info) {
+    extern __shared__ __attribute__((aligned(16))) uint32_t lds_stack[];
+    const WaveStack ws = WaveStack::of_wave(lds_stack);
+    LaneStack stk{lds_stack + PBRS_PACKET_LDS_WORDS + threadIdx.x, origins, dirs, 0u};
+    for (uint32_t base = blockIdx.x * blockDim.x; base < n; base += gridDim.x * blockDim.x) {
+        const uint32_t i = base + threadIdx.x;
+        const bool active = i < n;
+        f3 o = gray(0.0f), d = gray(1.0f);
+        float t_max = 0.0f;
+        if (active) {
+            o = xyz(origins[i]);
+            d = xyz(dirs[i]);
+            t_max = tmax[i];
+            stk.item = i;
+        }
+        Hit h;
+        bool refused = false;
+        if (S.exact_extent) tlas_closest_packets<PBRS_FEAT_EXTENT>(S, active, o, d, t_max, stk, ws, h, refused);
+        else tlas_closest_packets<0u>(S, active, o, d, t_max, stk, ws, h, refused);
+        if (active) {
+            pbrs_hit_record r;
+            r.t = h.t;
+            r.inst = h.inst;
+            r.prim = 0;
+            if (h.inst != 0xffffffffu && S.inst[h.inst].shape_kind == PBRS_SHAPE_MESH) r.prim = S.ts[h.prim].orig;
+            r.b1 = h.b1;
+            r.b2 = h.b2;
+            hits[i] = r;
+            if (refused) atomicAdd(info + 1, 1u);
+        }
+    }
+}
 
 template <bool WIDE_ANY>
 __global__ void __launch_bounds__(256) k_intersect_rays(DevScene S, uint32_t n, const float4* origins, const float4* dirs, const float* tmax,
diff --git a/pbrs_amd/csrc/device/packet.h b/pbrs_amd/csrc/device/packet.h
--- /dev/null
+++ b/pbrs_amd/csrc/device/packet.h
@@ -0,0 +1,158 @@
+#pragma once
+#include "traverse.h"
+
+struct WaveStack {
+    uint32_t* base;
+    PD static WaveStack of_wave(uint32_t* lds) { return WaveStack{lds + (threadIdx.x >> 6) * PBRS_PACKET_WAVE_WORDS}; }
+    PD void put(uint32_t at, uint32_t node, uint64_t mask) const {
+        base[3u * at] = node;
+        base[3u * at + 1u] = (uint32_t)mask;
+        base[3u * at + 2u] = (uint32_t)(mask >> 32);
+    }
+    PD uint32_t node(uint32_t at) const { return (uint32_t)__builtin_amdgcn_readfirstlane((int)base[3u * at]); }
+    PD uint64_t mask(uint32_t at) const {
+        const uint32_t lo = (uint32_t)__builtin_amdgcn_readfirstlane((int)base[3u * at + 1u]), hi = (uint32_t)__builtin_amdgcn_readfirstlane((int)base[3u * at + 2u]);
+        return (uint64_t)lo | ((uint64_t)hi << 32);
+    }
+};
+
+#ifndef PBRS_PACKET_SCALAR_NODES
+#define PBRS_PACKET_SCALAR_NODES 1
+#endif
+#ifndef PBRS_PACKET_CULL
+#define PBRS_PACKET_CULL 1
+#endif
+PD pbrs_node packet_node(const DevScene& S, uint32_t ni) {
+#if PBRS_PACKET_SCALAR_NODES
+    typedef __attribute__((address_space(4))) const pbrs_f4v* const_f4v_ptr;
+    const const_f4v_ptr q = (const_f4v_ptr)(reinterpret_cast<uintptr_t>(S.nodes) + (uintptr_t)ni * sizeof(pbrs_node));
+    const pbrs_f4v a = q[0], b = q[1];
+    pbrs_node n;
+    n.min[0] = a.x; n.min[1] = a.y; n.min[2] = a.z; n.a = __float_as_uint(a.w);
+    n.max[0] = b.x; n.max[1] = b.y; n.max[2] = b.z; n.b = __float_as_uint(b.w);
+    return n;
+#else
+    return load_node_at(S.nodes, ni);
+#endif
+}
+
+template <bool BARY, bool SHADE, class Walk>
+PD bool packet_walk(const DevScene& S, Walk& w, bool take, uint32_t root, WaveStack ws) {
+    const uint64_t all = __ballot(take);
+    if (all == 0) return true;
+    const uint64_t me = 1ull << (threadIdx.x & 63u);
+    RaySpace F = w.C;
+    F.fast = true;
+    uint32_t sp = 0;
+    ws.put(sp++, root, all);
+    while (sp != 0u) {
+        --sp;
+        const uint32_t ni = ws.node(sp);
+        const bool in = (ws.mask(sp) & me) != 0u;
+        const pbrs_node node = packet_node(S, ni);
+        float t_low = 0.0f, hi_el = 0.0f;
+        const bool pass = in && slab_rs(node, F, w.lt, t_low, hi_el);
+        if (__ballot(pass) == 0) continue;
+        const uint32_t nb = (uint32_t)__builtin_amdgcn_readfirstlane((int)node.b), na = (uint32_t)__builtin_amdgcn_readfirstlane((int)node.a);
+        if (!(nb & PBRS_LEAF_FLAG)) {
+            const float dk = comp(w.C.d, (int)(nb & 3u));
+            const bool pos = dk > 0.0f;
+            uint32_t keep = 3u;
+            if constexpr (Walk::CULL && PBRS_PACKET_CULL != 0) {
+                if (pass) keep = w.cull_children(node, dk, t_low, hi_el);
+            }
+            if (pass) w.lt = w.mt;
+            const uint32_t left = ni + 1u, right = na;
+            const uint64_t pos_far = __ballot(pass && pos && (keep & 2u)), pos_near = __ballot(pass && pos && (keep & 1u));
+            const uint64_t neg_far = __ballot(pass && !pos && (keep & 2u)), neg_near = __ballot(pass && !pos && (keep & 1u));
+            if (sp + 4u > PBRS_PACKET_STACK) return false;
+            if (pos_far) ws.put(sp++, right, pos_far);
+            if (pos_near) ws.put(sp++, left, pos_near);
+            if (neg_far) ws.put(sp++, left, neg_far);
+            if (neg_near) ws.put(sp++, right, neg_near);
+        } else {
+            const uint32_t n_tris = nb & ~PBRS_LEAF_FLAG;
+            const float ext = w.lt;
+            for (uint32_t j = 0; j < n_tris; ++j) {
+                const pbrs_tri_verts tv = load_tri(S.tv + na + j);
+                if (pass) {
+                    TriHit h;
+                    bool hit = mesh_tri_hit_t<BARY>(tv, w.C.o, w.C.d, ext, S.fast_slab != 0u, h);
+                    if constexpr (SHADE) {
+                        if (hit && h.t < w.mt && !((w.inst_info >> 3) & PBRS_MESH_SHADING_OK_MASK)) {
+                            f3 n, dpdu;
+                            hit = mesh_tri_shading(tv, S.ts[na + j], w.C.d, h, n, dpdu);
+                        }
+                    }
+                    if (hit && h.t < w.mt) {
+                        w.mt = h.t;
+                        w.mprim = na + j;
+                        w.mb1 = h.b1;
+                        w.mb2 = h.b2;
+                    }
+                }
+            }
+            if (pass) w.lt = w.mt;
+        }
+    }
+    return true;
+}
+
+template <bool BARY, bool SHADE, class Walk>
+PD bool packet_meshes(const DevScene& S, Walk& w, bool fresh, LaneStack stk, WaveStack ws) {
+    bool unfit = false;
+    for (uint64_t m = __ballot(fresh); m != 0; m = __ballot(fresh)) {
+        const int first = __ffsll((unsigned long long)m) - 1;
+        const uint32_t inst = (uint32_t)__builtin_amdgcn_readlane((int)w.cur_inst, first);
+        const bool take = fresh && w.cur_inst == inst;
+        uint32_t root = 0;
+        if (take) root = stk.get(--w.sp);
+        root = (uint32_t)__builtin_amdgcn_readlane((int)root, first);
+        const bool ok = packet_walk<BARY, SHADE>(S, w, take, root, ws);
+        if (take) {
+            fresh = false;
+            unfit = !ok;
+            w.mode = w.exit_mode();
+        }
+    }
+    return unfit;
+}
+
+template <uint32_t EXTRA>
+PD void tlas_closest_packets(const DevScene& S, bool active, f3 o, f3 d, float t_max, LaneStack stk, WaveStack ws, Hit& best, bool& refused) {
+    constexpr uint32_t FEAT = PBRS_FEAT_ALL | EXTRA;
+    Cnt<false> cnt;
+    ClosestWalk<false, FEAT> w;
+    w.start(S, o, d, t_max, stk);
+    refused = active && !w.C.fast;
+    if (!active) w.mode = PBRS_WALK_DONE;
+    w.scan_wave(S, cnt);
+    bool again = false;
+    while (__ballot(w.mode != PBRS_WALK_DONE)) {
+        bool fresh = false;
+        if (w.mode == PBRS_WALK_XFER) {
+            const bool entering = !w.in_blas;
+            w.xfer_step(S, stk, cnt);
+            if (entering && w.in_blas && w.mode == PBRS_WALK_NODE) {
+                fresh = w.C.fast;
+                refused = refused || !fresh;
+            }
+        }
+        if (packet_meshes<true, (FEAT & PBRS_FEAT_SHADING_CHECK) != 0u>(S, w, fresh, stk, ws)) {
+            again = true;
+            w.mode = PBRS_WALK_DONE;
+        }
+        if (w.mode == PBRS_WALK_NODE) w.node_step(S, stk, cnt);
+        if (__ballot(w.mode == PBRS_WALK_LEAF)) w.leaf_wave(S, cnt);
+    }
+    w.finish(cnt);
+    best = w.best;
+    if (__ballot(again)) {
+        Hit alone;
+        tlas_closest<false, EXTRA>(S, again, o, d, t_max, stk, alone, cnt);
+        if (again) {
+            best = alone;
+            refused = true;
+        }
+    }
+}
diff --git a/pbrs_amd/csrc/device/scene.h b/pbrs_amd/csrc/device/scene.h
--- a/pbrs_amd/csrc/device/scene.h
+++ b/pbrs_amd/csrc/device/scene.h
@@ -90,6 +90,13 @@
 #endif
 #define PBRS_LONG_WALK_HEIGHT 12u
 
+#ifndef PBRS_PACKET_STACK
+#define PBRS_PACKET_STACK 128u
+#endif
+#define PBRS_PACKET_WAVE_WORDS (3u * PBRS_PACKET_STACK)
+#define PBRS_PACKET_LDS_WORDS ((kBlock / 64u) * PBRS_PACKET_WAVE_WORDS)
+#define PBRS_PACKET_MIN_SAMPLES 32u
+
 #define PBRS_SHADE_LAMBERT 1u
 #define PBRS_SHADE_LIGHT_SPHERE 2u
 #define PBRS_SHADE_LIGHT_TRIANGLE 4u
diff --git a/pbrs_amd/csrc/host/kernel_choice.cpp b/pbrs_amd/csrc/host/kernel_choice.cpp
--- a/pbrs_amd/csrc/host/kernel_choice.cpp
+++ b/pbrs_amd/csrc/host/kernel_choice.cpp
@@ -22,6 +22,9 @@
         p.extend[0] = {(f.features & PBRS_FEAT_ALL) | steps | p.lds_staging, staged};
         p.extend[1] = {kStatsKey | PBRS_FEAT_ALL, stack};
     }
+    p.camera_packets = dev.camera_packets && !f.exact_extent && (f.features & PBRS_FEAT_FLAT_TLAS) && !(f.features & PBRS_FEAT_SHADING_CHECK) && long_walks && !full_steps &&
+                       !p.lds_staging && 3u * (f.stack_bytes / (kBlock * sizeof(uint32_t))) + 4u <= PBRS_PACKET_STACK;
+    if (p.camera_packets) p.packets = {kPacketKey | kPacketFeatures | (f.features & PBRS_FEAT_ANALYTIC), (PBRS_PACKET_LDS_WORDS + kBlock) * sizeof(uint32_t)};
     const uint32_t shadow_feat = (f.features & PBRS_FEAT_ANALYTIC) | (f.tlas_scanned ? PBRS_FEAT_FLAT_TLAS : 0u) | steps;
     if (p.wide_shadow) {
         p.shadow[0] = {shadow_feat | PBRS_FEAT_WIDE, f.wide_stack_bytes};
diff --git a/pbrs_amd/csrc/host/kernel_choice.h b/pbrs_amd/csrc/host/kernel_choice.h
--- a/pbrs_amd/csrc/host/kernel_choice.h
+++ b/pbrs_amd/csrc/host/kernel_choice.h
@@ -17,6 +17,7 @@
     bool lds_scene = true;
     bool lds_top = true;
     bool raygen_tiles8 = true;
+    bool camera_packets = true;
     uint32_t shade_spec = ~0u;
     uint32_t shade_lds = ~0u;
     std::optional<bool> long_walks, full_steps;
@@ -61,6 +62,10 @@
     if ((f & PBRS_FEAT_LDS_TOP) && (f & (PBRS_FEAT_LDS_SCENE | PBRS_FEAT_FULL_STEPS | PBRS_FEAT_FLAT_TLAS))) return false;
     return true;
 }
+constexpr uint32_t kPacketKey = kTraversalKeys;
+constexpr uint32_t kExtendKeys = 2u * kTraversalKeys;
+constexpr uint32_t kPacketFeatures = PBRS_FEAT_FLAT_TLAS | PBRS_FEAT_LONG_WALKS;
+constexpr bool packet_key_ok(uint32_t k) { return (k & ~PBRS_FEAT_ANALYTIC) == (kPacketKey | kPacketFeatures); }
 constexpr bool shadow_key_ok(uint32_t k) {
     const uint32_t f = k & ~kStatsKey;
     if (k & kStatsKey) return f == kShadowStatsFeatures;
@@ -122,6 +127,8 @@
     TraversalKey shadow[2];
     bool wide_shadow = false;
     TraversalKey shadow_slow;
+    bool camera_packets = false;
+    TraversalKey packets;
     bool split_queue = false;
     uint32_t lds_staging = 0;
     IntegratorChoice integ[PBRS_INTEGRATOR_NORMALS + 1];
diff --git a/pbrs_amd/csrc/host/pass_plan.cpp b/pbrs_amd/csrc/host/pass_plan.cpp
--- a/pbrs_amd/csrc/host/pass_plan.cpp
+++ b/pbrs_amd/csrc/host/pass_plan.cpp
@@ -57,6 +57,10 @@
     return s;
 }
 
+bool camera_packets(const KernelChoice& choice, bool instrumented, uint32_t kc) { return choice.camera_packets && !instrumented && kc >= PBRS_PACKET_MIN_SAMPLES; }
+
+uint32_t pass_chunk_pixels(bool packets, uint32_t chunk, uint32_t P) { return packets ? 1u : chunk > P ? P : chunk; }
+
 BouncePlan bounce_plan(uint32_t integrator, bool split_queue, const IntegratorChoice& ic, int split_decision, uint32_t bounce) {
     BouncePlan b{};
     const bool split = integrator == PBRS_INTEGRATOR_PATH && split_queue && split_decision != 2;
diff --git a/pbrs_amd/csrc/host/pass_plan.h b/pbrs_amd/csrc/host/pass_plan.h
--- a/pbrs_amd/csrc/host/pass_plan.h
+++ b/pbrs_amd/csrc/host/pass_plan.h
@@ -81,6 +81,9 @@
 }
 constexpr CounterLayout kCounters = counter_layout(kMaxDepth, kHeadWords);
 static_assert(kCounters.ns % 2 == 0, "ns is read as 64-bit words");
+constexpr uint32_t kPacketSlowCount = kCounters.slows + kMaxDepth + 1;
+constexpr uint32_t kPacketSlowHeads = kCounters.xhead + (kMaxDepth + 1) * kHeadWords;
+static_assert(kPacketSlowCount < kCounters.xhead && kPacketSlowHeads + kHeadWords <= kCounters.shead, "the spare entries of slows and xhead");
 
 uint32_t samples_per_pass(uint64_t tile_pixels, uint64_t spp, uint32_t requested, bool with_direct, uint64_t held_slots, uint64_t held_direct_bytes,
                           std::optional<uint64_t> free_bytes);
@@ -100,6 +103,9 @@
 };
 PassShape pass_shape(uint32_t P, uint32_t kc);
 
+bool camera_packets(const KernelChoice& choice, bool instrumented, uint32_t kc);
+uint32_t pass_chunk_pixels(bool packets, uint32_t chunk, uint32_t P);
+
 struct BouncePlan {
     uint32_t split;
     IntegratorChoice::Order order;
diff --git a/pbrs_amd/csrc/kernel_tables.h b/pbrs_amd/csrc/kernel_tables.h
--- a/pbrs_amd/csrc/kernel_tables.h
+++ b/pbrs_amd/csrc/kernel_tables.h
@@ -13,9 +13,10 @@
                            const uint32_t*);
 typedef void (*intersect_fn_t)(DevScene, uint32_t, const float4*, const float4*, const float*, pbrs_hit_record*, uint8_t*, uint32_t*);
 
+constexpr uint32_t kIntersectBinaryAny = 0u, kIntersectWideAny = 1u, kIntersectPackets = 2u;
 const extend_fn_t* extend_fns();
 const shadow_fn_t* shadow_fns();
-intersect_fn_t intersect_fn(bool wide_any);
+intersect_fn_t intersect_fn(uint32_t walk);
 
 shade_fn_t shade_fn(const ShadeKey& key);
 
diff --git a/pbrs_amd/csrc/pbrs_gpu.hip b/pbrs_amd/csrc/pbrs_gpu.hip
--- a/pbrs_amd/csrc/pbrs_gpu.hip
+++ b/pbrs_amd/csrc/pbrs_gpu.hip
@@ -60,6 +60,7 @@
     flag("PBRS_LDS_SCENE", o.lds_scene);
     flag("PBRS_LDS_TOP", o.lds_top);
     flag("PBRS_RAYGEN_TILES8", o.raygen_tiles8);
+    flag("PBRS_CAMERA_PACKETS", o.camera_packets);
     if (const char* e = dev_env("PBRS_WIDE")) o.wide_shadow = (std::atoi(e) & 2) != 0;
     if (const char* e = dev_env("PBRS_SHADE_SPEC")) o.shade_spec = (uint32_t)std::atoi(e);
     if (const char* e = dev_env("PBRS_SHADE_LDS")) o.shade_lds = (uint32_t)std::atoi(e);
@@ -83,6 +84,7 @@
 struct KernelPlan {
     KernelChoice choice;
     extend_fn_t extend[2] = {};
+    extend_fn_t packets = nullptr;
     shadow_fn_t shadow[2] = {};
     shadow_fn_t shadow_slow = nullptr;
     IntegratorPlan integ[PBRS_INTEGRATOR_NORMALS + 1];
@@ -462,7 +464,8 @@
         p.shadow[s] = shadow_fns()[ch.shadow[s].key];
     }
     if (ch.wide_shadow) p.shadow_slow = shadow_fns()[ch.shadow_slow.key];
-    bool ok = p.extend[0] && p.extend[1] && p.shadow[0] && p.shadow[1] && (!ch.wide_shadow || p.shadow_slow);
+    if (ch.camera_packets) p.packets = extend_fns()[ch.packets.key];
+    bool ok = p.extend[0] && p.extend[1] && p.shadow[0] && p.shadow[1] && (!ch.wide_shadow || p.shadow_slow) && (!ch.camera_packets || p.packets);
     for (uint32_t i = 0; i <= PBRS_INTEGRATOR_NORMALS; ++i) {
         IntegratorPlan& ip = p.integ[i];
         ip.choice = ch.integ[i];
@@ -516,6 +519,8 @@
     const KernelChoice& choice = plan.choice;
     const IntegratorPlan& ip = plan.integ[rc.integrator];
     const TraversalKey &xk = choice.extend[stats], &sk = choice.shadow[stats];
+    const bool packets = camera_packets(choice, stats, kc);
+    rc.chunk_pixels = pass_chunk_pixels(packets, rc.chunk_pixels, P);
     DevScene xS = c->S;
     if (!(xS.features & PBRS_FEAT_FLAT_TLAS)) xS.n_flat = 0u;
     HIPCHK(c, hipMemsetAsync(set.counters, 0, kCounters.words * sizeof(uint32_t), c->stream));
@@ -532,9 +537,17 @@
         const BouncePlan bp = bounce_plan(rc.integrator, choice.split_queue, ip.choice, c->split_decision, b);
         const uint32_t qsplit = bp.split;
         if (tm.begin(1)) return fail(c, PBRS_E_DEVICE, "event record failed");
-        hipLaunchKernelGGL(plan.extend[stats], dim3(pgrid), dim3(kBlock), xk.lds, c->stream, xS, set.st, b & 1u, cnt_in, N, xhead + b * kHeadWords, c->gcnt, nullptr,
-                           nullptr, nullptr, qsplit);
-        c->pending.kernel_features_extend = reported_features(xk);
+        if (packets && b == 0) {
+            uint32_t* refused = set.counters + kPacketSlowCount;
+            hipLaunchKernelGGL(plan.packets, dim3(pgrid), dim3(kBlock), choice.packets.lds, c->stream, xS, set.st, 0u, nullptr, N, xhead, c->gcnt, nullptr, set.slow, refused,
+                               qsplit);
+            hipLaunchKernelGGL(plan.extend[0], dim3(shape.slow_grid), dim3(kBlock), xk.lds, c->stream, xS, set.st, 0u, refused, N, set.counters + kPacketSlowHeads, c->gcnt,
+                               set.slow, nullptr, nullptr, qsplit);
+        } else {
+            hipLaunchKernelGGL(plan.extend[stats], dim3(pgrid), dim3(kBlock), xk.lds, c->stream, xS, set.st, b & 1u, cnt_in, N, xhead + b * kHeadWords, c->gcnt, nullptr,
+                               nullptr, nullptr, qsplit);
+        }
+        c->pending.kernel_features_extend = reported_features(xk) | (packets ? 0x40000000u : 0u);
         tm.end();
         if (b == 0 && t.want_aovs())
             hipLaunchKernelGGL(k_aov, dim3((P + kBlock - 1) / kBlock), dim3(kBlock), 0, c->stream, c->S, set.st, c->buf[BUF_AOV_STATE].as<float>(), P, kc,
@@ -585,6 +598,8 @@
     if (const FilterConst* filt = t.filt)
         hipLaunchKernelGGL(k_filter_accumulate, dim3((filt->w + PBRS_FILTER_CELL - 1) / PBRS_FILTER_CELL, (filt->h + PBRS_FILTER_CELL - 1) / PBRS_FILTER_CELL),
                            dim3(kBlock), filter_lds_bytes(filt->hx, filt->hy), c->stream, set.st, c->buf[BUF_FILTER_SUM].as<float>(), rc, *filt, kc, c->nonfinite);
+    else if (packets)
+        hipLaunchKernelGGL(k_accumulate_pixels, dim3((P + kBlock - 1) / kBlock), dim3(kBlock), 0, c->stream, set.st, c->sum, P, kc, rc.w, rc.tiles8_per_row, c->nonfinite);
     else
         hipLaunchKernelGGL(k_accumulate, dim3((P + kBlock - 1) / kBlock), dim3(kBlock), 0, c->stream, set.st, c->sum, P, kc, rc.chunk_pixels, rc.w, rc.tiles8_per_row, c->nonfinite);
     if (t.variance)
@@ -719,11 +734,12 @@
     std::lock_guard<std::mutex> lock(g_kernel_cfg_mutex);
     if (c->device < 64 && g_kernel_cfg_done[c->device]) return PBRS_OK;
     const int cap = (int)(kLdsBytesPerCU / 2);
-    std::vector<const void*> traversal_kernels = {reinterpret_cast<const void*>(intersect_fn(false)), reinterpret_cast<const void*>(intersect_fn(true))};
-    for (uint32_t k = 0; k < kTraversalKeys; ++k) {
+    std::vector<const void*> traversal_kernels = {reinterpret_cast<const void*>(intersect_fn(kIntersectBinaryAny)), reinterpret_cast<const void*>(intersect_fn(kIntersectWideAny)),
+                                                  reinterpret_cast<const void*>(intersect_fn(kIntersectPackets))};
+    for (uint32_t k = 0; k < kExtendKeys; ++k)
         if (extend_fns()[k]) traversal_kernels.push_back(reinterpret_cast<const void*>(extend_fns()[k]));
+    for (uint32_t k = 0; k < kTraversalKeys; ++k)
         if (shadow_fns()[k]) traversal_kernels.push_back(reinterpret_cast<const void*>(shadow_fns()[k]));
-    }
     for (const void* k : traversal_kernels) HIPCHK(c, hipFuncSetAttribute(k, hipFuncAttributeMaxDynamicSharedMemorySize, cap));
     if (c->device < 64) g_kernel_cfg_done[c->device] = true;
     return PBRS_OK;
@@ -1568,8 +1584,8 @@
     return collect(c, stats_out);
 }
 
-int pbrs_intersect_rays(pbrs_ctx* c, uint32_t n, const float* origins, const float* dirs, const float* tmax, pbrs_hit_record* hits_out,
-                        uint8_t* occluded_out) {
+static int intersect_queries(pbrs_ctx* c, uint32_t n, const float* origins, const float* dirs, const float* tmax, pbrs_hit_record* hits_out, uint8_t* occluded_out,
+                             bool packets) {
     if (!c) return PBRS_E_INVALID;
     if (!c->has_scene) return fail(c, PBRS_E_NO_SCENE, "no scene uploaded");
     if (n == 0) return PBRS_OK;
@@ -1598,11 +1614,12 @@
     HIPCHK(c, hipMemcpyAsync(d_t, tmax, (size_t)n * 4, hipMemcpyHostToDevice, c->stream));
     {
         const uint32_t rows = std::max(c->stack_depth, c->S.wide_cap);
-        const size_t lds = (size_t)(rows + c->S.n_flat) * kBlock * sizeof(uint32_t);
+        const size_t lds = (size_t)(rows + c->S.n_flat) * kBlock * sizeof(uint32_t) + (packets ? PBRS_PACKET_LDS_WORDS * sizeof(uint32_t) : 0u);
         const dim3 grid(std::min<uint32_t>((n + kBlock - 1) / kBlock, kPersistentBlocks));
-        const bool wide = c->plan.choice.wide_shadow;
+        const bool wide = c->plan.choice.wide_shadow && !packets;
         c->last_intersect = pbrs_intersect_info{wide ? 1u : 0u, 0u, 0u, 0u};
-        hipLaunchKernelGGL(intersect_fn(wide), grid, dim3(kBlock), lds, c->stream, c->S, n, d_o, d_d, d_t, d_h, d_occ, d_info);
+        hipLaunchKernelGGL(intersect_fn(packets ? kIntersectPackets : wide ? kIntersectWideAny : kIntersectBinaryAny), grid, dim3(kBlock), lds, c->stream, c->S, n, d_o, d_d, d_t,
+                           d_h, d_occ, d_info);
     }
     HIPCHK(c, hipGetLastError());
     if (hits_out) HIPCHK(c, hipMemcpyAsync(hits_out, d_h, (size_t)n * sizeof(pbrs_hit_record), hipMemcpyDeviceToHost, c->stream));
@@ -1613,6 +1630,16 @@
     c->last_intersect.slow_any = slow[0];
     c->last_intersect.slow_closest = slow[1];
     return PBRS_OK;
+}
+
+int pbrs_intersect_rays(pbrs_ctx* c, uint32_t n, const float* origins, const float* dirs, const float* tmax, pbrs_hit_record* hits_out,
+                        uint8_t* occluded_out) {
+    return intersect_queries(c, n, origins, dirs, tmax, hits_out, occluded_out, false);
+}
+
+int pbrs_intersect_packets(pbrs_ctx* c, uint32_t n, const float* origins, const float* dirs, const float* tmax, pbrs_hit_record* hits_out) {
+    if (c && n != 0 && !hits_out) return fail(c, PBRS_E_INVALID, "null hit array");
+    return intersect_queries(c, n, origins, dirs, tmax, hits_out, nullptr, true);
 }
 
 int pbrs_last_intersect_info(const pbrs_ctx* c, pbrs_intersect_info* out) {
diff --git a/pbrs_amd/csrc/traverse.hip b/pbrs_amd/csrc/traverse.hip
--- a/pbrs_amd/csrc/traverse.hip
+++ b/pbrs_amd/csrc/traverse.hip
@@ -21,8 +21,14 @@
 
 template <uint32_t K>
 constexpr extend_fn_t extend_fn_of() {
-    if constexpr (extend_key_ok(K)) return &k_extend<(K & kStatsKey) != 0u, (K & ~kStatsKey)>;
-    else return nullptr;
+    if constexpr (K >= kPacketKey) {
+        if constexpr (packet_key_ok(K)) return &k_extend_packets<(K & ~kPacketKey)>;
+        else return nullptr;
+    } else if constexpr (extend_key_ok(K)) {
+        return &k_extend<(K & kStatsKey) != 0u, (K & ~kStatsKey)>;
+    } else {
+        return nullptr;
+    }
 }
 template <uint32_t K>
 constexpr shadow_fn_t shadow_fn_of() {
@@ -44,9 +50,9 @@
 
 namespace pbrs {
 
-const extend_fn_t* extend_fns() { return extend_table(std::make_integer_sequence<uint32_t, kTraversalKeys>{}); }
+const extend_fn_t* extend_fns() { return extend_table(std::make_integer_sequence<uint32_t, kExtendKeys>{}); }
 const shadow_fn_t* shadow_fns() { return shadow_table(std::make_integer_sequence<uint32_t, kTraversalKeys>{}); }
-intersect_fn_t intersect_fn(bool wide_any) { return wide_any ? &k_intersect_rays<true> : &k_intersect_rays<false>; }
+intersect_fn_t intersect_fn(uint32_t walk) { return walk == kIntersectPackets ? &k_intersect_packets : walk == kIntersectWideAny ? &k_intersect_rays<true> : &k_intersect_rays<false>; }
 
 }
 
```

Result: faster. 1841, median of 6 (+9.7%).
